# carmysouschef/mpcium

Hardware: AMD Instinct MI355X
Metric: 4096-bit modexp/s per GPU & node; 2-of-3 ECDSA sigs/s over 10k wallets (higher is better)
Workload: dtype u32; 1 GPU; config2: x^N mod N^2, 4096-bit modulus, shared 2048-bit exponent y=N; operands_per_gpu=65536, modulus_bits=4096, exp_bits=2048, parallelism=shard1 (independent operands, no collective)

## Files before the change

### include/mpcx.h

```cpp
#ifndef MPCX_H_
#define MPCX_H_

#include <stddef.h>
#include <stdint.h>

#ifdef __cplusplus
extern "C" {
#endif

#define MPCX_OK 0
#define MPCX_EINVAL 1
#define MPCX_ENODEV 2
#define MPCX_EHIP 3
#define MPCX_ENOMEM 4

#define MPCX_MAX_MODULUS_BITS 4096

typedef struct mpcx_modulus_s* mpcx_mod_t;

int mpcx_version(void);

const char* mpcx_last_error(void);

int mpcx_device_count(int* out_count);

#define MPCX_MAX_DEVICES 16

int mpcx_init(int device);

int mpcx_init_devices(int n_gpus);

int mpcx_partition(uint32_t count, int n_devices, uint32_t min_slice, uint32_t* first, uint32_t* n,
                   uint32_t* n_slices);

int mpcx_bound_devices(int* out_count, int* ordinals, int max_ordinals);

int mpcx_device_launches(int index, uint64_t* out);

int mpcx_kernel_stats(char* buf, size_t cap, int reset);

int mpcx_select_device(int index);

int mpcx_shutdown(void);

int mpcx_modulus_register(const uint32_t* m_words, uint32_t m_len, mpcx_mod_t* out);
int mpcx_modulus_release(mpcx_mod_t mod);

int mpcx_modulus_info(mpcx_mod_t mod, uint32_t* out_bits, uint32_t* out_class_words);

int mpcx_modexp_batch(mpcx_mod_t mod, uint32_t count,
                      const uint32_t* bases, uint32_t base_words,
                      const uint32_t* exps, uint32_t exp_words, int exp_shared,
                      uint32_t* out, uint32_t out_words);

int mpcx_modexp_batch_device(mpcx_mod_t mod, uint32_t count,
                             const uint32_t* d_bases, uint32_t base_words,
                             const uint32_t* d_exps, uint32_t exp_words, int exp_shared,
                             uint32_t exp_bits,
                             uint32_t* d_out, uint32_t out_words, void* stream);

int mpcx_modexp_mul_batch(mpcx_mod_t mod, uint32_t count,
                          const uint32_t* bases, uint32_t base_words,
                          const uint32_t* exps, uint32_t exp_words, int exp_shared,
                          const uint32_t* muls, uint32_t mul_words,
                          uint32_t* out, uint32_t out_words);
int mpcx_modexp_mul_batch_device(mpcx_mod_t mod, uint32_t count,
                                 const uint32_t* d_bases, uint32_t base_words,
                                 const uint32_t* d_exps, uint32_t exp_words, int exp_shared,
                                 uint32_t exp_bits,
                                 const uint32_t* d_muls, uint32_t mul_words,
                                 uint32_t* d_out, uint32_t out_words, void* stream);

typedef struct mpcx_job_s* mpcx_job_t;
int mpcx_modexp_submit(mpcx_mod_t mod, uint32_t count,
                       const uint32_t* bases, uint32_t base_words,
                       const uint32_t* exps, uint32_t exp_words, int exp_shared,
                       const uint32_t* muls, uint32_t mul_words,
                       uint32_t* out, uint32_t out_words, mpcx_job_t* job);
int mpcx_job_test(mpcx_job_t job, int* done);
int mpcx_job_wait(mpcx_job_t job);

int mpcx_mulmod_batch(mpcx_mod_t mod, uint32_t count,
                      const uint32_t* a, uint32_t a_words,
                      const uint32_t* b, uint32_t b_words,
                      uint32_t* out, uint32_t out_words);

int mpcx_fermat2_batch(uint32_t count, const uint32_t* p, uint32_t p_words, uint8_t* ok);

typedef struct {
  mpcx_mod_t mod;
  uint32_t count;
  const uint32_t* bases;
  uint32_t base_words;
  const uint32_t* exps;
  uint32_t exp_words;
  int exp_shared;
  const uint32_t* muls;
  uint32_t mul_words;
  uint32_t* out;
  uint32_t out_words;
} mpcx_modexp_group_t;
int mpcx_modexp_multi_batch(uint32_t n_groups, const mpcx_modexp_group_t* groups);

int mpcx_ec_combine_batch(uint32_t count, const uint32_t* scalars, const uint32_t* points, uint32_t* out);

int mpcx_mr_batch(uint32_t count, const uint32_t* n, uint32_t n_words, const uint32_t* bases, uint8_t* ok);

int mpcx_lucas_batch(uint32_t count, const uint32_t* n, uint32_t n_words, const uint32_t* P, uint8_t* ok);

int mpcx_safeprime_step(uint64_t seed, const uint8_t* raw, uint64_t stream_off, uint32_t count, uint32_t q_bits,
                        const uint32_t* sprp_q, uint32_t n_sprp, uint32_t max_pass, uint32_t* n_sieved,
                        uint32_t* n_pass, uint32_t* pass_idx, uint32_t* pass_p, uint8_t* sprp_ok);

int mpcx_safeprime_sieve_fermat(const uint8_t* raw, uint32_t nbytes, uint32_t count, uint32_t q_bits,
                                uint32_t* n_out, uint32_t* idx_out, uint8_t* ok_out);

typedef struct mpcx_fixedbase_s* mpcx_fb_t;
#define MPCX_FB_MAX_EXP_BITS 65536
int mpcx_fixedbase_register(mpcx_mod_t mod, const uint32_t* base, uint32_t base_words,
                            uint32_t max_exp_bits, mpcx_fb_t* out);
int mpcx_fixedbase_release(mpcx_fb_t fb);
int mpcx_fixedbase_info(mpcx_fb_t fb, uint32_t* max_exp_bits, size_t* table_bytes);

int mpcx_fixedbase_exp_batch(uint32_t nbases, const mpcx_fb_t* fbs, uint32_t count,
                             const uint32_t* const* exps, const uint32_t* exp_words,
                             const uint32_t* muls, uint32_t mul_words,
                             uint32_t* out, uint32_t out_words);

#define MPCX_FB_MAX_BASES 2
typedef struct {
  uint32_t nbases;
  mpcx_fb_t fbs[MPCX_FB_MAX_BASES];
  uint32_t count;
  const uint32_t* exps[MPCX_FB_MAX_BASES];
  uint32_t exp_words[MPCX_FB_MAX_BASES];
  const uint32_t* muls;
  uint32_t mul_words;
  uint32_t* out;
  uint32_t out_words;
} mpcx_fixedbase_group_t;
int mpcx_fixedbase_multi_batch(uint32_t n_groups, const mpcx_fixedbase_group_t* groups);

int mpcx_dev_alloc(size_t bytes, void** out_ptr);
int mpcx_dev_free(void* ptr);
int mpcx_host_alloc(size_t bytes, void** out_ptr);
int mpcx_host_free(void* ptr);
int mpcx_copy_stats(uint64_t* direct_bytes, uint64_t* bounced_bytes, uint64_t* bounce_allocs);
int mpcx_memcpy_h2d(void* d_dst, const void* h_src, size_t bytes);
int mpcx_memcpy_d2h(void* h_dst, const void* d_src, size_t bytes);
int mpcx_stream_create(void** out_stream);
int mpcx_stream_destroy(void* stream);
int mpcx_stream_sync(void* stream);
int mpcx_sync(void* stream);

int mpcx_set_option(const char* key, int value);
int mpcx_get_option(const char* key, int* value);

int mpcx_mx_tables(const uint32_t* m_words, uint32_t m_len, uint32_t L, uint8_t* out, size_t cap);

int mpcx_modulus_geometry(mpcx_mod_t mod, uint32_t* L, uint32_t* P, uint32_t* K, uint32_t* G);

#ifdef __cplusplus
}
#endif

#endif
```

### mpcium_amd/csrc/mpcx_api.cpp

```cpp
#include <hip/hip_runtime.h>

#include <algorithm>
#include <atomic>
#include <chrono>
#include <cmath>
#include <condition_variable>
#include <cstdarg>
#include <cstdio>
#include <cstdlib>
#include <cstring>
#include <ctime>
#include <deque>
#include <functional>
#include <map>
#include <memory>
#include <mutex>
#include <shared_mutex>
#include <string>
#include <thread>
#include <vector>

#include "../../include/mpcx.h"
#include "mpcx_internal.h"

#define MPCX_GEOM_DECL(g)                                                                              \
  hipError_t mpcx_launch_modexp_g##g(const mpcx::ModexpArgs* a, uint32_t waves, hipStream_t st);     \
  hipError_t mpcx_launch_modexp_multi_g##g(const mpcx::ModexpArgs* segs, const uint32_t* first,      \
                                           uint32_t nsegs, uint32_t waves, int mx, hipStream_t st);  \
  hipError_t mpcx_modexp_occupancy_g##g(int* blocks_per_cu);
#define MPCX_FOR_EACH_GEOM(X) X(0) X(1) X(2) X(3) X(4) X(5) X(6)
static_assert(MPCX_NUM_GEOMS == 7, "update MPCX_FOR_EACH_GEOM and build.py GEOMS");
extern "C" {
MPCX_FOR_EACH_GEOM(MPCX_GEOM_DECL)
hipError_t mpcx_launch_drbg(const mpcx::DrbgArgs* a, hipStream_t st);
hipError_t mpcx_launch_prime2c(mpcx::Prime2Args a, hipStream_t st);
hipError_t mpcx_launch_mrc(const mpcx::MrArgs* a, hipStream_t st);
hipError_t mpcx_launch_lucasc(const mpcx::LucasArgs* a, hipStream_t st);
hipError_t mpcx_launch_lucasc_wide(const mpcx::LucasArgs* a, hipStream_t st);
hipError_t mpcx_launch_expsched(const mpcx::ExpSchedArgs* a, hipStream_t st);
hipError_t mpcx_launch_fixedbase_g0(const mpcx::FixedBaseArgs* a, uint32_t blocks, uint32_t split, hipStream_t st);
hipError_t mpcx_launch_fixedbase_g1(const mpcx::FixedBaseArgs* a, uint32_t blocks, uint32_t split, hipStream_t st);
hipError_t mpcx_launch_fixedbase_multi_g0(const mpcx::FixedBaseArgs* segs, const uint32_t* first, uint32_t nsegs,
                                          uint32_t blocks, uint32_t split, hipStream_t st);
hipError_t mpcx_launch_fixedbase_multi_g1(const mpcx::FixedBaseArgs* segs, const uint32_t* first, uint32_t nsegs,
                                          uint32_t blocks, uint32_t split, hipStream_t st);
hipError_t mpcx_launch_sieve(const mpcx::SieveArgs* a, hipStream_t st);
hipError_t mpcx_launch_selftest(uint32_t* d_out, hipStream_t st);
hipError_t mpcx_launch_ec_combine(const uint32_t* sc, const uint32_t* pts, uint32_t* out, const uint32_t* gtab,
                                  uint32_t* ws, uint32_t count, hipStream_t st);
}

namespace {
constexpr int kMaxDevices = MPCX_MAX_DEVICES;
}

struct mpcx_modulus_s {
  int cls;
  uint32_t bits;
  uint32_t words;
  uint32_t n0inv;
  uint32_t const_off[MPCX_NUM_GEOMS];
  std::vector<uint32_t> m;
  std::vector<uint32_t> host_const;
  std::mutex mu;
  uint32_t* d_const[kMaxDevices] = {};
  std::vector<uint8_t> mx_host;
  uint8_t* d_mx[kMaxDevices] = {};
};

struct mpcx_fixedbase_s {
  mpcx_mod_t mod;
  int geom;
  uint32_t nwin;
  uint32_t wbits;
  std::vector<uint32_t> host_table;
  size_t table_words = 0;
  std::mutex mu;
  uint32_t* d_table[kMaxDevices] = {};
};

namespace {

constexpr int kDigitBits = 28;
constexpr uint32_t kM28 = (1u << kDigitBits) - 1u;

thread_local std::string g_err;
std::mutex g_mu;
int g_force_geom = -1;
double g_narrow_rounds = 0.15;
int g_geom_policy = 1;
int g_fixed_win = 5;
int g_sched_width = MPCX_SCHED_MAX_WIDTH;
int g_main_geom[MPCX_NUM_CLASSES] = {MPCX_MAIN_GEOM(0), MPCX_MAIN_GEOM(1), MPCX_MAIN_GEOM(2)};
int g_fb_window = MPCX_FB_WINDOW_BITS;
#ifndef MPCX_FB_SPLIT_DEFAULT
#define MPCX_FB_SPLIT_DEFAULT 0
#endif
int g_fb_split = MPCX_FB_SPLIT_DEFAULT;
uint32_t g_split_min = 4096;
bool g_dup_device = false;
#ifndef MPCX_MX_DEFAULT
#define MPCX_MX_DEFAULT 1
#endif
int g_mx = MPCX_MX_DEFAULT;
uint32_t g_mx_min = 2048;
uint32_t g_mx_seg_min = 64;
double g_mx_step = 0.81;
double g_geom_tput = 0.0;
struct Staging {
  void* ptr = nullptr;
  size_t bytes = 0;
};
struct Lane {
  std::mutex mu;
  hipStream_t st = nullptr;
  bool own_stream = true;
  hipEvent_t ev = nullptr;
  uint32_t* ws = nullptr;
  size_t ws_bytes = 0;
  Staging stage[4];
  Staging sieve[8];
  struct KEv {
    hipEvent_t a = nullptr, b = nullptr;
  };
  struct KPend {
    KEv ev;
    hipEvent_t ref;
    int dev;
    const char* kind;
    int geom;
    uint32_t ops;
    double alg;
  };
  std::vector<KEv> kev_free;
  std::vector<KPend> kpend;
  struct Bounce {
    char* p = nullptr;
    size_t cap = 0, used = 0;
    size_t peak = 0;
    uint32_t quiet = 0;
  };
  Bounce hin, hout;
  struct Post {
    void* dst;
    const void* src;
    size_t bytes;
  };
  std::vector<Post> post;
  bool pending = false;
};
constexpr int kMaxLanes = 8;
std::atomic<int> g_lanes{6};

struct Device {
  int ordinal = -1;
  hipEvent_t kref = nullptr;
  int num_cus = 0;
  int geom_slots[MPCX_NUM_GEOMS] = {0};
  Lane lanes[kMaxLanes];
  std::atomic<unsigned> lane_rr{0};
  std::mutex dev_mu;
  std::map<hipStream_t, std::unique_ptr<Lane>> dev_lanes;
  Lane build_lane;
  std::atomic<uint64_t> launches{0};
  std::mutex ec_mu;
  uint32_t* ec_gtab = nullptr;
};
Device g_devs[kMaxDevices];
std::atomic<int> g_ndev{0};
std::atomic<unsigned> g_dev_rr{0};
thread_local int t_sel = 0;
thread_local int t_hip = -1;

int fail(int code, const char* fmt, ...) {
  char buf[512];
  va_list ap;
  va_start(ap, fmt);
  vsnprintf(buf, sizeof buf, fmt, ap);
  va_end(ap);
  g_err = buf;
  return code;
}

int hip_fail(hipError_t e, const char* what) {
  return fail(MPCX_EHIP, "%s: %s", what, hipGetErrorString(e));
}

struct PinRegistry {
  std::shared_mutex mu;
  std::map<uintptr_t, size_t> ranges;
  void add(const void* p, size_t bytes) {
    std::unique_lock<std::shared_mutex> lk(mu);
    ranges[(uintptr_t)p] = bytes;
  }
  void remove(const void* p) {
    std::unique_lock<std::shared_mutex> lk(mu);
    ranges.erase((uintptr_t)p);
  }
  int lookup(const void* p, size_t bytes) {
    const uintptr_t a = (uintptr_t)p;
    std::shared_lock<std::shared_mutex> lk(mu);
    auto it = ranges.upper_bound(a);
    if (it == ranges.begin()) return 0;
    --it;
    if (a >= it->first + it->second) return 0;
    return a + bytes <= it->first + it->second ? 1 : -1;
  }
};
PinRegistry g_pins;
std::atomic<uint64_t> g_cp_direct{0}, g_cp_bounced{0}, g_cp_bounce_grow{0};

double go_macs(uint32_t mod_bits, uint32_t e_bits) {
  const double L = (double)((mod_bits + 31) / 32);
  return ((double)e_bits + (double)((e_bits + 3) / 4)) * 2.0 * L * L;
}
void launch_log(const char* kind, int geom, uint32_t count, uint32_t mod_bits, uint32_t exp_bits, double alg) {
  static std::mutex mu;
  static FILE* f = [] {
    const char* p = std::getenv("MPCX_LAUNCH_LOG");
    FILE* h = p && *p ? std::fopen(p, "w") : nullptr;
    if (h) std::fprintf(h, "kind,geom,operands,modulus_bits,exp_bits,alg_macs\n");
    return h;
  }();
  if (!f) return;
  std::lock_guard<std::mutex> lk(mu);
  std::fprintf(f, "%s,%d,%u,%u,%u,%.0f\n", kind, geom, count, mod_bits, exp_bits, alg);
  std::fflush(f);
}

std::atomic<bool> g_kstats{false};
struct KAgg {
  uint64_t launches = 0, ops = 0;
  double alg = 0.0, ms = 0.0;
};
std::mutex g_kmu;
std::map<std::pair<std::string, int>, KAgg> g_kagg;
std::vector<std::pair<double, double>> g_kiv[8];
uint64_t g_kref_host_ns[8] = {};
uint64_t mono_ns() {
  timespec ts{};
  clock_gettime(CLOCK_MONOTONIC, &ts);
  return (uint64_t)ts.tv_sec * 1000000000ull + (uint64_t)ts.tv_nsec;
}
FILE* ktrace_file() {
  static FILE* f = [] {
    const char* p = std::getenv("MPCX_KTRACE");
    FILE* h = p && *p ? std::fopen(p, "w") : nullptr;
    if (h) std::fprintf(h, "dev,kind,geom,ops,t0_ns,t1_ns\n");
    return h;
  }();
  return f;
}

int kstat_begin(Lane& l) {
  if (!g_kstats.load(std::memory_order_relaxed) || l.kpend.size() >= 512) return -1;
  Lane::KEv ev;
  if (!l.kev_free.empty()) {
    ev = l.kev_free.back();
    l.kev_free.pop_back();
  } else if (hipEventCreate(&ev.a) != hipSuccess || hipEventCreate(&ev.b) != hipSuccess) {
    return -1;
  }
  if (hipEventRecord(ev.a, l.st) != hipSuccess) {
    l.kev_free.push_back(ev);
    return -1;
  }
  l.kpend.push_back({ev, nullptr, -1, nullptr, 0, 0, 0.0});
  return (int)l.kpend.size() - 1;
}

void kstat_end(Lane& l, int slot, const Device& d, int dev, const char* kind, int geom, uint32_t ops, double alg) {
  if (slot < 0) return;
  Lane::KPend& p = l.kpend[(size_t)slot];
  if (!d.kref || hipEventRecord(p.ev.b, l.st) != hipSuccess) {
    l.kev_free.push_back(p.ev);
    l.kpend.erase(l.kpend.begin() + slot);
    return;
  }
  p.ref = d.kref;
  p.dev = dev;
  p.kind = kind;
  p.geom = geom;
  p.ops = ops;
  p.alg = alg;
}

void kstat_credit(const char* kind, int geom, uint64_t ops, double alg) {
  if (!g_kstats.load(std::memory_order_relaxed)) return;
  std::lock_guard<std::mutex> lk(g_kmu);
  KAgg& a = g_kagg[{kind, geom}];
  a.ops += ops;
  a.alg += alg;
}

void kstat_resolve(Lane& l) {
  std::lock_guard<std::mutex> lk(g_kmu);
  for (auto& p : l.kpend) {
    float ms = 0.f, t0 = 0.f;
    if (p.kind && hipEventElapsedTime(&ms, p.ev.a, p.ev.b) == hipSuccess &&
        hipEventElapsedTime(&t0, p.ref, p.ev.a) == hipSuccess) {
      KAgg& a = g_kagg[{p.kind, p.geom}];
      a.launches += 1;
      a.ops += p.ops;
      a.alg += p.alg;
      a.ms += ms;
      if (p.dev >= 0 && p.dev < 8) g_kiv[p.dev].push_back({(double)t0, (double)t0 + ms});
      if (FILE* kf = ktrace_file(); kf && p.dev >= 0 && p.dev < 8) {
        const uint64_t b = g_kref_host_ns[p.dev];
        std::fprintf(kf, "%d,%s,%d,%u,%llu,%llu\n", p.dev, p.kind, p.geom, p.ops,
                     (unsigned long long)(b + (uint64_t)(t0 * 1e6)), (unsigned long long)(b + (uint64_t)((t0 + ms) * 1e6)));
      }
    }
    l.kev_free.push_back(p.ev);
  }
  l.kpend.clear();
}

int class_for_bits(uint32_t bits) {
  for (int c = 0; c < MPCX_NUM_CLASSES; ++c)
    if ((int)bits <= MPCX_CLASS_MAXBITS(c)) return c;
  return -1;
}

uint32_t bit_length(const std::vector<uint32_t>& x) {
  for (int i = (int)x.size() - 1; i >= 0; --i)
    if (x[i]) return (uint32_t)(32 * i + (32 - __builtin_clz(x[i])));
  return 0;
}

uint32_t bit_length_words(const uint32_t* x, uint32_t n) {
  for (int i = (int)n - 1; i >= 0; --i)
    if (x[i]) return (uint32_t)(32 * i + (32 - __builtin_clz(x[i])));
  return 0;
}

bool geq(const std::vector<uint32_t>& x, const std::vector<uint32_t>& m) {
  for (int i = (int)x.size() - 1; i >= 0; --i)
    if (x[i] != m[i]) return x[i] > m[i];
  return true;
}

std::vector<uint32_t> pow2_mod(uint32_t k, const std::vector<uint32_t>& m) {
  const size_t n = m.size();
  std::vector<uint32_t> x(n + 1, 0), mm(m);
  mm.push_back(0);
  x[0] = 1;
  if (n == 1 && m[0] == 1) return std::vector<uint32_t>(n, 0);
  for (uint32_t i = 0; i < k; ++i) {
    uint32_t c = 0;
    for (size_t j = 0; j <= n; ++j) {
      const uint32_t nc = x[j] >> 31;
      x[j] = (x[j] << 1) | c;
      c = nc;
    }
    if (geq(x, mm)) {
      uint64_t br = 0;
      for (size_t j = 0; j <= n; ++j) {
        const uint64_t d = (uint64_t)x[j] - mm[j] - br;
        x[j] = (uint32_t)d;
        br = (d >> 63) & 1;
      }
    }
  }
  x.resize(n);
  return x;
}

std::vector<uint32_t> to_digits(const std::vector<uint32_t>& w, uint32_t L) {
  std::vector<uint32_t> d(L, 0);
  for (uint32_t i = 0; i < L; ++i) {
    const uint32_t bit = i * kDigitBits, wi = bit >> 5, s = bit & 31;
    uint64_t v = 0;
    if (wi < w.size()) v = w[wi];
    if (wi + 1 < w.size()) v |= (uint64_t)w[wi + 1] << 32;
    d[i] = (uint32_t)(v >> s) & kM28;
  }
  return d;
}

static void mul_lo(const uint32_t* a, const uint32_t* b, uint32_t* out, uint32_t n) {
  std::vector<uint64_t> acc(n, 0);
  for (uint32_t i = 0; i < n; ++i) {
    uint64_t carry = 0;
    for (uint32_t j = 0; i + j < n; ++j) {
      const uint64_t t = (uint64_t)a[i] * b[j] + (acc[i + j] & 0xFFFFFFFFu) + carry;
      acc[i + j] = (acc[i + j] & ~0xFFFFFFFFull) | (t & 0xFFFFFFFFu);
      carry = t >> 32;
    }
  }
  for (uint32_t i = 0; i < n; ++i) out[i] = (uint32_t)acc[i];
}

struct MxDims {
  uint32_t n7, d, stride, img;
};
static bool mx_dims(uint32_t L, MxDims* o) {
  if (L == mpcx::MxG2::L) {
    *o = {mpcx::MxG2::N7, mpcx::MxG2::D, mpcx::MxG2::TAB_STRIDE, mpcx::MxG2::IMG_BYTES};
  } else if (L == mpcx::MxG5::L) {
    *o = {mpcx::MxG5::N7, mpcx::MxG5::D, mpcx::MxG5::TAB_STRIDE, mpcx::MxG5::IMG_BYTES};
  } else {
    return false;
  }
  return true;
}

static void mx_tables(const std::vector<uint32_t>& m, uint32_t L, std::vector<uint8_t>& out) {
  MxDims dm{};
  (void)mx_dims(L, &dm);
  const uint32_t W = (kDigitBits * L + 31) / 32;
  std::vector<uint32_t> mm(W, 0), x(W, 0), t(W, 0), u(W, 0);
  for (size_t i = 0; i < m.size() && i < W; ++i) mm[i] = m[i];
  uint32_t inv = mm[0];
  for (int i = 0; i < 5; ++i) inv *= 2u - mm[0] * inv;
  x[0] = inv;
  for (uint32_t prec = 1; prec < W;) {
    const uint32_t np = std::min(2 * prec, W);
    mul_lo(mm.data(), x.data(), t.data(), np);
    uint64_t c = 3;
    for (uint32_t i = 0; i < np; ++i) {
      const uint64_t v = (uint64_t)(uint32_t)~t[i] + c;
      t[i] = (uint32_t)v;
      c = v >> 32;
    }
    mul_lo(x.data(), t.data(), u.data(), np);
    for (uint32_t i = 0; i < np; ++i) x[i] = u[i];
    prec = np;
  }
  uint64_t br = 1;
  for (uint32_t i = 0; i < W; ++i) {
    const uint64_t v = (uint64_t)(uint32_t)~x[i] + br;
    x[i] = (uint32_t)v;
    br = v >> 32;
  }
  auto d7 = [](const std::vector<uint32_t>& w, uint32_t d) -> uint8_t {
    const uint32_t bit = 7 * d, wi = bit >> 5, sh = bit & 31;
    uint64_t v = wi < w.size() ? w[wi] : 0;
    if (wi + 1 < w.size()) v |= (uint64_t)w[wi + 1] << 32;
    return (uint8_t)((v >> sh) & 0x7F);
  };
  std::vector<uint8_t> n2(dm.n7), n1(dm.n7);
  std::vector<uint32_t> mv(m);
  for (uint32_t d = 0; d < dm.n7; ++d) {
    n2[d] = d7(x, d);
    n1[d] = d7(mv, d);
  }
  out.assign(dm.img, 0);
  auto fill = [&](const std::vector<uint8_t>& v7, uint8_t* dst) {
    for (int i = 0; i < 16; ++i)
      for (int xx = 0; xx < (int)dm.stride; ++xx) {
        const int idx = (int)dm.d - xx + i;
        if (idx >= 0 && idx < (int)dm.n7) dst[i * dm.stride + xx] = v7[idx];
      }
  };
  fill(n2, out.data());
  fill(n1, out.data() + dm.img / 2);
}

hipError_t mpcx_launch_modexp(int geom, const mpcx::ModexpArgs* a, uint32_t waves, hipStream_t st) {
  switch (geom) {
#define MPCX_CASE(g) \
  case g:            \
    return mpcx_launch_modexp_g##g(a, waves, st);
    MPCX_FOR_EACH_GEOM(MPCX_CASE)
#undef MPCX_CASE
    default:
      return hipErrorInvalidValue;
  }
}

hipError_t mpcx_launch_modexp_multi(int geom, const mpcx::ModexpArgs* segs, const uint32_t* first, uint32_t nsegs,
                                    uint32_t waves, int mx, hipStream_t st) {
  switch (geom) {
#define MPCX_CASE(g) \
  case g:            \
    return mpcx_launch_modexp_multi_g##g(segs, first, nsegs, waves, mx, st);
    MPCX_FOR_EACH_GEOM(MPCX_CASE)
#undef MPCX_CASE
    default:
      return hipErrorInvalidValue;
  }
}

hipError_t mpcx_modexp_occupancy(int geom, int* blocks_per_cu) {
  switch (geom) {
#define MPCX_CASE(g) \
  case g:            \
    return mpcx_modexp_occupancy_g##g(blocks_per_cu);
    MPCX_FOR_EACH_GEOM(MPCX_CASE)
#undef MPCX_CASE
    default:
      return hipErrorInvalidValue;
  }
}

int bind(const Device& d) {
  if (t_hip != d.ordinal) {
    hipError_t e = hipSetDevice(d.ordinal);
    if (e != hipSuccess) return hip_fail(e, "hipSetDevice");
    t_hip = d.ordinal;
  }
  return MPCX_OK;
}

int ndev_or_fail() {
  const int n = g_ndev.load(std::memory_order_acquire);
  if (n <= 0) return -fail(MPCX_ENODEV, "mpcx_init() has not been called");
  return n;
}

int selected(Device** out) {
  const int n = ndev_or_fail();
  if (n < 0) return -n;
  if (t_sel < 0 || t_sel >= n) return fail(MPCX_EINVAL, "selected device %d not bound (%d bound)", t_sel, n);
  *out = &g_devs[t_sel];
  return bind(**out);
}

Lane& acquire_lane(Device& d, std::unique_lock<std::mutex>& lk) {
  const unsigned start = d.lane_rr.fetch_add(1, std::memory_order_relaxed);
  const int nl = g_lanes.load(std::memory_order_relaxed);
  for (int i = 0; i < nl; ++i) {
    Lane& l = d.lanes[(start + i) % nl];
    std::unique_lock<std::mutex> t(l.mu, std::try_to_lock);
    if (t.owns_lock()) {
      lk = std::move(t);
      return l;
    }
  }
  Lane& l = d.lanes[start % nl];
  lk = std::unique_lock<std::mutex>(l.mu);
  return l;
}

int lane_stream(Lane& l) {
  if (!l.st && l.own_stream) {
    hipError_t e = hipStreamCreateWithFlags(&l.st, hipStreamNonBlocking);
    if (e != hipSuccess) {
      l.st = nullptr;
      return hip_fail(e, "hipStreamCreate(lane)");
    }
  }
  if (!l.ev) {
    hipError_t e = hipEventCreateWithFlags(&l.ev, hipEventBlockingSync | hipEventDisableTiming);
    if (e != hipSuccess) {
      l.ev = nullptr;
      return hip_fail(e, "hipEventCreate(lane)");
    }
  }
  return MPCX_OK;
}

constexpr size_t kBounceKeep = (size_t)64 << 20;
constexpr uint32_t kBounceQuiet = 256;
void retire_pinned(char* p, size_t bytes);
void bounce_trim(Lane& l) {
  for (Lane::Bounce* b : {&l.hin, &l.hout}) {
    if (b->cap <= kBounceKeep) {
      b->peak = 0;
      continue;
    }
    b->quiet = b->peak <= kBounceKeep ? b->quiet + 1 : 0;
    b->peak = 0;
    if (b->quiet >= kBounceQuiet) {
      retire_pinned(b->p, b->cap);
      *b = Lane::Bounce{};
    }
  }
}

int lane_wait(Lane& l) {
  static const int mode = [] {
    const char* e = std::getenv("MPCX_LANE_WAIT");
    return !e ? 0 : std::strcmp(e, "event") == 0 ? 1 : std::strcmp(e, "stream") == 0 ? 2 : 0;
  }();
  hipError_t e;
  if (mode == 2) {
    e = hipStreamSynchronize(l.st);
  } else {
    e = hipEventRecord(l.ev, l.st);
    if (e == hipSuccess && mode == 1) {
      e = hipEventSynchronize(l.ev);
    } else if (e == hipSuccess) {
      for (int us = 20;; us = std::min(100, us + us / 2)) {
        e = hipEventQuery(l.ev);
        if (e != hipErrorNotReady) break;
        std::this_thread::sleep_for(std::chrono::microseconds(us));
      }
    }
  }
  if (e != hipSuccess) {
    (void)hipStreamSynchronize(l.st);
    l.post.clear();
    l.hin.used = l.hout.used = 0;
    l.pending = false;
    return hip_fail(e, "lane wait");
  }
  for (const auto& p : l.post) std::memcpy(p.dst, p.src, p.bytes);
  l.post.clear();
  l.hin.used = l.hout.used = 0;
  l.pending = false;
  bounce_trim(l);
  if (!l.kpend.empty()) kstat_resolve(l);
  return MPCX_OK;
}

struct LaneDrain {
  Lane& l;
  explicit LaneDrain(Lane& lane) : l(lane) {}
  ~LaneDrain() {
    if (!l.pending) return;
    if (l.st) (void)hipStreamSynchronize(l.st);
    l.post.clear();
    l.hin.used = l.hout.used = 0;
    l.pending = false;
  }
  LaneDrain(const LaneDrain&) = delete;
  LaneDrain& operator=(const LaneDrain&) = delete;
};

void retire_pinned(char* p, size_t bytes);
int bounce_reserve(Lane& l, Lane::Bounce& b, size_t bytes, char** out) {
  const size_t need = (bytes + 255) & ~(size_t)255;
  if (b.used + need > b.cap) {
    if (l.hin.used || l.hout.used) {
      hipError_t e = hipStreamSynchronize(l.st);
      if (e != hipSuccess) return hip_fail(e, "bounce-buffer wait");
      for (const auto& p : l.post) std::memcpy(p.dst, p.src, p.bytes);
      l.post.clear();
      l.hin.used = l.hout.used = 0;
    }
    if (need > b.cap) {
      if (b.p) retire_pinned(b.p, b.cap);
      b.p = nullptr;
      b.cap = 0;
      const size_t want = std::max<size_t>({need + need / 4, (size_t)1 << 20});
      hipError_t e = hipHostMalloc((void**)&b.p, want, hipHostMallocPortable);
      if (e != hipSuccess) {
        b.p = nullptr;
        return fail(MPCX_ENOMEM, "hipHostMalloc(bounce %zu): %s", want, hipGetErrorString(e));
      }
      b.cap = want;
      g_cp_bounce_grow.fetch_add(1, std::memory_order_relaxed);
    }
  }
  *out = b.p + b.used;
  b.used += need;
  b.peak = std::max(b.peak, b.used);
  return MPCX_OK;
}

int h2d(Lane& l, void* d, const void* h, size_t bytes) {
  if (!bytes) return MPCX_OK;
  const int pin = g_pins.lookup(h, bytes);
  if (pin < 0) return fail(MPCX_EINVAL, "host source of %zu B at %p overruns its pinned allocation", bytes, h);
  const void* src = h;
  if (pin == 0) {
    char* b = nullptr;
    if (int rc = bounce_reserve(l, l.hin, bytes, &b)) return rc;
    std::memcpy(b, h, bytes);
    src = b;
    g_cp_bounced.fetch_add(bytes, std::memory_order_relaxed);
  } else {
    g_cp_direct.fetch_add(bytes, std::memory_order_relaxed);
  }
  l.pending = true;
  hipError_t e = hipMemcpyAsync(d, src, bytes, hipMemcpyHostToDevice, l.st);
  return e == hipSuccess ? MPCX_OK : hip_fail(e, "copy inputs");
}

int d2h(Lane& l, void* h, const void* d, size_t bytes) {
  if (!bytes) return MPCX_OK;
  const int pin = g_pins.lookup(h, bytes);
  if (pin < 0) return fail(MPCX_EINVAL, "host destination of %zu B at %p overruns its pinned allocation", bytes, h);
  void* dst = h;
  if (pin == 0) {
    char* b = nullptr;
    if (int rc = bounce_reserve(l, l.hout, bytes, &b)) return rc;
    dst = b;
    l.post.push_back({h, b, bytes});
    g_cp_bounced.fetch_add(bytes, std::memory_order_relaxed);
  } else {
    g_cp_direct.fetch_add(bytes, std::memory_order_relaxed);
  }
  l.pending = true;
  hipError_t e = hipMemcpyAsync(dst, d, bytes, hipMemcpyDeviceToHost, l.st);
  return e == hipSuccess ? MPCX_OK : hip_fail(e, "copy results");
}

int d2h_sync(void* h, const void* d, size_t bytes, Lane& l) {
  if (int rc = d2h(l, h, d, bytes)) return rc;
  return lane_wait(l);
}

constexpr size_t kStageChunk = (size_t)16 << 20;
struct StageChunks {
  std::mutex mu;
  std::vector<char*> free_list;
  size_t allocated = 0;
  char* get() {
    {
      std::lock_guard<std::mutex> lk(mu);
      if (!free_list.empty()) {
        char* c = free_list.back();
        free_list.pop_back();
        return c;
      }
    }
    char* c = nullptr;
    if (hipHostMalloc((void**)&c, kStageChunk, hipHostMallocPortable) != hipSuccess) return nullptr;
    std::lock_guard<std::mutex> lk(mu);
    ++allocated;
    return c;
  }
  void put(char* c) {
    std::lock_guard<std::mutex> lk(mu);
    free_list.push_back(c);
  }
  void release_all() {
    std::lock_guard<std::mutex> lk(mu);
    for (char* c : free_list) (void)hipHostFree(c);
    free_list.clear();
    allocated = 0;
  }
};
StageChunks g_stage_chunks;

constexpr size_t kRetireMax = (size_t)1 << 30;
std::mutex g_retire_mu;
std::vector<std::pair<char*, size_t>> g_retired;
size_t g_retired_bytes = 0;
void retire_pinned(char* p, size_t bytes) {
  std::vector<std::pair<char*, size_t>> out;
  {
    std::lock_guard<std::mutex> lk(g_retire_mu);
    g_retired.push_back({p, bytes});
    g_retired_bytes += bytes;
    if (g_retired_bytes > kRetireMax) {
      out.swap(g_retired);
      g_retired_bytes = 0;
    }
  }
  for (auto& r : out) (void)hipHostFree(r.first);
}
void free_retired() {
  std::lock_guard<std::mutex> lk(g_retire_mu);
  for (auto& r : g_retired) (void)hipHostFree(r.first);
  g_retired.clear();
  g_retired_bytes = 0;
}

int copy_sync(void* dst, const void* src, size_t bytes, hipMemcpyKind kind, hipStream_t st) {
  if (!bytes) return MPCX_OK;
  const void* hp = kind == hipMemcpyHostToDevice ? src : dst;
  const int pin = g_pins.lookup(hp, bytes);
  if (pin < 0) return fail(MPCX_EINVAL, "host range of %zu B at %p overruns its pinned allocation", bytes, hp);
  hipError_t e;
  if (pin == 1) {
    e = hipMemcpyAsync(dst, src, bytes, kind, st);
    if (e == hipSuccess) e = hipStreamSynchronize(st);
    return e == hipSuccess ? MPCX_OK : hip_fail(e, "copy");
  }
  char* buf = g_stage_chunks.get();
  if (!buf) return fail(MPCX_ENOMEM, "hipHostMalloc(copy chunk %zu)", kStageChunk);
  const size_t cb = std::min(bytes, kStageChunk);
  e = hipSuccess;
  for (size_t off = 0; off < bytes && e == hipSuccess; off += cb) {
    const size_t n = std::min(cb, bytes - off);
    if (kind == hipMemcpyHostToDevice) {
      std::memcpy(buf, (const char*)src + off, n);
      e = hipMemcpyAsync((char*)dst + off, buf, n, kind, st);
      if (e == hipSuccess) e = hipStreamSynchronize(st);
    } else {
      e = hipMemcpyAsync(buf, (const char*)src + off, n, kind, st);
      if (e == hipSuccess) e = hipStreamSynchronize(st);
      if (e == hipSuccess) std::memcpy((char*)dst + off, buf, n);
    }
  }
  g_stage_chunks.put(buf);
  g_cp_bounced.fetch_add(bytes, std::memory_order_relaxed);
  return e == hipSuccess ? MPCX_OK : hip_fail(e, "copy");
}

size_t grown(size_t old_bytes, size_t bytes) {
  return std::max<size_t>({bytes + bytes / 4, old_bytes + old_bytes / 2, (size_t)1 << 20});
}

int ensure_buffer(Staging& s, size_t bytes) {
  if (s.bytes >= bytes && s.ptr) return MPCX_OK;
  const size_t want = grown(s.bytes, bytes);
  if (s.ptr) (void)hipFree(s.ptr);
  s.ptr = nullptr;
  s.bytes = 0;
  hipError_t e = hipMalloc(&s.ptr, want);
  if (e != hipSuccess) return fail(MPCX_ENOMEM, "hipMalloc(%zu): %s", want, hipGetErrorString(e));
  s.bytes = want;
  return MPCX_OK;
}

int ensure_workspace(Lane& l, size_t bytes) {
  if (l.ws_bytes >= bytes) return MPCX_OK;
  if (l.ws) {
    (void)hipStreamSynchronize(l.st);
    (void)hipFree(l.ws);
  }
  const size_t want = grown(l.ws_bytes, bytes);
  l.ws = nullptr;
  l.ws_bytes = 0;
  hipError_t e = hipMalloc((void**)&l.ws, want);
  if (e != hipSuccess) return fail(MPCX_ENOMEM, "hipMalloc(workspace %zu): %s", want, hipGetErrorString(e));
  l.ws_bytes = want;
  return MPCX_OK;
}

void drop_lane(Lane& l) {
  std::lock_guard<std::mutex> ll(l.mu);
  if (l.st) {
    (void)hipStreamSynchronize(l.st);
    if (l.own_stream) (void)hipStreamDestroy(l.st);
  }
  l.st = nullptr;
  if (l.ev) (void)hipEventDestroy(l.ev);
  l.ev = nullptr;
  for (auto& p : l.kpend) l.kev_free.push_back(p.ev);
  l.kpend.clear();
  for (auto& ev : l.kev_free) {
    (void)hipEventDestroy(ev.a);
    (void)hipEventDestroy(ev.b);
  }
  l.kev_free.clear();
  if (l.ws) (void)hipFree(l.ws);
  l.ws = nullptr;
  l.ws_bytes = 0;
  for (auto& s : l.stage) {
    if (s.ptr) (void)hipFree(s.ptr);
    s = Staging{};
  }
  for (auto& s : l.sieve) {
    if (s.ptr) (void)hipFree(s.ptr);
    s = Staging{};
  }
  for (Lane::Bounce* b : {&l.hin, &l.hout}) {
    if (b->p) (void)hipHostFree(b->p);
    *b = Lane::Bounce{};
  }
  l.post.clear();
  l.pending = false;
}

Lane& stream_lane(Device& d, hipStream_t st) {
  std::lock_guard<std::mutex> lk(d.dev_mu);
  auto& p = d.dev_lanes[st];
  if (!p) {
    p.reset(new Lane());
    p->own_stream = false;
    p->st = st;
  }
  return *p;
}

int run_selftest() {
  uint32_t* d = nullptr;
  hipError_t e = hipMalloc((void**)&d, 256 * sizeof(uint32_t));
  if (e != hipSuccess) return hip_fail(e, "selftest alloc");
  e = mpcx_launch_selftest(d, nullptr);
  std::vector<uint32_t> h(256);
  if (e == hipSuccess && copy_sync(h.data(), d, 256 * sizeof(uint32_t), hipMemcpyDeviceToHost, nullptr) != MPCX_OK)
    e = hipErrorInvalidValue;
  (void)hipFree(d);
  if (e != hipSuccess) return hip_fail(e, "selftest");
  for (uint32_t l = 0; l < 64; ++l) {
    const uint32_t nxt = l < 63 ? 1000 + l + 1 : 0;
    const uint32_t prv = l > 0 ? 1000 + l - 1 : 0;
    const uint32_t bp = 2000 + (l / 7) * 7;
    const uint64_t acc = (uint64_t)(0xFFFFFFF0u + l) * (0xFFFFFFF7u - l) + 0xFFFFFFFFFFFFull;
    if (h[l] != nxt || h[64 + l] != prv || h[128 + l] != bp || h[192 + l] != (uint32_t)(acc >> 32))
      return fail(MPCX_EHIP,
                  "device self-test failed at lane %u (dpp next %u/%u prev %u/%u bpermute %u/%u mad %u/%u)", l,
                  h[l], nxt, h[64 + l], prv, h[128 + l], bp, h[192 + l], (uint32_t)(acc >> 32));
  }
  return MPCX_OK;
}

int bind_new_device(int ordinal) {
  const int n = g_ndev.load();
  for (int i = 0; i < n && !g_dup_device; ++i)
    if (g_devs[i].ordinal == ordinal) return MPCX_OK;
  if (n >= kMaxDevices) return fail(MPCX_EINVAL, "more than %d devices", kMaxDevices);
  int vis = 0;
  hipError_t e = hipGetDeviceCount(&vis);
  if (e != hipSuccess || vis <= 0) return fail(MPCX_ENODEV, "no HIP device visible");
  if (ordinal < 0 || ordinal >= vis) return fail(MPCX_EINVAL, "device %d out of range [0,%d)", ordinal, vis);
  e = hipSetDevice(ordinal);
  if (e != hipSuccess) return hip_fail(e, "hipSetDevice");
  t_hip = ordinal;
  hipDeviceProp_t prop;
  e = hipGetDeviceProperties(&prop, ordinal);
  if (e != hipSuccess) return hip_fail(e, "hipGetDeviceProperties");
  if (std::strncmp(prop.gcnArchName, "gfx950", 6) != 0)
    return fail(MPCX_ENODEV, "device %d is %s; libmpcx is built for gfx950 only", ordinal, prop.gcnArchName);
  Device& d = g_devs[n];
  d.ordinal = ordinal;
  d.num_cus = prop.multiProcessorCount;
  for (int g = 0; g < MPCX_NUM_GEOMS; ++g) {
    int b = 0;
    if (mpcx_modexp_occupancy(g, &b) != hipSuccess || b <= 0) b = 1;
    d.geom_slots[g] = b * d.num_cus;
  }
  int rc = run_selftest();
  if (rc != MPCX_OK) {
    d.ordinal = -1;
    return rc;
  }
  g_ndev.store(n + 1, std::memory_order_release);
  return MPCX_OK;
}

int mod_const(mpcx_mod_t mod, int di, const uint32_t** out) {
  std::lock_guard<std::mutex> lk(mod->mu);
  if (!mod->d_const[di]) {
    uint32_t* p = nullptr;
    hipError_t e = hipMalloc((void**)&p, mod->host_const.size() * sizeof(uint32_t));
    if (e != hipSuccess) return fail(MPCX_ENOMEM, "hipMalloc(modulus): %s", hipGetErrorString(e));
    if (int rc = copy_sync(p, mod->host_const.data(), mod->host_const.size() * sizeof(uint32_t),
                           hipMemcpyHostToDevice, nullptr)) {
      (void)hipFree(p);
      return rc;
    }
    mod->d_const[di] = p;
  }
  *out = mod->d_const[di];
  return MPCX_OK;
}

int mx_const(mpcx_mod_t mod, int di, const uint8_t** out) {
  std::lock_guard<std::mutex> lk(mod->mu);
  if (!mod->d_mx[di]) {
    if (mod->mx_host.empty()) mx_tables(mod->m, (uint32_t)MPCX_GEOM_L(MPCX_MAIN_GEOM(mod->cls)), mod->mx_host);
    uint8_t* p = nullptr;
    hipError_t e = hipMalloc((void**)&p, mod->mx_host.size());
    if (e != hipSuccess) return fail(MPCX_ENOMEM, "hipMalloc(mx tables): %s", hipGetErrorString(e));
    if (int rc = copy_sync(p, mod->mx_host.data(), mod->mx_host.size(), hipMemcpyHostToDevice, nullptr)) {
      (void)hipFree(p);
      return rc;
    }
    mod->d_mx[di] = p;
  }
  *out = mod->d_mx[di];
  return MPCX_OK;
}

int fb_table(mpcx_fb_t fb, int di, const uint32_t** out) {
  std::lock_guard<std::mutex> lk(fb->mu);
  if (!fb->d_table[di]) {
    uint32_t* p = nullptr;
    const size_t bytes = fb->table_words * sizeof(uint32_t);
    hipError_t e = hipMalloc((void**)&p, bytes);
    if (e != hipSuccess) return fail(MPCX_ENOMEM, "hipMalloc(fixed-base table %zu B)", bytes);
    if (!fb->host_table.empty()) {
      const int rc = copy_sync(p, fb->host_table.data(), bytes, hipMemcpyHostToDevice, nullptr);
      e = rc ? hipErrorInvalidValue : hipSuccess;
      if (rc == MPCX_OK) std::vector<uint32_t>().swap(fb->host_table);
    } else {
      int src = -1;
      for (int j = 0; j < kMaxDevices && src < 0; ++j)
        if (fb->d_table[j]) src = j;
      e = src < 0 ? hipErrorInvalidValue
                  : hipMemcpyPeerAsync(p, g_devs[di].ordinal, fb->d_table[src], g_devs[src].ordinal, bytes, nullptr);
      if (e == hipSuccess) e = hipStreamSynchronize(nullptr);
    }
    if (e != hipSuccess) {
      (void)hipFree(p);
      return hip_fail(e, "upload fixed-base table");
    }
    fb->d_table[di] = p;
  }
  *out = fb->d_table[di];
  return MPCX_OK;
}

uint32_t partition(uint32_t count, int n_dev, uint32_t min_slice, uint32_t* first, uint32_t* cnt) {
  uint32_t slices = n_dev > 0 ? (uint32_t)n_dev : 1u;
  if (min_slice == 0) slices = 1;
  else slices = std::min<uint32_t>(slices, std::max<uint32_t>(1, count / min_slice));
  const uint32_t per = (count + slices - 1) / std::max<uint32_t>(slices, 1);
  uint32_t used = 0;
  for (uint32_t s = 0; s < slices; ++s) {
    const uint32_t f = std::min(count, s * per), c = std::min(count, f + per) - f;
    if (first) first[s] = f;
    if (cnt) cnt[s] = c;
    used = s + 1;
  }
  return used;
}

int run_sliced(uint32_t count, uint32_t min_slice, const std::function<int(int, uint32_t, uint32_t)>& fn) {
  const int n = ndev_or_fail();
  if (n < 0) return -n;
  uint32_t first[kMaxDevices], cnt[kMaxDevices];
  const uint32_t slices = partition(count, n, min_slice, first, cnt);
  if (slices <= 1) {
    const int di = (int)(g_dev_rr.fetch_add(1, std::memory_order_relaxed) % (unsigned)n);
    int rc = bind(g_devs[di]);
    return rc ? rc : fn(di, 0, count);
  }
  std::vector<int> rcs(slices, MPCX_OK);
  std::vector<std::string> msgs(slices);
  std::vector<std::thread> th;
  for (uint32_t s = 0; s < slices; ++s) {
    th.emplace_back([&, s] {
      int rc = bind(g_devs[s]);
      if (!rc) rc = fn((int)s, first[s], cnt[s]);
      rcs[s] = rc;
      if (rc) msgs[s] = g_err;
    });
  }
  for (auto& t : th) t.join();
  for (uint32_t s = 0; s < slices; ++s)
    if (rcs[s]) {
      g_err = msgs[s];
      return rcs[s];
    }
  return MPCX_OK;
}

bool geom_serves(int g, const mpcx_modulus_s* mod, bool ops_fit) {
  const uint32_t rb = (uint32_t)MPCX_GEOM_RBITS(g);
  if (mod->bits + 2u > rb) return false;
  return ops_fit || rb >= 32u * (uint32_t)MPCX_CLASS_WORDS(mod->cls);
}

bool host_ops_below(const uint32_t* x, uint32_t count, uint32_t words, uint32_t rbits) {
  if (!x || 32u * words <= rbits) return true;
  const uint32_t w0 = rbits / 32u, sh = rbits % 32u;
  for (uint32_t i = 0; i < count; ++i) {
    const uint32_t* v = x + (size_t)i * words;
    if (sh && (v[w0] >> sh)) return false;
    for (uint32_t w = w0 + (sh ? 1u : 0u); w < words; ++w)
      if (v[w]) return false;
  }
  return true;
}

int main_geom_for(const mpcx_modulus_s* mod, bool ops_fit) {
  const int g = g_main_geom[mod->cls];
  return geom_serves(g, mod, ops_fit) ? g : MPCX_FULL_GEOM(mod->cls);
}


bool runs_on_mx(int g, uint32_t total, uint32_t min_seg, bool multi) {
  const bool has_kernel = g == 2 || (g == 5 && !multi && g_mx >= 2);
  return g_mx && has_kernel && total >= g_mx_min && (!multi || min_seg >= g_mx_seg_min);
}

int fastest_geom(int cls, uint32_t count, int nsimd, bool mx_ok) {
  struct M {
    int g;
    double c0, s;
  };
  const M ms[3] = {{MPCX_MAIN_GEOM(cls), 0.10, mx_ok ? g_mx_step : 1.0}, {MPCX_MID_GEOM(cls), 0.12, 0.585},
                   {MPCX_NARROW_GEOM(cls), 0.20, 0.245}};
  int best = ms[0].g;
  double tb = 1e300;
  for (const M& m : ms) {
    const uint32_t G = (uint32_t)MPCX_GEOM_G(m.g);
    const double waves = (double)((count + G - 1) / G);
    const double t = m.c0 + m.s * std::ceil(waves / (double)std::max(1, nsimd)) +
                     g_geom_tput * m.s * waves / (double)std::max(1, nsimd);
    if (t < tb) {
      tb = t;
      best = m.g;
    }
  }
  return best;
}

int choose_geom(const Device& dev, int cls, uint32_t count, bool main_serves, bool forced_serves, bool mx_ok) {
  const int gm = main_serves ? g_main_geom[cls] : MPCX_FULL_GEOM(cls);
  const int gn = MPCX_NARROW_GEOM(cls), gmid = MPCX_MID_GEOM(cls);
  if (g_force_geom >= 0 && MPCX_GEOM_CLASS(g_force_geom) == cls)
    return forced_serves ? g_force_geom : MPCX_FULL_GEOM(cls);
  if (g_geom_policy == 2) return gm;
  if (g_geom_policy == 1 && gmid >= 0 && gn >= 0) return fastest_geom(cls, count, dev.num_cus * 4, mx_ok && main_serves);
  const uint32_t G = (uint32_t)MPCX_GEOM_G(gm);
  const double rounds = (double)((count + G - 1) / G) / (double)std::max(1, dev.geom_slots[gm]);
  if (gn >= 0 && rounds < g_narrow_rounds) return gn;
  return gm;
}

int check_batch(const char* pre, const mpcx_modulus_s* mod, uint32_t count, const uint32_t* bases,
                uint32_t base_words, const uint32_t* exps, uint32_t exp_words, const uint32_t* muls,
                uint32_t mul_words, const uint32_t* out, uint32_t out_words) {
  const bool grp = *pre;
  const uint32_t cw = (uint32_t)MPCX_CLASS_WORDS(mod->cls);
  if (base_words == 0 || base_words > cw)
    return grp ? fail(MPCX_EINVAL, "%sbase_words %u", pre, base_words)
               : fail(MPCX_EINVAL, "base_words %u outside [1, %u] (reduce mod m first)", base_words, cw);
  if (muls && (mul_words == 0 || mul_words > cw))
    return grp ? fail(MPCX_EINVAL, "%smul_words", pre)
               : fail(MPCX_EINVAL, "mul_words %u outside [1, %u]", mul_words, cw);
  if (out_words < mod->words)
    return grp ? fail(MPCX_EINVAL, "%sout_words < modulus words", pre)
               : fail(MPCX_EINVAL, "out_words %u < modulus words %u", out_words, mod->words);
  if (count && (!bases || !out || (exp_words && !exps))) return fail(MPCX_EINVAL, "%snull buffer", pre);
  return MPCX_OK;
}

double go_macs_sum(uint32_t mod_bits, const uint32_t* exps, uint32_t exp_words, uint32_t count) {
  double alg = 0.0;
  for (uint32_t i = 0; i < count; ++i)
    alg += go_macs(mod_bits, bit_length_words(exps + (size_t)i * exp_words, exp_words));
  return alg;
}

int launch_expsched(const uint32_t* d_exp, uint32_t exp_words, uint32_t* sched, hipStream_t st) {
  mpcx::ExpSchedArgs sa{};
  sa.exp = d_exp;
  sa.exp_words = exp_words;
  sa.max_width = (uint32_t)g_sched_width;
  sa.sched = sched;
  hipError_t e = mpcx_launch_expsched(&sa, st);
  return e == hipSuccess ? MPCX_OK : hip_fail(e, "launch k_expsched");
}

mpcx::ModexpArgs modexp_args(const mpcx_modulus_s* mod, int geom, const uint32_t* dconst, uint32_t count,
                             const uint32_t* base, uint32_t base_words, const uint32_t* exps, uint32_t exp_words,
                             const uint32_t* mul, uint32_t mul_words, uint32_t* out, uint32_t out_words,
                             uint32_t* table, uint32_t exp_bits, int exp_shared, const uint32_t* sched,
                             const uint8_t* mx_img, uint32_t nwaves) {
  const uint32_t L = (uint32_t)MPCX_GEOM_L(geom);
  mpcx::ModexpArgs a{};
  a.nd = dconst + mod->const_off[geom];
  a.r1d = a.nd + L;
  a.r2d = a.nd + 2 * L;
  a.base = base;
  a.exps = exps;
  a.mul = mul;
  a.out = out;
  a.table = table;
  a.count = count;
  a.base_words = base_words;
  a.exp_words = exp_words;
  a.mul_words = mul ? mul_words : 0;
  a.exp_bits = exp_words ? exp_bits : 0;
  a.win_bits = (!exp_shared && a.exp_bits > 1024u && g_fixed_win >= 5) ? 5u : 4u;
  a.out_words = out_words;
  a.n0inv = mod->n0inv;
  a.exp_shared = exp_shared ? 1 : 0;
  a.sched = sched;
  a.mx_img = mx_img;
  a.nwaves = nwaves;
  return a;
}


int fb_group_check(const mpcx_fixedbase_group_t& g, const char* pre, uint32_t* nwin) {
  const bool grp = *pre;
  if (g.nbases == 0 || g.nbases > MPCX_FB_MAX_BASES)
    return fail(MPCX_EINVAL, "%snbases %u outside [1, %d]", pre, g.nbases, MPCX_FB_MAX_BASES);
  for (uint32_t t = 0; t < g.nbases; ++t) {
    if (!g.fbs[t]) return fail(MPCX_EINVAL, "%snull fixed base %u", pre, t);
    if (g.fbs[t]->mod != g.fbs[0]->mod) return fail(MPCX_EINVAL, "%sfixed bases of different moduli", pre);
  }
  mpcx_mod_t mod = g.fbs[0]->mod;
  const uint32_t cw = (uint32_t)MPCX_CLASS_WORDS(mod->cls);
  if (g.out_words < mod->words)
    return grp ? fail(MPCX_EINVAL, "%sout_words < modulus words", pre)
               : fail(MPCX_EINVAL, "out_words %u < modulus words %u", g.out_words, mod->words);
  if (g.muls && (g.mul_words == 0 || g.mul_words > cw))
    return grp ? fail(MPCX_EINVAL, "%smul_words", pre)
               : fail(MPCX_EINVAL, "mul_words %u outside [1, %u]", g.mul_words, cw);
  if (g.count == 0) return MPCX_OK;
  if (!g.out) return fail(MPCX_EINVAL, "%snull output", pre);
  for (uint32_t t = 0; t < g.nbases; ++t) {
    if (g.exp_words[t] && !g.exps[t]) return fail(MPCX_EINVAL, "%snull exponents %u", pre, t);
    uint32_t bits = 0;
    for (uint32_t i = 0; i < g.count && g.exp_words[t]; ++i)
      bits = std::max(bits, bit_length_words(g.exps[t] + (size_t)i * g.exp_words[t], g.exp_words[t]));
    const uint32_t wb = g.fbs[t]->wbits;
    if (bits > g.fbs[t]->nwin * wb)
      return fail(MPCX_EINVAL, "%sexponent of %u bits > fixed-base table's %u", pre, bits, g.fbs[t]->nwin * wb);
    nwin[t] = (bits + wb - 1) / wb;
  }
  return MPCX_OK;
}

struct FbWork {
  double alg = 0.0, exec = 0.0;
  uint32_t eb_max = 0;
};
FbWork fb_group_work(const mpcx_fixedbase_group_t& g) {
  FbWork w;
  const uint32_t bits = g.fbs[0]->mod->bits;
  const double l2 = 2.0 * (double)((bits + 31) / 32) * (double)((bits + 31) / 32);
  for (uint32_t t = 0; t < g.nbases; ++t)
    for (uint32_t i = 0; i < g.count && g.exp_words[t]; ++i) {
      const uint32_t b = bit_length_words(g.exps[t] + (size_t)i * g.exp_words[t], g.exp_words[t]);
      w.alg += go_macs(bits, b);
      w.exec += (double)((b + g.fbs[t]->wbits - 1) / g.fbs[t]->wbits) * l2;
      w.eb_max = std::max(w.eb_max, b);
    }
  if (g.muls) w.exec += (double)g.count * l2;
  return w;
}

int fixedbase_args(const mpcx_fixedbase_group_t& g, int geom, int di, const uint32_t* nwin,
                   const uint32_t* const* d_exps, const uint32_t* d_mul, uint32_t* d_out, mpcx::FixedBaseArgs* out) {
  mpcx_mod_t mod = g.fbs[0]->mod;
  const uint32_t* dconst = nullptr;
  int rc;
  if ((rc = mod_const(mod, di, &dconst))) return rc;
  mpcx::FixedBaseArgs a{};
  a.nd = dconst + mod->const_off[geom];
  a.r1d = a.nd + MPCX_GEOM_L(geom);
  a.r2d = a.nd + 2 * MPCX_GEOM_L(geom);
  for (uint32_t t = 0; t < g.nbases; ++t) {
    if ((rc = fb_table(g.fbs[t], di, &a.tables[t]))) return rc;
    a.exps[t] = d_exps[t];
    a.exp_words[t] = g.exp_words[t];
    a.nwin[t] = nwin[t];
    a.wbits[t] = g.fbs[t]->wbits;
  }
  a.nbases = g.nbases;
  a.mul = g.muls ? d_mul : nullptr;
  a.mul_words = g.muls ? g.mul_words : 0;
  a.out = d_out;
  a.out_words = g.out_words;
  a.count = g.count;
  a.n0inv = mod->n0inv;
  *out = a;
  return MPCX_OK;
}

int fb_geom_for(const mpcx_modulus_s* mod) { return MPCX_FULL_GEOM(mod->cls); }
hipError_t launch_fixedbase(int geom, const mpcx::FixedBaseArgs* a, uint32_t blocks, uint32_t split, hipStream_t st) {
  return geom == 0 ? mpcx_launch_fixedbase_g0(a, blocks, split, st) : mpcx_launch_fixedbase_g1(a, blocks, split, st);
}
hipError_t launch_fixedbase_multi(int geom, const mpcx::FixedBaseArgs* segs, const uint32_t* first, uint32_t nsegs,
                                  uint32_t blocks, uint32_t split, hipStream_t st) {
  return geom == 0 ? mpcx_launch_fixedbase_multi_g0(segs, first, nsegs, blocks, split, st)
                   : mpcx_launch_fixedbase_multi_g1(segs, first, nsegs, blocks, split, st);
}

constexpr uint32_t kFbSplitWaves = 4;
uint32_t fb_split_for(const Device& dev, uint32_t blocks) {
  if (g_fb_split) return (uint32_t)g_fb_split;
  const uint64_t cap = (uint64_t)std::max(1, dev.num_cus) * 4u * kFbSplitWaves;
  for (uint32_t s = MPCX_FB_MAX_SPLIT; s > 1; s >>= 1)
    if ((uint64_t)blocks * s <= cap) return s;
  return 1;
}

}

extern "C" {

int mpcx_version(void) { return 200; }

int mpcx_get_option(const char* key, int* value) {
  if (!key || !value) return fail(MPCX_EINVAL, "null option or output");
  std::lock_guard<std::mutex> lk(g_mu);
  if (std::strcmp(key, "mx") == 0) {
    *value = g_mx;
  } else if (std::strcmp(key, "mx_min") == 0) {
    *value = (int)g_mx_min;
  } else if (std::strcmp(key, "mx_seg_min") == 0) {
    *value = (int)g_mx_seg_min;
  } else if (std::strcmp(key, "mx_step") == 0) {
    *value = (int)std::lround(g_mx_step * 100.0);
  } else if (std::strcmp(key, "geom_tput") == 0) {
    *value = (int)std::lround(g_geom_tput * 100.0);
  } else if (std::strcmp(key, "geom_policy") == 0) {
    *value = g_geom_policy;
  } else if (std::strcmp(key, "sched_width") == 0) {
    *value = g_sched_width;
  } else if (std::strcmp(key, "fixed_window") == 0) {
    *value = g_fixed_win;
  } else if (std::strcmp(key, "fb_split") == 0) {
    *value = g_fb_split;
  } else if (std::strcmp(key, "lanes") == 0) {
    *value = g_lanes.load();
  } else {
    return fail(MPCX_EINVAL, "option %s cannot be read", key);
  }
  return MPCX_OK;
}

int mpcx_set_option(const char* key, int value) {
  if (!key) return fail(MPCX_EINVAL, "null option");
  std::lock_guard<std::mutex> lk(g_mu);
  if (std::strcmp(key, "force_geom") == 0) {
    if (value < -1 || value >= MPCX_NUM_GEOMS) return fail(MPCX_EINVAL, "force_geom %d out of range", value);
    g_force_geom = value;
  } else if (std::strcmp(key, "sched_width") == 0) {
    if (value < 0 || value > MPCX_SCHED_MAX_WIDTH) return fail(MPCX_EINVAL, "sched_width %d out of range", value);
    g_sched_width = value;
  } else if (std::strcmp(key, "narrow_rounds") == 0) {
    if (value < 0 || value > 100) return fail(MPCX_EINVAL, "narrow_rounds %d out of range", value);
    g_narrow_rounds = value / 100.0;
  } else if (std::strcmp(key, "fb_window") == 0) {
    if (value < 4 || value > MPCX_FB_MAX_WINDOW_BITS) return fail(MPCX_EINVAL, "fb_window %d out of range", value);
    g_fb_window = value;
  } else if (std::strcmp(key, "fb_split") == 0) {
    if (value != 0 && value != 1 && value != 2 && value != 4) return fail(MPCX_EINVAL, "fb_split %d not 0/1/2/4", value);
    g_fb_split = value;
  } else if (std::strcmp(key, "mx") == 0) {
    if (value < 0 || value > 2) return fail(MPCX_EINVAL, "mx %d not 0, 1 or 2", value);
    g_mx = value;
  } else if (std::strcmp(key, "mx_min") == 0) {
    if (value < 1) return fail(MPCX_EINVAL, "mx_min %d < 1", value);
    g_mx_min = (uint32_t)value;
  } else if (std::strcmp(key, "mx_seg_min") == 0) {
    if (value < 1) return fail(MPCX_EINVAL, "mx_seg_min %d < 1", value);
    g_mx_seg_min = (uint32_t)value;
  } else if (std::strcmp(key, "mx_step") == 0) {
    if (value < 10 || value > 200) return fail(MPCX_EINVAL, "mx_step %d outside [10, 200]", value);
    g_mx_step = value / 100.0;
  } else if (std::strcmp(key, "geom_tput") == 0) {
    if (value < 0 || value > 1000) return fail(MPCX_EINVAL, "geom_tput %d outside [0, 1000]", value);
    g_geom_tput = value / 100.0;
  } else if (std::strcmp(key, "fixed_window") == 0) {
    if (value != 4 && value != 5) return fail(MPCX_EINVAL, "fixed_window %d not 4 or 5", value);
    g_fixed_win = value;
  } else if (std::strcmp(key, "lanes") == 0) {
    if (value < 1 || value > kMaxLanes) return fail(MPCX_EINVAL, "lanes %d outside [1, %d]", value, kMaxLanes);
    g_lanes = value;
  } else if (std::strcmp(key, "geom_policy") == 0) {
    if (value < 0 || value > 2) return fail(MPCX_EINVAL, "geom_policy %d out of range", value);
    g_geom_policy = value;
  } else if (std::strcmp(key, "main_geom") == 0) {
    if (value < 0 || value >= MPCX_NUM_GEOMS) return fail(MPCX_EINVAL, "main_geom %d out of range", value);
    g_main_geom[MPCX_GEOM_CLASS(value)] = value;
  } else if (std::strcmp(key, "duplicate_device") == 0) {
    g_dup_device = value != 0;
  } else if (std::strcmp(key, "kernel_stats") == 0) {
    g_kstats = value != 0;
  } else if (std::strcmp(key, "device_split_min") == 0) {
    if (value < 0) return fail(MPCX_EINVAL, "device_split_min %d < 0", value);
    g_split_min = (uint32_t)value;
  } else {
    return fail(MPCX_EINVAL, "unknown option %s", key);
  }
  return MPCX_OK;
}

const char* mpcx_last_error(void) { return g_err.c_str(); }

int mpcx_device_count(int* out_count) {
  if (!out_count) return fail(MPCX_EINVAL, "null out_count");
  int n = 0;
  hipError_t e = hipGetDeviceCount(&n);
  if (e != hipSuccess) n = 0;
  *out_count = n;
  return MPCX_OK;
}

static void read_env_options() {
  const char* nr = std::getenv("MPCX_NARROW_ROUNDS");
  if (nr) g_narrow_rounds = std::max(0, std::min(100, std::atoi(nr))) / 100.0;
  const char* gp = std::getenv("MPCX_GEOM_POLICY");
  if (gp) g_geom_policy = std::max(0, std::min(2, std::atoi(gp)));
  const char* ln = std::getenv("MPCX_LANES");
  if (ln && g_ndev.load() == 0) g_lanes = std::max(1, std::min(kMaxLanes, std::atoi(ln)));
  const char* fw = std::getenv("MPCX_FB_WINDOW");
  if (fw) g_fb_window = std::max(4, std::min(MPCX_FB_MAX_WINDOW_BITS, std::atoi(fw)));
  const char* mx = std::getenv("MPCX_MX");
  if (mx) g_mx = std::max(0, std::min(2, std::atoi(mx)));
  const char* ms = std::getenv("MPCX_MX_STEP");
  if (ms) g_mx_step = std::max(10, std::min(200, std::atoi(ms))) / 100.0;
  const char* gt = std::getenv("MPCX_GEOM_TPUT");
  if (gt) g_geom_tput = std::max(0, std::min(1000, std::atoi(gt))) / 100.0;
}

int mpcx_init(int device) {
  std::lock_guard<std::mutex> lk(g_mu);
  read_env_options();
  return bind_new_device(device);
}

int mpcx_init_devices(int n_gpus) {
  std::lock_guard<std::mutex> lk(g_mu);
  read_env_options();
  int vis = 0;
  hipError_t e = hipGetDeviceCount(&vis);
  if (e != hipSuccess || vis <= 0) return fail(MPCX_ENODEV, "no HIP device visible");
  if (n_gpus <= 0) n_gpus = vis;
  if (n_gpus > vis) return fail(MPCX_EINVAL, "%d GPUs requested, %d visible", n_gpus, vis);
  for (int i = 0; i < n_gpus; ++i)
    if (int rc = bind_new_device(i)) return rc;
  return MPCX_OK;
}

int mpcx_bound_devices(int* out_count, int* ordinals, int max_ordinals) {
  if (!out_count) return fail(MPCX_EINVAL, "null out_count");
  const int n = g_ndev.load(std::memory_order_acquire);
  *out_count = n;
  for (int i = 0; ordinals && i < n && i < max_ordinals; ++i) ordinals[i] = g_devs[i].ordinal;
  return MPCX_OK;
}

int mpcx_partition(uint32_t count, int n_devices, uint32_t min_slice, uint32_t* first, uint32_t* n,
                   uint32_t* n_slices) {
  if (!n_slices) return fail(MPCX_EINVAL, "null n_slices");
  if (n_devices < 1 || n_devices > kMaxDevices) return fail(MPCX_EINVAL, "n_devices %d outside [1, %d]", n_devices, kMaxDevices);
  *n_slices = partition(count, n_devices, min_slice, first, n);
  return MPCX_OK;
}

int mpcx_device_launches(int index, uint64_t* out) {
  const int n = g_ndev.load(std::memory_order_acquire);
  if (!out) return fail(MPCX_EINVAL, "null out");
  if (index < 0 || index >= n) return fail(MPCX_EINVAL, "device index %d not bound (%d bound)", index, n);
  *out = g_devs[index].launches.load();
  return MPCX_OK;
}

int mpcx_kernel_stats(char* buf, size_t cap, int reset) {
  const int n = g_ndev.load(std::memory_order_acquire);
  std::string out;
  {
    std::lock_guard<std::mutex> lk(g_kmu);
    double busy = 0.0, alg = 0.0;
    for (int i = 0; i < n && i < 8; ++i) {
      auto iv = g_kiv[i];
      std::sort(iv.begin(), iv.end());
      double s0 = 0.0, e0 = -1.0;
      for (const auto& x : iv) {
        if (x.first > e0) {
          if (e0 > s0) busy += e0 - s0;
          s0 = x.first;
          e0 = x.second;
        } else {
          e0 = std::max(e0, x.second);
        }
      }
      if (e0 > s0) busy += e0 - s0;
    }
    char line[320];
    std::string ks;
    for (const auto& kv : g_kagg) {
      alg += kv.second.alg;
      std::snprintf(line, sizeof line,
                    "%s{\"kind\":\"%s\",\"geom\":%d,\"launches\":%llu,\"operands\":%llu,\"alg_macs\":%.6e,"
                    "\"kernel_ms\":%.4f}",
                    ks.empty() ? "" : ",", kv.first.first.c_str(), kv.first.second,
                    (unsigned long long)kv.second.launches, (unsigned long long)kv.second.ops, kv.second.alg,
                    kv.second.ms);
      ks += line;
    }
    std::snprintf(line, sizeof line, "{\"enabled\":%d,\"busy_ms\":%.4f,\"alg_macs\":%.6e,\"kernels\":[",
                  g_kstats.load() ? 1 : 0, busy, alg);
    out = line + ks + "]}";
    if (reset) {
      g_kagg.clear();
      for (auto& v : g_kiv) v.clear();
    }
  }
  if (reset) {
    for (int i = 0; i < n; ++i) {
      Device& d = g_devs[i];
      if (int rc = bind(d)) return rc;
      hipError_t e = d.kref ? hipSuccess : hipEventCreate(&d.kref);
      if (e == hipSuccess) e = hipEventRecord(d.kref, nullptr);
      if (e == hipSuccess) e = hipEventSynchronize(d.kref);
      if (e != hipSuccess) return hip_fail(e, "kernel stats time origin");
      if (i < 8) g_kref_host_ns[i] = mono_ns();
    }
  }
  if (buf && cap) {
    if (out.size() + 1 > cap) return fail(MPCX_EINVAL, "kernel stats need %zu bytes", out.size() + 1);
    std::memcpy(buf, out.c_str(), out.size() + 1);
  }
  return MPCX_OK;
}

int mpcx_select_device(int index) {
  const int n = g_ndev.load(std::memory_order_acquire);
  if (index < 0 || index >= n) return fail(MPCX_EINVAL, "device index %d not bound (%d bound)", index, n);
  t_sel = index;
  return bind(g_devs[index]);
}

int mpcx_shutdown(void) {
  std::lock_guard<std::mutex> lk(g_mu);
  const int n = g_ndev.load();
  for (int i = 0; i < n; ++i) {
    Device& d = g_devs[i];
    if (hipSetDevice(d.ordinal) != hipSuccess) continue;
    t_hip = d.ordinal;
    for (auto& l : d.lanes) drop_lane(l);
    drop_lane(d.build_lane);
    if (d.ec_gtab) (void)hipFree(d.ec_gtab);
    d.ec_gtab = nullptr;
    {
      std::lock_guard<std::mutex> dl(d.dev_mu);
      for (auto& kv : d.dev_lanes) drop_lane(*kv.second);
      d.dev_lanes.clear();
    }
    d.ordinal = -1;
  }
  g_stage_chunks.release_all();
  free_retired();
  g_ndev.store(0);
  return MPCX_OK;
}

int mpcx_modulus_register(const uint32_t* m_words, uint32_t m_len, mpcx_mod_t* out) {
  if (!m_words || !out || m_len == 0) return fail(MPCX_EINVAL, "null modulus or output");
  Device* dev = nullptr;
  if (int rc = selected(&dev)) return rc;
  std::vector<uint32_t> m(m_words, m_words + m_len);
  while (m.size() > 1 && m.back() == 0) m.pop_back();
  const uint32_t bits = bit_length(m);
  if (bits == 0) return fail(MPCX_EINVAL, "modulus is zero");
  if ((m[0] & 1u) == 0) return fail(MPCX_EINVAL, "modulus is even (math/big uses a non-Montgomery path; keep it on the host)");
  const int cls = class_for_bits(bits);
  if (cls < 0) return fail(MPCX_EINVAL, "modulus has %u bits > %d", bits, MPCX_MAX_MODULUS_BITS);
  auto* mod = new mpcx_modulus_s();
  mod->cls = cls;
  mod->bits = bits;
  mod->words = (uint32_t)m.size();
  mod->m = m;
  uint32_t inv = m[0];
  for (int i = 0; i < 5; ++i) inv *= 2u - m[0] * inv;
  mod->n0inv = (0u - inv) & kM28;
  for (int g = 0; g < MPCX_NUM_GEOMS; ++g) {
    mod->const_off[g] = 0;
    if (MPCX_GEOM_CLASS(g) != cls) continue;
    const uint32_t L = (uint32_t)MPCX_GEOM_L(g);
    mod->const_off[g] = (uint32_t)mod->host_const.size();
    auto nd = to_digits(m, L);
    auto r1 = to_digits(pow2_mod(kDigitBits * L, m), L);
    auto r2 = to_digits(pow2_mod(2 * kDigitBits * L, m), L);
    auto& h = mod->host_const;
    h.insert(h.end(), nd.begin(), nd.end());
    h.insert(h.end(), r1.begin(), r1.end());
    h.insert(h.end(), r2.begin(), r2.end());
  }
  const uint32_t* p = nullptr;
  if (int rc = mod_const(mod, (int)(dev - g_devs), &p)) {
    delete mod;
    return rc;
  }
  *out = mod;
  return MPCX_OK;
}

int mpcx_modulus_release(mpcx_mod_t mod) {
  if (!mod) return fail(MPCX_EINVAL, "null modulus");
  const int n = g_ndev.load();
  for (int i = 0; i < n && i < kMaxDevices; ++i) {
    if (mod->d_const[i] && bind(g_devs[i]) == MPCX_OK) (void)hipFree(mod->d_const[i]);
    if (mod->d_mx[i] && bind(g_devs[i]) == MPCX_OK) (void)hipFree(mod->d_mx[i]);
  }
  delete mod;
  return MPCX_OK;
}

int mpcx_mx_tables(const uint32_t* m_words, uint32_t m_len, uint32_t L, uint8_t* out, size_t cap) {
  if (!m_words || !out || m_len == 0) return fail(MPCX_EINVAL, "null modulus or output");
  MxDims dm{};
  if (!mx_dims(L, &dm)) return fail(MPCX_EINVAL, "L %u is not an MX geometry's (148 or 74)", L);
  if (cap < dm.img) return fail(MPCX_EINVAL, "mx tables need %u bytes", dm.img);
  std::vector<uint32_t> m(m_words, m_words + m_len);
  while (m.size() > 1 && m.back() == 0) m.pop_back();
  if ((m[0] & 1u) == 0 || bit_length(m) + 2 > kDigitBits * L)
    return fail(MPCX_EINVAL, "mx tables need an odd modulus of < %u bits", kDigitBits * L - 2);
  std::vector<uint8_t> t;
  mx_tables(m, L, t);
  std::memcpy(out, t.data(), dm.img);
  return MPCX_OK;
}

int mpcx_modulus_info(mpcx_mod_t mod, uint32_t* out_bits, uint32_t* out_class_words) {
  if (!mod) return fail(MPCX_EINVAL, "null modulus");
  if (out_bits) *out_bits = mod->bits;
  if (out_class_words) *out_class_words = (uint32_t)MPCX_CLASS_WORDS(mod->cls);
  return MPCX_OK;
}

int mpcx_modulus_geometry(mpcx_mod_t mod, uint32_t* L, uint32_t* P, uint32_t* K, uint32_t* G) {
  if (!mod) return fail(MPCX_EINVAL, "null modulus");
  const int g = main_geom_for(mod, true);
  if (L) *L = (uint32_t)MPCX_GEOM_L(g);
  if (P) *P = (uint32_t)MPCX_GEOM_P(g);
  if (K) *K = (uint32_t)MPCX_GEOM_K(g);
  if (G) *G = (uint32_t)MPCX_GEOM_G(g);
  return MPCX_OK;
}

}

static int modexp_enqueue(int di, Lane& lane, mpcx_mod_t mod, uint32_t count, const uint32_t* d_bases,
                          uint32_t base_words, const uint32_t* d_exps, uint32_t exp_words, int exp_shared,
                          uint32_t exp_bits, const uint32_t* d_muls, uint32_t mul_words, uint32_t* d_out,
                          uint32_t out_words, bool ops_fit, double alg_macs = -1.0) {
  Device& dev = g_devs[di];
  int rc;
  if ((rc = check_batch("", mod, count, d_bases, base_words, d_exps, exp_words, d_muls, mul_words, d_out, out_words)))
    return rc;
  if (exp_bits > 32u * exp_words) return fail(MPCX_EINVAL, "exp_bits %u > 32*exp_words", exp_bits);
  if (count == 0) return MPCX_OK;
  const uint32_t* dconst = nullptr;
  if ((rc = mod_const(mod, di, &dconst))) return rc;
  const int cls = mod->cls;
  const bool forced_serves =
      g_force_geom >= 0 && MPCX_GEOM_CLASS(g_force_geom) == cls && geom_serves(g_force_geom, mod, ops_fit);
  const bool mx_ok = runs_on_mx(main_geom_for(mod, ops_fit), count, count, false);
  const int geom = choose_geom(dev, cls, count, geom_serves(g_main_geom[cls], mod, ops_fit), forced_serves, mx_ok);
  const uint32_t G = (uint32_t)MPCX_GEOM_G(geom), K = (uint32_t)MPCX_GEOM_K(geom);
  const uint32_t waves = (count + G - 1) / G;
  const bool use_sched = exp_shared && exp_bits > 0 && g_sched_width > 0;
  const size_t sched_off = (size_t)waves * MPCX_TABLE_ENTRIES * K * 64u;
  const size_t ws_words = sched_off + (use_sched ? MPCX_SCHED_WORDS(32u * exp_words) : 0);
  if ((rc = ensure_workspace(lane, ws_words * sizeof(uint32_t)))) return rc;
  uint32_t* sched = use_sched ? lane.ws + sched_off : nullptr;
  if (use_sched && (rc = launch_expsched(d_exps, exp_words, sched, lane.st))) return rc;
  const bool mx = runs_on_mx(geom, count, count, false);
  const uint8_t* mx_img = nullptr;
  if (mx && (rc = mx_const(mod, di, &mx_img))) return rc;
  const mpcx::ModexpArgs a =
      modexp_args(mod, geom, dconst, count, d_bases, base_words, d_exps, exp_words, d_muls, mul_words, d_out,
                  out_words, lane.ws, exp_bits, exp_shared, sched, mx_img, waves);
  const char* kind = mx ? "modexp_mx" : "modexp";
  const int ks = kstat_begin(lane);
  hipError_t e = mpcx_launch_modexp(geom, &a, waves, lane.st);
  if (e != hipSuccess) return hip_fail(e, "launch k_modexp");
  dev.launches.fetch_add(1, std::memory_order_relaxed);
  const double alg = alg_macs >= 0 ? alg_macs : go_macs(mod->bits, a.exp_bits) * count;
  kstat_end(lane, ks, dev, di, kind, geom, count, alg);
  launch_log(kind, geom, count, mod->bits, a.exp_bits, alg);
  return MPCX_OK;
}

static uint32_t max_exp_bits(const uint32_t* exps, uint32_t exp_words, int exp_shared, uint32_t count) {
  uint32_t bits = 0;
  if (!exp_words) return 0;
  if (exp_shared) return bit_length_words(exps, exp_words);
  for (uint32_t i = 0; i < count; ++i) bits = std::max(bits, bit_length_words(exps + (size_t)i * exp_words, exp_words));
  return bits;
}

static int modexp_host_range(int di, mpcx_mod_t mod, uint32_t count, const uint32_t* bases, uint32_t base_words,
                             const uint32_t* exps, uint32_t exp_words, int exp_shared, const uint32_t* muls,
                             uint32_t mul_words, uint32_t* out, uint32_t out_words) {
  const uint32_t exp_bits = max_exp_bits(exps, exp_words, exp_shared, count);
  const size_t n_exp_words = exp_shared ? exp_words : (size_t)count * exp_words;
  const size_t bb = (size_t)count * base_words * 4, eb = std::max<size_t>(n_exp_words * 4, 4),
               ob = (size_t)count * out_words * 4, mb = muls ? (size_t)count * mul_words * 4 : 0;
  std::unique_lock<std::mutex> lk;
  Lane& l = acquire_lane(g_devs[di], lk);
  LaneDrain drain(l);
  int rc;
  if ((rc = lane_stream(l))) return rc;
  Staging* sg = l.stage;
  if ((rc = ensure_buffer(sg[0], bb)) || (rc = ensure_buffer(sg[1], eb)) || (rc = ensure_buffer(sg[2], ob)) ||
      (muls && (rc = ensure_buffer(sg[3], mb))))
    return rc;
  if ((rc = h2d(l, sg[0].ptr, bases, bb)) || (rc = h2d(l, sg[1].ptr, exps, n_exp_words * 4)) ||
      (muls && (rc = h2d(l, sg[3].ptr, muls, mb))))
    return rc;
  const uint32_t rb = (uint32_t)MPCX_GEOM_RBITS(g_main_geom[mod->cls]);
  const bool ops_fit = host_ops_below(bases, count, base_words, rb) && host_ops_below(muls, count, mul_words, rb);
  const double alg = !exp_shared && exp_words ? go_macs_sum(mod->bits, exps, exp_words, count) : -1.0;
  rc = modexp_enqueue(di, l, mod, count, (const uint32_t*)sg[0].ptr, base_words, (const uint32_t*)sg[1].ptr,
                      exp_words, exp_shared, exp_bits, muls ? (const uint32_t*)sg[3].ptr : nullptr, mul_words,
                      (uint32_t*)sg[2].ptr, out_words, ops_fit, alg);
  if (rc) return rc;
  return d2h_sync(out, sg[2].ptr, ob, l);
}

static int modexp_host(mpcx_mod_t mod, uint32_t count, const uint32_t* bases, uint32_t base_words,
                       const uint32_t* exps, uint32_t exp_words, int exp_shared, const uint32_t* muls,
                       uint32_t mul_words, uint32_t* out, uint32_t out_words) {
  if (!mod) return fail(MPCX_EINVAL, "null modulus");
  if (count == 0) return MPCX_OK;
  if (!bases || !out || (exp_words && !exps)) return fail(MPCX_EINVAL, "null buffer");
  return run_sliced(count, g_split_min, [&](int di, uint32_t first, uint32_t n) {
    return modexp_host_range(di, mod, n, bases + (size_t)first * base_words, base_words,
                             exps ? (exp_shared ? exps : exps + (size_t)first * exp_words) : nullptr, exp_words,
                             exp_shared, muls ? muls + (size_t)first * mul_words : nullptr, mul_words,
                             out + (size_t)first * out_words, out_words);
  });
}

struct mpcx_job_s {
  std::mutex mu;
  std::condition_variable cv;
  bool done = false;
  int rc = MPCX_OK;
  std::string msg;
  std::function<int()> work;
};

namespace {
struct JobPool {
  std::mutex mu;
  std::condition_variable cv;
  std::deque<mpcx_job_t> q;
  std::vector<std::thread> th;
  void start(size_t n) {
    while (th.size() < n)
      th.emplace_back([this] {
        for (;;) {
          mpcx_job_t j;
          {
            std::unique_lock<std::mutex> lk(mu);
            cv.wait(lk, [&] { return !q.empty(); });
            j = q.front();
            q.pop_front();
          }
          const int rc = j->work();
          std::lock_guard<std::mutex> lk(j->mu);
          j->rc = rc;
          if (rc) j->msg = g_err;
          j->done = true;
          j->cv.notify_all();
        }
      });
  }
};
JobPool& job_pool() {
  static JobPool* p = new JobPool();
  return *p;
}
}

extern "C" {

int mpcx_modexp_batch_device(mpcx_mod_t mod, uint32_t count, const uint32_t* d_bases, uint32_t base_words,
                             const uint32_t* d_exps, uint32_t exp_words, int exp_shared, uint32_t exp_bits,
                             uint32_t* d_out, uint32_t out_words, void* stream) {
  if (!mod) return fail(MPCX_EINVAL, "null modulus");
  Device* dev = nullptr;
  if (int rc = selected(&dev)) return rc;
  Lane& l = stream_lane(*dev, (hipStream_t)stream);
  std::lock_guard<std::mutex> lk(l.mu);
  const bool ops_fit = 32u * base_words <= (uint32_t)MPCX_GEOM_RBITS(g_main_geom[mod->cls]);
  return modexp_enqueue((int)(dev - g_devs), l, mod, count, d_bases, base_words, d_exps, exp_words, exp_shared,
                        exp_bits, nullptr, 0, d_out, out_words, ops_fit);
}

int mpcx_modexp_mul_batch_device(mpcx_mod_t mod, uint32_t count, const uint32_t* d_bases, uint32_t base_words,
                                 const uint32_t* d_exps, uint32_t exp_words, int exp_shared, uint32_t exp_bits,
                                 const uint32_t* d_muls, uint32_t mul_words, uint32_t* d_out, uint32_t out_words,
                                 void* stream) {
  if (!mod) return fail(MPCX_EINVAL, "null modulus");
  if (!d_muls) return fail(MPCX_EINVAL, "null multipliers");
  Device* dev = nullptr;
  if (int rc = selected(&dev)) return rc;
  Lane& l = stream_lane(*dev, (hipStream_t)stream);
  std::lock_guard<std::mutex> lk(l.mu);
  const uint32_t rb = (uint32_t)MPCX_GEOM_RBITS(g_main_geom[mod->cls]);
  const bool ops_fit = 32u * base_words <= rb && 32u * mul_words <= rb;
  return modexp_enqueue((int)(dev - g_devs), l, mod, count, d_bases, base_words, d_exps, exp_words, exp_shared,
                        exp_bits, d_muls, mul_words, d_out, out_words, ops_fit);
}

int mpcx_modexp_batch(mpcx_mod_t mod, uint32_t count, const uint32_t* bases, uint32_t base_words,
                      const uint32_t* exps, uint32_t exp_words, int exp_shared, uint32_t* out,
                      uint32_t out_words) {
  return modexp_host(mod, count, bases, base_words, exps, exp_words, exp_shared, nullptr, 0, out, out_words);
}

int mpcx_modexp_mul_batch(mpcx_mod_t mod, uint32_t count, const uint32_t* bases, uint32_t base_words,
                          const uint32_t* exps, uint32_t exp_words, int exp_shared, const uint32_t* muls,
                          uint32_t mul_words, uint32_t* out, uint32_t out_words) {
  if (!muls) return fail(MPCX_EINVAL, "null multipliers");
  return modexp_host(mod, count, bases, base_words, exps, exp_words, exp_shared, muls, mul_words, out, out_words);
}

int mpcx_modexp_submit(mpcx_mod_t mod, uint32_t count, const uint32_t* bases, uint32_t base_words,
                       const uint32_t* exps, uint32_t exp_words, int exp_shared, const uint32_t* muls,
                       uint32_t mul_words, uint32_t* out, uint32_t out_words, mpcx_job_t* job) {
  if (!job) return fail(MPCX_EINVAL, "null job");
  *job = nullptr;
  if (!mod) return fail(MPCX_EINVAL, "null modulus");
  const int n = ndev_or_fail();
  if (n < 0) return -n;
  auto* j = new mpcx_job_s();
  j->work = [=] {
    return modexp_host(mod, count, bases, base_words, exps, exp_words, exp_shared, muls, mul_words, out, out_words);
  };
  JobPool& p = job_pool();
  {
    std::lock_guard<std::mutex> lk(p.mu);
    p.start((size_t)n * kMaxLanes);
    p.q.push_back(j);
  }
  p.cv.notify_one();
  *job = j;
  return MPCX_OK;
}

int mpcx_job_test(mpcx_job_t job, int* done) {
  if (!job || !done) return fail(MPCX_EINVAL, "null job");
  std::lock_guard<std::mutex> lk(job->mu);
  *done = job->done ? 1 : 0;
  return MPCX_OK;
}

int mpcx_job_wait(mpcx_job_t job) {
  if (!job) return fail(MPCX_EINVAL, "null job");
  int rc;
  {
    std::unique_lock<std::mutex> lk(job->mu);
    job->cv.wait(lk, [&] { return job->done; });
    rc = job->rc;
    if (rc) g_err = job->msg;
  }
  delete job;
  return rc;
}

int mpcx_mulmod_batch(mpcx_mod_t mod, uint32_t count, const uint32_t* a, uint32_t a_words, const uint32_t* b,
                      uint32_t b_words, uint32_t* out, uint32_t out_words) {
  if (!a || !b) return fail(MPCX_EINVAL, "null operands");
  const uint32_t one = 1;
  return modexp_host(mod, count, a, a_words, &one, 1, 1, b, b_words, out, out_words);
}

int mpcx_modexp_multi_batch(uint32_t n_groups, const mpcx_modexp_group_t* gs) {
  if (n_groups == 0) return MPCX_OK;
  if (!gs) return fail(MPCX_EINVAL, "null groups");
  const int n = ndev_or_fail();
  if (n < 0) return -n;
  int cls = -1, rc;
  uint64_t total = 0;
  uint32_t min_seg = 0xFFFFFFFFu;
  for (uint32_t i = 0; i < n_groups; ++i) {
    const mpcx_modexp_group_t& g = gs[i];
    if (!g.mod) return fail(MPCX_EINVAL, "group %u: null modulus", i);
    if (cls < 0) cls = g.mod->cls;
    if (g.mod->cls != cls) return fail(MPCX_EINVAL, "group %u: modulus class differs from group 0's", i);
    if (g.count == 0) continue;
    char pre[24];
    std::snprintf(pre, sizeof pre, "group %u: ", i);
    if ((rc = check_batch(pre, g.mod, g.count, g.bases, g.base_words, g.exps, g.exp_words, g.muls, g.mul_words, g.out,
                          g.out_words)))
      return rc;
    total += g.count;
    min_seg = std::min(min_seg, g.count);
  }
  if (total == 0) return MPCX_OK;
  if (total > 0xFFFFFFFFull) return fail(MPCX_EINVAL, "too many operands");
  const int di = (int)(g_dev_rr.fetch_add(1, std::memory_order_relaxed) % (unsigned)n);
  Device& dev = g_devs[di];
  if ((rc = bind(dev))) return rc;
  bool main_ok = true, forced_ok = true;
  {
    const int gf = g_force_geom >= 0 && MPCX_GEOM_CLASS(g_force_geom) == cls ? g_force_geom : -1;
    const uint32_t rb = (uint32_t)MPCX_GEOM_RBITS(g_main_geom[cls]);
    for (uint32_t i = 0; i < n_groups && (main_ok || forced_ok); ++i) {
      const mpcx_modexp_group_t& g = gs[i];
      if (g.count == 0) continue;
      const bool fit = host_ops_below(g.bases, g.count, g.base_words, rb) &&
                       host_ops_below(g.muls, g.count, g.mul_words, rb);
      main_ok = main_ok && geom_serves(g_main_geom[cls], g.mod, fit);
      if (gf >= 0) {
        const uint32_t rf = (uint32_t)MPCX_GEOM_RBITS(gf);
        forced_ok = forced_ok && geom_serves(gf, g.mod, host_ops_below(g.bases, g.count, g.base_words, rf) &&
                                                            host_ops_below(g.muls, g.count, g.mul_words, rf));
      }
    }
  }
  const bool mx_ok = runs_on_mx(MPCX_MAIN_GEOM(cls), (uint32_t)total, min_seg, true);
  const int geom = choose_geom(dev, cls, (uint32_t)total, main_ok, forced_ok, mx_ok);
  const uint32_t G = (uint32_t)MPCX_GEOM_G(geom), K = (uint32_t)MPCX_GEOM_K(geom);
  const bool mx = runs_on_mx(geom, (uint32_t)total, min_seg, true);
  struct Seg {
    uint32_t gi, waves, exp_bits;
    size_t in_b, in_e, in_m, out_o, ws, sched;
    bool use_sched;
    double alg;
  };
  std::vector<Seg> segs;
  size_t in_words = 0, out_words = 0, ws_words = 0;
  for (uint32_t i = 0; i < n_groups; ++i) {
    const mpcx_modexp_group_t& g = gs[i];
    if (g.count == 0) continue;
    Seg sg{};
    sg.gi = i;
    sg.waves = (g.count + G - 1) / G;
    sg.exp_bits = max_exp_bits(g.exps, g.exp_words, g.exp_shared, g.count);
    sg.in_b = in_words;
    in_words += (size_t)g.count * g.base_words;
    sg.in_e = in_words;
    in_words += g.exp_shared ? g.exp_words : (size_t)g.count * g.exp_words;
    sg.in_m = in_words;
    if (g.muls) in_words += (size_t)g.count * g.mul_words;
    sg.out_o = out_words;
    out_words += (size_t)g.count * g.out_words;
    sg.ws = ws_words;
    ws_words += (size_t)sg.waves * MPCX_TABLE_ENTRIES * K * 64u;
    sg.use_sched = g.exp_shared && sg.exp_bits > 0 && g_sched_width > 0;
    sg.alg = g.exp_shared || !g.exp_words ? go_macs(g.mod->bits, sg.exp_bits) * g.count
                                          : go_macs_sum(g.mod->bits, g.exps, g.exp_words, g.count);
    segs.push_back(sg);
  }
  for (auto& sg : segs)
    if (sg.use_sched) {
      sg.sched = ws_words;
      ws_words += MPCX_SCHED_WORDS(32u * gs[sg.gi].exp_words);
    }
  const size_t nseg = segs.size();
  const size_t seg_bytes = nseg * sizeof(mpcx::ModexpArgs), first_bytes = (nseg + 1) * sizeof(uint32_t);
  std::unique_lock<std::mutex> lk;
  Lane& l = acquire_lane(dev, lk);
  LaneDrain drain(l);
  if ((rc = lane_stream(l))) return rc;
  if ((rc = ensure_buffer(l.stage[0], std::max<size_t>(in_words * 4, 4))) ||
      (rc = ensure_buffer(l.stage[2], out_words * 4)) || (rc = ensure_buffer(l.stage[3], seg_bytes + first_bytes)) ||
      (rc = ensure_workspace(l, ws_words * 4)))
    return rc;
  const uint32_t* d_in = (const uint32_t*)l.stage[0].ptr;
  uint32_t* d_out = (uint32_t*)l.stage[2].ptr;
  for (const auto& sg : segs) {
    const mpcx_modexp_group_t& g = gs[sg.gi];
    const size_t ne = g.exp_shared ? g.exp_words : (size_t)g.count * g.exp_words;
    if ((rc = h2d(l, (uint32_t*)l.stage[0].ptr + sg.in_b, g.bases, (size_t)g.count * g.base_words * 4)) ||
        (rc = h2d(l, (uint32_t*)l.stage[0].ptr + sg.in_e, g.exps, ne * 4)) ||
        (g.muls && (rc = h2d(l, (uint32_t*)l.stage[0].ptr + sg.in_m, g.muls, (size_t)g.count * g.mul_words * 4))))
      return rc;
  }
  std::vector<mpcx::ModexpArgs> args(nseg);
  std::vector<uint32_t> first(nseg + 1, 0);
  for (size_t k = 0; k < nseg; ++k) {
    const Seg& sg = segs[k];
    const mpcx_modexp_group_t& g = gs[sg.gi];
    const uint32_t* dconst = nullptr;
    const uint8_t* mx_img = nullptr;
    if ((rc = mod_const(g.mod, di, &dconst)) || (mx && (rc = mx_const(g.mod, di, &mx_img)))) return rc;
    uint32_t* sched = sg.use_sched ? l.ws + sg.sched : nullptr;
// ... 808 lines not shown
```

### mpcium_amd/csrc/mpcx_device.hpp

```cpp
#pragma once
#include <hip/hip_runtime.h>
#include <stdint.h>

#include <type_traits>

#include "mpcx_internal.h"

#if defined(MX_EMIT) || defined(MX_ITER_FENCE) || defined(MX_SPLIT_MAD) || defined(MX_READ_FENCE) ||          \
    defined(MX_PRIO) || defined(MX_PRIO_P) || defined(MX_PRIO_F) || defined(MX_PRIO_R) || defined(MX_PRIO_R2) || \
    defined(MX_PRIO_C) || defined(MX_CARRY_SKIP) || defined(MPCX_SCHED_BARRIER) || defined(MPCX_SQR_OPT) ||      \
    defined(MPCX_PREFETCH_B) || defined(MPCX_SQR_B2) || defined(MPCX_PRIME2C_DBL_FOLD)
#error "retired A/B switch; see DESIGN.md 5.2g"
#endif

#ifndef MPCX_PREFETCH2_KMAX
#define MPCX_PREFETCH2_KMAX 24
#endif
#ifndef MPCX_BLOCK_FENCE
#define MPCX_BLOCK_FENCE 0
#endif
#ifndef MPCX_WAVES_PER_EU_PRIME2C
#define MPCX_WAVES_PER_EU_PRIME2C 3
#endif
#ifndef MPCX_WAVES_PER_EU_MRC
// ... 170 lines not shown
  constexpr int L = P * K;
  canonicalize<P, K>(A);
  bool eq = true;
#pragma unroll
  for (int k = 0; k < K; ++k) eq &= (A[k] == Nd[k]);
  const uint64_t bal = __ballot(eq || idle);
  const uint64_t gmask = (P == 64 ? ~0ull : (((1ull << P) - 1ull) << (g_raw * P)));
  if (!idle && (bal & gmask) == gmask) {
#pragma unroll
    for (int k = 0; k < K; ++k) A[k] = 0;
  }
  wave_lds_fence();
  lds_store_digits<K>(bl, p, A);
  wave_lds_fence();
  if (active) {
    for (uint32_t w = (uint32_t)p; w < out_words; w += P) {
      const uint32_t bit = w * 32u;
      const uint32_t d0 = bit / DB, s0 = bit % DB;
      uint32_t v = 0;
      if (d0 < (uint32_t)L) {
        const uint64_t lo = bl[d0];
        const uint64_t hi = (d0 + 1 < (uint32_t)L) ? bl[d0 + 1] : 0u;
        v = (uint32_t)((lo | (hi << DB)) >> s0);
      }
      o[w] = v;
    }
  }
}

}
#include "mpcx_mx.hpp"
namespace mpcx {

template <int P, int K, int G, bool MX = false>
__device__ __forceinline__ void modexp_wave(const ModexpArgs& a, const uint32_t blk) {
  constexpr int L = P * K;
  using S = MxShape<P, K, G>;
  static_assert(!MX || (P == 4 && K == 37 && G == 16) || (P == 2 && K == 37 && G == 32),
                "montmul_mx serves geometries 2 and 5");
  __shared__ __attribute__((aligned(16))) uint32_t lds_all[MX ? S::LDS_WORDS_WG : (G + 1) * L + 2];
  uint32_t* lds = lds_all;
  if constexpr (MX) {
    const uint32_t* img = static_cast<const uint32_t*>(a.mx_img);
    for (int i = (int)threadIdx.x; i < S::IMG_BYTES / 4; i += 64 * MX_WG) lds_all[i] = img[i];
    for (int i = (int)threadIdx.x; i < L; i += 64 * MX_WG) lds_all[S::IMG_BYTES / 4 + i] = a.nd[i];
    __syncthreads();
    if (blk >= a.nwaves) return;
    lds = lds_all + S::IMG_BYTES / 4 + L + 4 + (threadIdx.x >> 6) * S::WAVE_WORDS;
  }
  const int lane = MX ? (int)(threadIdx.x & 63u) : (int)threadIdx.x;
  const int g_raw = lane / P;
  const bool idle = g_raw >= G;
  const int g = idle ? G : g_raw;
  const int p = lane - g_raw * P;
  const uint32_t op = blk * G + (idle ? 0 : g_raw);
  const bool active = !idle && op < a.count;
  uint32_t* bl = lds + g * (MX ? S::ROW : L);
  const int m_src_addr = (idle ? lane : g_raw * P) * 4;

  uint32_t Nd[K], A[K];
  auto load_const = [&] __attribute__((always_inline))(const uint32_t* src, uint32_t (&v)[K]) {
    if constexpr (MX) asm volatile("" : "+s"(src));
    int pp = p;
    if constexpr (MX) asm volatile("" : "+v"(pp));
#pragma unroll
    for (int k = 0; k < K; ++k) v[k] = idle ? 0u : src[pp * K + k];
  };
  auto load_nd = [&] __attribute__((always_inline))() { load_const(a.nd, Nd); };
  if constexpr (!MX) load_nd();
  MxConsts mxc{};
  const uint32_t* mx_md = lds_all + S::IMG_BYTES / 4;
  if constexpr (MX) mxc = mx_consts<S>(reinterpret_cast<const uint8_t*>(lds_all), lane);

  auto load_digits = [&] __attribute__((always_inline))(const uint32_t* src, uint32_t words) {
    asm volatile("" : "+s"(src));
    int pp = p;
    asm volatile("" : "+v"(pp));
#pragma unroll
    for (int k = 0; k < K; ++k) {
      const uint32_t bit = (uint32_t)(pp * K + k) * DB;
      const uint32_t w = bit >> 5, sh = bit & 31u;
      uint64_t v = 0;
      if (active) {
        const uint32_t* x = src + (size_t)op * words;
        const uint32_t lo = w < words ? x[w] : 0u;
        const uint32_t hi = (w + 1) < words ? x[w + 1] : 0u;
        v = ((uint64_t)hi << 32) | lo;
      }
      A[k] = (uint32_t)(v >> sh) & M28;
    }
  };

  const uint32_t wb = a.win_bits;
  const uint32_t nw = (a.exp_bits + wb - 1u) / wb;
  const uint32_t* ex = a.exp_shared ? a.exps : a.exps + (size_t)(active ? op : 0) * a.exp_words;
  uint32_t* tbl = a.table + (size_t)blk * MPCX_TABLE_ENTRIES * K * 64u;
  const auto tbl_rsrc =
      __builtin_amdgcn_make_buffer_rsrc(tbl, (short)0, (int)(MPCX_TABLE_ENTRIES * K * 64u * 4u), 0x00020000);
  const int tbl_lane_off = lane * 4;
  auto tbl_store = [&](uint32_t e, const uint32_t (&v)[K]) __attribute__((always_inline)) {
    const int voff = tbl_lane_off + (int)(e * K * 256u);
#pragma unroll
    for (int k = 0; k < K; ++k) __builtin_amdgcn_raw_buffer_store_b32(v[k], tbl_rsrc, voff, k * 256, 0);
  };
  auto tbl_load = [&](uint32_t e, uint32_t (&v)[K]) __attribute__((always_inline)) {
    const int voff = tbl_lane_off + (int)(e * K * 256u);
#pragma unroll
    for (int k = 0; k < K; ++k) v[k] = __builtin_amdgcn_raw_buffer_load_b32(tbl_rsrc, voff, k * 256, 0);
  };
  auto lds_from_table = [&] __attribute__((always_inline))(uint32_t e) {
    uint32_t tv[K];
    tbl_load(e, tv);
    lds_store_digits<K>(bl, p, tv);
  };
  auto lds_one = [&] __attribute__((always_inline))() {
    uint32_t one[K];
#pragma unroll
    for (int k = 0; k < K; ++k) one[k] = (p == 0 && k == 0 && !idle) ? 1u : 0u;
    lds_store_digits<K>(bl, p, one);
  };

  {
    uint32_t r1[K];
#pragma unroll
    for (int k = 0; k < K; ++k) r1[k] = idle ? 0u : a.r1d[p * K + k];
    tbl_store(0, r1);
  }
  {
    uint32_t r2[K];
#pragma unroll
    for (int k = 0; k < K; ++k) r2[k] = idle ? 0u : a.r2d[p * K + k];
    lds_store_digits<K>(bl, p, r2);
  }
  const bool has_mul = a.mul != nullptr;
  const bool sched = a.exp_shared != 0 && a.sched != nullptr &&
                     __builtin_amdgcn_readfirstlane(a.sched[MPCX_SCHED_TOP]) != MPCX_SCHED_NONE;
  const uint32_t wt = nw > 0 ? window_of(ex, nw - 1u, wb, a.exp_words) : 0u;
  const uint32_t wt_u = __builtin_amdgcn_readfirstlane(wt);
  const uint32_t T = sched ? __builtin_amdgcn_readfirstlane(a.sched[MPCX_SCHED_TN])
                           : (a.exp_shared && nw <= 1u ? (wt_u > 1u ? wt_u : 1u) : (1u << wb) - 1u);
  const uint32_t nsteps = sched ? __builtin_amdgcn_readfirstlane(a.sched[MPCX_SCHED_N]) : (nw > 0 ? nw - 1u : 0u);

  enum { ST_PRE, ST_TAB, ST_TSQ, ST_STAB, ST_EXP, ST_MULF, ST_FIN };
  int st;
  uint32_t idx = 1;
  bool sqr = false;
  if (has_mul) {
    load_digits(a.mul, a.mul_words);
    st = ST_PRE;
  } else {
    load_digits(a.base, a.base_words);
    st = ST_TAB;
  }
  wave_lds_fence();

  uint32_t sq_left = 0;
  int pend = -1;
  auto prepare_exp = [&] __attribute__((always_inline))() {
    for (;;) {
      if (sq_left) {
        --sq_left;
        lds_store_sqr<K>(bl, p, A);
        sqr = true;
        return;
      }
      if (pend >= 0) {
        lds_from_table(pend == 0x100 ? window_of(ex, nw - 1u - idx, wb, a.exp_words) : (uint32_t)pend);
        pend = -1;
        return;
      }
      if (idx == nsteps) {
        if (has_mul) {
          st = ST_MULF;
          lds_from_table(MPCX_MUL_ENTRY);
        } else {
          st = ST_FIN;
          lds_one();
        }
        return;
      }
      if (sched) {
        const uint32_t s = __builtin_amdgcn_readfirstlane(a.sched[MPCX_SCHED_STEPS + idx]);
        sq_left = s >> 8;
        pend = (s & 0xFFu) == 0xFFu ? -1 : (int)(s & 0xFFu);
      } else {
        sq_left = wb;
        pend = 0x100;
      }
      ++idx;
    }
  };

  int restage = -1;
  constexpr int MX_RESTAGE_R2 = -2;
  for (;;) {
    if constexpr (MX) {
      if (restage != -1) {
        if (restage == MX_RESTAGE_R2) {
          uint32_t r2[K];
          load_const(a.r2d, r2);
          lds_store_digits<K>(bl, p, r2);
        } else {
          lds_from_table((uint32_t)restage);
        }
        restage = -1;
        wave_lds_fence();
      }
      if (st == ST_FIN) break;
      if (sqr) {
        montmul_mx<S, true, true>(A, lds, mx_md, mxc, lane);
      } else {
        montmul_mx<S, false, false>(A, lds, mx_md, mxc, lane);
      }
    } else if (sqr) {
      montmul<P, K, true, true>(A, bl, Nd, a.n0inv, m_src_addr, p);
    } else {
      montmul<P, K, false>(A, bl, Nd, a.n0inv, m_src_addr, p);
    }
    sqr = false;
    wave_lds_fence();
    bool start_exp = false, run_exp = false;
    if (st == ST_PRE) {
      tbl_store(MPCX_MUL_ENTRY, A);
      load_digits(a.base, a.base_words);
      if constexpr (MX) restage = MX_RESTAGE_R2;
      st = ST_TAB;
      idx = 1;
    } else if (st == ST_TAB) {
      tbl_store(sched ? 0u : idx, A);
      if (sched && T > 0u) {
        lds_store_sqr<K>(bl, p, A);
        sqr = true;
        st = ST_TSQ;
      } else if (!sched && idx == 1) {
        lds_store_digits<K>(bl, p, A);
      } else if (MX && !sched && idx < T) {
        restage = 1;
      }
      if (!sched && idx < T) {
        ++idx;
      } else if (st == ST_TAB) {
        start_exp = true;
      }
    } else if (st == ST_TSQ) {
      lds_store_digits<K>(bl, p, A);
      if constexpr (MX) tbl_store(MPCX_SQ_ENTRY, A);
      tbl_load(0, A);
      st = ST_STAB;
      idx = 1;
    } else if (st == ST_STAB) {
      tbl_store(idx, A);
      if (MX && idx < T) restage = MPCX_SQ_ENTRY;
      if (idx < T) {
        ++idx;
      } else {
        start_exp = true;
      }
    } else if (st == ST_EXP) {
      run_exp = true;
    } else if (st == ST_MULF) {
      st = ST_FIN;
      lds_one();
    } else {
      break;
    }
    if (start_exp) {
      tbl_load(sched ? __builtin_amdgcn_readfirstlane(a.sched[MPCX_SCHED_TOP]) : wt, A);
      st = ST_EXP;
      idx = 0;
      run_exp = true;
    }
    if (run_exp) prepare_exp();
    wave_lds_fence();
  }

  if constexpr (MX) {
    load_nd();
    montmul<P, K, false>(A, bl, Nd, a.n0inv, m_src_addr, p);
  }
  store_result<P, K>(A, Nd, bl, p, g_raw, idle, active, a.out + (size_t)op * a.out_words, a.out_words);
}

template <int P, int K, int G, int WPE>
__global__ __launch_bounds__(64) __attribute__((amdgpu_waves_per_eu(WPE))) void k_modexp(const ModexpArgs a) {
  modexp_wave<P, K, G>(a, blockIdx.x);
}

template <int P, int K, int G, int WPE>
__global__ __launch_bounds__(64 * MX_WG) __attribute__((amdgpu_waves_per_eu(WPE))) void k_modexp_multi_mx(
    const ModexpArgs* __restrict__ segs, const uint32_t* __restrict__ first, uint32_t nsegs) {
  const uint32_t b = blockIdx.x;
  uint32_t s = 0;
  while (s + 1u < nsegs && __builtin_amdgcn_readfirstlane(first[s + 1u]) <= b) ++s;
  s = __builtin_amdgcn_readfirstlane(s);
  modexp_wave<P, K, G, true>(segs[s], (b - __builtin_amdgcn_readfirstlane(first[s])) * MX_WG + (threadIdx.x >> 6));
}

template <int P, int K, int G, int WPE>
__global__ __launch_bounds__(64 * MX_WG) __attribute__((amdgpu_waves_per_eu(WPE))) void k_modexp_mx(
    const ModexpArgs a) {
  modexp_wave<P, K, G, true>(a, blockIdx.x * MX_WG + (threadIdx.x >> 6));
}

template <int P, int K, int G, int WPE>
__global__ __launch_bounds__(64) __attribute__((amdgpu_waves_per_eu(WPE))) void k_modexp_multi(
    const ModexpArgs* __restrict__ segs, const uint32_t* __restrict__ first, uint32_t nsegs) {
  const uint32_t b = blockIdx.x;
  uint32_t s = 0;
  while (s + 1u < nsegs && __builtin_amdgcn_readfirstlane(first[s + 1u]) <= b) ++s;
  s = __builtin_amdgcn_readfirstlane(s);
  modexp_wave<P, K, G>(segs[s], b - __builtin_amdgcn_readfirstlane(first[s]));
}

template <int P, int K, int G>
constexpr uint32_t fb_lds_slice_words() {
  return (uint32_t)((G + 1) * P * K + 2);
}

template <int P, int K, int G>
__device__ __forceinline__ void fixedbase_wave(const FixedBaseArgs& a, const uint32_t blk) {
  constexpr int L = P * K;
  constexpr uint32_t kSlice = fb_lds_slice_words<P, K, G>();
  extern __shared__ uint32_t fb_lds[];
  const uint32_t S = __builtin_amdgcn_readfirstlane(blockDim.x >> 6);
  const uint32_t wv = __builtin_amdgcn_readfirstlane(threadIdx.x >> 6);
  const int lane = __builtin_amdgcn_mbcnt_hi(~0u, __builtin_amdgcn_mbcnt_lo(~0u, 0u));
  const int g_raw = lane / P;
  const bool idle = g_raw >= G;
  const int g = idle ? G : g_raw;
  const int p = lane - g_raw * P;
  const uint32_t op = blk * G + (idle ? 0 : g_raw);
  const bool active = !idle && op < a.count;
  uint32_t* bl = fb_lds + wv * kSlice + g * L;
  const int m_src_addr = (idle ? lane : g_raw * P) * 4;

  uint32_t Nd[K], A[K];
#pragma unroll
  for (int k = 0; k < K; ++k) Nd[k] = idle ? 0u : a.nd[p * K + k];
  auto lds_digits = [&](const uint32_t* src) __attribute__((always_inline)) {
    uint32_t t[K];
#pragma unroll
    for (int k = 0; k < K; ++k) t[k] = idle ? 0u : src[p * K + k];
    lds_store_digits<K>(bl, p, t);
  };
  uint32_t t = 0, j = wv;
  uint32_t part = 1;
  bool own = true, fin = false;
  auto fetch = [&] __attribute__((always_inline))() -> bool {
    for (; t < a.nbases; ++t, j = wv) {
      const uint32_t ew = a.exp_words[t], wb = a.wbits[t];
      const uint32_t* ex = a.exps[t] + (size_t)(active ? op : 0) * ew;
      for (; j < a.nwin[t]; j += S) {
        const uint32_t v = (active && ew) ? window_of(ex, j, wb, ew) : 0u;
        if (__ballot(v != 0u) == 0ull) continue;
        const uint32_t* e = a.tables[t] + (((size_t)j << wb) + v) * L;
        uint32_t nx[K];
#pragma unroll
        for (int k = 0; k < K; ++k) nx[k] = idle ? 0u : e[k * P + p];
        lds_store_digits<K>(bl, p, nx);
        j += S;
        return true;
      }
    }
    if (own) {
      own = false;
      if (S > 1u) {
        if (wv) lds_store_digits<K>(bl, p, A);
        __syncthreads();
        if (wv) return false;
      }
    }
    if (part < S) {
      const uint32_t* src = fb_lds + part * kSlice + g * L;
      uint32_t nx[K];
#pragma unroll
      for (int k = 0; k < K; ++k) nx[k] = src[p * K + k];
      lds_store_digits<K>(bl, p, nx);
      ++part;
      return true;
    }
    if (fin) return false;
    fin = true;
    uint32_t one[K];
#pragma unroll
    for (int k = 0; k < K; ++k) one[k] = (p == 0 && k == 0 && !idle) ? 1u : 0u;
    lds_store_digits<K>(bl, p, one);
    return true;
  };

  bool more = true;
  if (a.mul && wv == 0u) {
    lds_digits(a.r2d);
#pragma unroll
    for (int k = 0; k < K; ++k) {
      const uint32_t bit = (uint32_t)(p * K + k) * DB;
      const uint32_t w = bit >> 5, sh = bit & 31u;
      uint64_t v = 0;
      if (active) {
        const uint32_t* x = a.mul + (size_t)op * a.mul_words;
        const uint32_t lo = w < a.mul_words ? x[w] : 0u;
        const uint32_t hi = (w + 1) < a.mul_words ? x[w + 1] : 0u;
        v = ((uint64_t)hi << 32) | lo;
      }
      A[k] = (uint32_t)(v >> sh) & M28;
    }
  } else {
#pragma unroll
    for (int k = 0; k < K; ++k) A[k] = idle ? 0u : a.r1d[p * K + k];
    more = fetch();
  }
  while (more) {
    wave_lds_fence();
    montmul<P, K, false>(A, bl, Nd, a.n0inv, m_src_addr, p);
    wave_lds_fence();
    more = fetch();
  }
  if (wv == 0u)
    store_result<P, K>(A, Nd, bl, p, g_raw, idle, active, a.out + (size_t)op * a.out_words, a.out_words);
}

template <int P, int K, int G, int WPE>
__global__ __launch_bounds__(64 * MPCX_FB_MAX_SPLIT) __attribute__((amdgpu_waves_per_eu(WPE))) void k_fixedbase(
    const FixedBaseArgs a) {
  fixedbase_wave<P, K, G>(a, blockIdx.x);
}

template <int P, int K, int G, int WPE>
__global__ __launch_bounds__(64 * MPCX_FB_MAX_SPLIT) __attribute__((amdgpu_waves_per_eu(WPE))) void k_fixedbase_multi(
    const FixedBaseArgs* __restrict__ segs, const uint32_t* __restrict__ first, uint32_t nsegs) {
  const uint32_t b = blockIdx.x;
  uint32_t s = 0;
  while (s + 1u < nsegs && __builtin_amdgcn_readfirstlane(first[s + 1u]) <= b) ++s;
  s = __builtin_amdgcn_readfirstlane(s);
  fixedbase_wave<P, K, G>(segs[s], b - __builtin_amdgcn_readfirstlane(first[s]));
}

template <int K>
__device__ __forceinline__ bool ge_digits(const uint32_t (&x)[K], const uint32_t (&y)[K]) {
  int r = 0;
#pragma unroll
  for (int k = K - 1; k >= 0; --k) {
    const int c = (x[k] > y[k]) - (x[k] < y[k]);
    r = r != 0 ? r : c;
  }
  return r >= 0;
}
template <int K>
__device__ __forceinline__ void sub_digits(uint32_t (&x)[K], const uint32_t (&y)[K]) {
  uint32_t br = 0;
#pragma unroll
  for (int k = 0; k < K; ++k) {
    const uint32_t t = x[k] - y[k] - br;
    br = (t >> 31) & 1u;
    x[k] = t & M28;
  }
}
template <int K>
__device__ __forceinline__ void norm_serial(uint32_t (&x)[K]) {
  uint32_t c = 0;
#pragma unroll
  for (int k = 0; k < K; ++k) {
    const uint32_t t = x[k] + c;
    x[k] = t & M28;
    c = t >> DB;
  }
}
template <int K>
__device__ __forceinline__ void add_digits(uint32_t (&x)[K], const uint32_t (&y)[K]) {
#pragma unroll
  for (int k = 0; k < K; ++k) x[k] += y[k];
  norm_serial<K>(x);
}
template <int K>
__device__ __forceinline__ void load_candidate(const uint32_t* w, uint32_t words, uint32_t (&Nd)[K]) {
#pragma unroll
  for (int k = 0; k < K; ++k) {
    const uint32_t bit = (uint32_t)k * DB, wi = bit >> 5, sh = bit & 31u;
    const uint64_t v = ((uint64_t)((wi + 1) < words ? w[wi + 1] : 0u) << 32) | (wi < words ? w[wi] : 0u);
    Nd[k] = (uint32_t)(v >> sh) & M28;
  }
}
__device__ __forceinline__ uint32_t neg_inv28(uint32_t n0) {
  uint32_t inv = n0;
  for (int i = 0; i < 5; ++i) inv *= 2u - n0 * inv;
  return (0u - inv) & M28;
}
template <int K>
__device__ __forceinline__ int bitlen_digits(const uint32_t (&Nd)[K]) {
  int nbits = 1;
#pragma unroll
  for (int k = 0; k < K; ++k)
    if (Nd[k] != 0u) nbits = k * DB + (32 - __builtin_clz(Nd[k]));
  return nbits;
}
template <int K>
__device__ __forceinline__ void r_mod(const uint32_t (&Nd)[K], int nbits, uint32_t (&A)[K]) {
  uint32_t c = 1;
#pragma unroll
  for (int k = 0; k < K; ++k) {
    const int lo = k * DB;
    uint32_t maskk = 0;
    if (nbits >= lo + DB) maskk = M28;
    else if (nbits > lo) maskk = (1u << (nbits - lo)) - 1u;
    const uint32_t t = ((~Nd[k]) & maskk) + c;
    c = t >> DB;
    A[k] = t & maskk;
  }
  for (int i = nbits; i < DB * K; ++i) {
#pragma unroll
    for (int k = 0; k < K; ++k) A[k] <<= 1;
    norm_serial<K>(A);
    if (ge_digits<K>(A, Nd)) sub_digits<K>(A, Nd);
  }
}
__device__ __forceinline__ uint32_t word_bit(const uint32_t* w, int j) { return (w[j >> 5] >> (j & 31)) & 1u; }


template <int L>
__device__ __forceinline__ void pprep_item(const uint32_t* nw, uint32_t n_words, uint32_t* r1_out, uint32_t* meta_out) {
  uint32_t Nd[L], R1[L];
  load_candidate<L>(nw, n_words, Nd);
  const int nbits = bitlen_digits<L>(Nd);
  r_mod<L>(Nd, nbits, R1);
  int s = 1;
  while (s < nbits && !word_bit(nw, s)) ++s;
#pragma unroll
  for (int d = 0; d < L; ++d) r1_out[d] = R1[d];
  meta_out[0] = neg_inv28(Nd[0]);
  meta_out[1] = (uint32_t)nbits | ((uint32_t)s << 16);
}

template <int L>
__global__ __launch_bounds__(64) void k_pprep_prime2(const Prime2Args a) {
  const bool strong = blockIdx.x >= a.fp_blocks;
  uint32_t cnt, i;
  const uint32_t* src;
  size_t base;
  if (!strong) {
    cnt = a.count_dev ? min(a.count_f, *a.count_dev) : a.count_f;
    i = blockIdx.x * 64u + threadIdx.x;
    src = a.nf;
    base = 0;
  } else {
    cnt = a.count_s;
    i = (blockIdx.x - a.fp_blocks) * 64u + threadIdx.x;
    src = a.ns;
    base = a.count_f;
  }
  if (i >= cnt) return;
  pprep_item<L>(src + (size_t)i * a.n_words, a.n_words, a.r1 + (base + i) * L, a.meta + (base + i) * 2);
}

template <int L>
__global__ __launch_bounds__(64) void k_pprep_mr(const MrArgs a) {
  const uint32_t i = blockIdx.x * 64u + threadIdx.x;
  if (i >= a.count) return;
  pprep_item<L>(a.n + (size_t)i * a.n_words, a.n_words, a.r1 + (size_t)i * L, a.meta + (size_t)i * 2);
}

template <int K>
__device__ __forceinline__ void load_group_digits(const uint32_t* w, uint32_t words, int p, uint32_t (&D)[K]) {
#pragma unroll
  for (int k = 0; k < K; ++k) {
    const uint32_t bit = (uint32_t)(p * K + k) * DB, wi = bit >> 5, sh = bit & 31u;
    const uint64_t v = ((uint64_t)((wi + 1) < words ? w[wi + 1] : 0u) << 32) | (wi < words ? w[wi] : 0u);
    D[k] = (uint32_t)(v >> sh) & M28;
  }
}

__device__ __forceinline__ int wave_max(int v) {
#pragma unroll
  for (int off = 32; off > 0; off >>= 1) v = max(v, __shfl_xor(v, off));
  return v;
}

template <int P>
__device__ __forceinline__ bool group_all(bool v, int g) {
  const uint64_t bal = __ballot(v);
  const uint64_t gmask = (P == 64 ? ~0ull : (((1ull << P) - 1ull) << (g * P)));
  return (bal & gmask) == gmask;
}

template <int P, int K>
__device__ __forceinline__ void exit_compare(const uint32_t (&X)[K], const uint32_t (&Nd)[K], uint32_t n0inv,
                                             uint32_t* bl, int p, int g, bool* is_one, bool* is_nm1) {
  uint32_t Y[K], one[K];
#pragma unroll
  for (int k = 0; k < K; ++k) {
    Y[k] = X[k];
    one[k] = (p == 0 && k == 0) ? 1u : 0u;
  }
  wave_lds_fence();
  lds_store_digits<K>(bl, p, one);
  wave_lds_fence();
  montmul<P, K, false>(Y, bl, Nd, n0inv, 0, p);
  wave_lds_fence();
  canonicalize<P, K>(Y);
  bool e1 = true, em = true;
#pragma unroll
  for (int k = 0; k < K; ++k) {
    const bool d0 = p == 0 && k == 0;
    e1 &= Y[k] == (d0 ? 1u : 0u);
    em &= Y[k] == (d0 ? Nd[0] - 1u : Nd[k]);
  }
  *is_one = group_all<P>(e1, g);
  *is_nm1 = group_all<P>(em, g);
// ... 404 lines not shown
```

### mpcium_amd/csrc/mpcx_geom.hip

```cpp
#include "mpcx_device.hpp"

#ifndef MPCX_GEOM_ID
#error "compile with -DMPCX_GEOM_ID=<geometry id>"
#endif

#ifndef MPCX_WPE
#if MPCX_GEOM_ID == 0
#define MPCX_WPE 2
#elif MPCX_GEOM_ID == 1
#define MPCX_WPE 3
#elif MPCX_GEOM_ID == 2
#define MPCX_WPE 2
#elif MPCX_GEOM_ID == 3 || MPCX_GEOM_ID == 4
#define MPCX_WPE 8
#elif MPCX_GEOM_ID == 5
#define MPCX_WPE 2
#else
#define MPCX_WPE 3
#endif
#endif

#if MPCX_GEOM_ID == 1
#ifndef MPCX_WPE_MULTI_G1
#define MPCX_WPE_MULTI_G1 4
#endif
#define MPCX_WPE_MULTI MPCX_WPE_MULTI_G1
#endif
#ifndef MPCX_WPE_MULTI
#define MPCX_WPE_MULTI MPCX_WPE
#endif
#if MPCX_GEOM_ID == 1 && defined(MPCX_WPE_SINGLE_G1)
#define MPCX_WPE_SINGLE MPCX_WPE_SINGLE_G1
#endif
#ifndef MPCX_WPE_SINGLE
#define MPCX_WPE_SINGLE MPCX_WPE
#endif

#define MPCX_CAT2(a, b) a##b
#define MPCX_CAT(a, b) MPCX_CAT2(a, b)
#define MPCX_THIS_KERNEL \
  mpcx::k_modexp<MPCX_GEOM_P(MPCX_GEOM_ID), MPCX_GEOM_K(MPCX_GEOM_ID), MPCX_GEOM_G(MPCX_GEOM_ID), MPCX_WPE_SINGLE>

extern "C" {

__attribute__((visibility("hidden"))) hipError_t MPCX_CAT(mpcx_launch_modexp_g, MPCX_GEOM_ID)(
    const mpcx::ModexpArgs* a, uint32_t waves, hipStream_t st) {
#if MPCX_GEOM_ID == 2 || MPCX_GEOM_ID == 5
  if (a->mx_img) {
    hipLaunchKernelGGL((mpcx::k_modexp_mx<MPCX_GEOM_P(MPCX_GEOM_ID), MPCX_GEOM_K(MPCX_GEOM_ID),
                                          MPCX_GEOM_G(MPCX_GEOM_ID), MPCX_WPE_SINGLE>),
                       dim3((waves + MX_WG - 1) / MX_WG), dim3(64 * MX_WG), 0, st, *a);
    return hipGetLastError();
  }
#endif
  hipLaunchKernelGGL((MPCX_THIS_KERNEL), dim3(waves), dim3(64), 0, st, *a);
  return hipGetLastError();
}

__attribute__((visibility("hidden"))) hipError_t MPCX_CAT(mpcx_launch_modexp_multi_g, MPCX_GEOM_ID)(
    const mpcx::ModexpArgs* segs, const uint32_t* first, uint32_t nsegs, uint32_t waves, int mx, hipStream_t st) {
#if MPCX_GEOM_ID == 2
  if (mx) {
    hipLaunchKernelGGL((mpcx::k_modexp_multi_mx<MPCX_GEOM_P(MPCX_GEOM_ID), MPCX_GEOM_K(MPCX_GEOM_ID),
                                                MPCX_GEOM_G(MPCX_GEOM_ID), MPCX_WPE_SINGLE>),
                       dim3(waves), dim3(64 * MX_WG), 0, st, segs, first, nsegs);
    return hipGetLastError();
  }
#else
  if (mx) return hipErrorInvalidValue;
#endif
  hipLaunchKernelGGL((mpcx::k_modexp_multi<MPCX_GEOM_P(MPCX_GEOM_ID), MPCX_GEOM_K(MPCX_GEOM_ID),
                                           MPCX_GEOM_G(MPCX_GEOM_ID), MPCX_WPE_MULTI>),
                     dim3(waves), dim3(64), 0, st, segs, first, nsegs);
  return hipGetLastError();
}

#if MPCX_GEOM_ID == MPCX_FULL_GEOM(0) || MPCX_GEOM_ID == MPCX_FULL_GEOM(1)
#define MPCX_FB_ARGS MPCX_GEOM_P(MPCX_GEOM_ID), MPCX_GEOM_K(MPCX_GEOM_ID), MPCX_GEOM_G(MPCX_GEOM_ID)
__attribute__((visibility("hidden"))) hipError_t MPCX_CAT(mpcx_launch_fixedbase_g, MPCX_GEOM_ID)(
    const mpcx::FixedBaseArgs* a, uint32_t blocks, uint32_t split, hipStream_t st) {
  const size_t lds = (size_t)mpcx::fb_lds_slice_words<MPCX_FB_ARGS>() * 4u * split;
  hipLaunchKernelGGL((mpcx::k_fixedbase<MPCX_FB_ARGS, MPCX_WPE>), dim3(blocks), dim3(64 * split), lds, st, *a);
  return hipGetLastError();
}

__attribute__((visibility("hidden"))) hipError_t MPCX_CAT(mpcx_launch_fixedbase_multi_g, MPCX_GEOM_ID)(
    const mpcx::FixedBaseArgs* segs, const uint32_t* first, uint32_t nsegs, uint32_t blocks, uint32_t split,
    hipStream_t st) {
  const size_t lds = (size_t)mpcx::fb_lds_slice_words<MPCX_FB_ARGS>() * 4u * split;
  hipLaunchKernelGGL((mpcx::k_fixedbase_multi<MPCX_FB_ARGS, MPCX_WPE>), dim3(blocks), dim3(64 * split), lds, st,
                     segs, first, nsegs);
  return hipGetLastError();
}
#undef MPCX_FB_ARGS
#endif

__attribute__((visibility("hidden"))) hipError_t MPCX_CAT(mpcx_modexp_occupancy_g, MPCX_GEOM_ID)(int* blocks_per_cu) {
  return hipOccupancyMaxActiveBlocksPerMultiprocessor(blocks_per_cu, MPCX_THIS_KERNEL, 64, 0);
}

}
```

### mpcium_amd/csrc/mpcx_internal.h

```cpp
#ifndef MPCX_INTERNAL_H_
#define MPCX_INTERNAL_H_

#include <stdint.h>

#define MPCX_NUM_CLASSES 3
#define MPCX_CLASS_LMIN(c) ((c) == 0 ? 37 : (c) == 1 ? 75 : 147)
#define MPCX_CLASS_WORDS(c) ((28 * MPCX_CLASS_LMIN(c)) / 32)
#define MPCX_CLASS_MAXBITS(c) (32 * MPCX_CLASS_WORDS(c))

#define MPCX_NUM_GEOMS 7
#define MPCX_GEOM_P(g) \
  ((g) == 0 ? 1 : (g) == 1 ? 4 : (g) == 2 ? 4 : (g) == 3 ? 16 : (g) == 4 ? 32 : (g) == 5 ? 2 : 8)
#define MPCX_GEOM_K(g) \
  ((g) == 0 ? 37 : (g) == 1 ? 19 : (g) == 2 ? 37 : (g) == 3 ? 5 : (g) == 4 ? 5 : (g) == 5 ? 37 : 19)
#define MPCX_GEOM_G(g) \
  ((g) == 0 ? 64 : (g) == 1 ? 16 : (g) == 2 ? 16 : (g) == 3 ? 4 : (g) == 4 ? 2 : (g) == 5 ? 32 : 8)
#define MPCX_GEOM_CLASS(g) ((g) == 0 ? 0 : ((g) == 1 || (g) == 3 || (g) == 5) ? 1 : 2)
#define MPCX_GEOM_L(g) (MPCX_GEOM_P(g) * MPCX_GEOM_K(g))
#define MPCX_GEOM_RBITS(g) (28 * MPCX_GEOM_L(g))
#define MPCX_MAIN_GEOM(c) ((c) == 0 ? 0 : (c) == 1 ? 5 : 2)
#define MPCX_NARROW_GEOM(c) ((c) == 1 ? 3 : (c) == 2 ? 4 : -1)
#define MPCX_MID_GEOM(c) ((c) == 2 ? 6 : -1)
#define MPCX_FULL_GEOM(c) ((c) == 0 ? 0 : (c) == 1 ? 1 : 2)

#define MPCX_TABLE_ENTRIES 34
#define MPCX_MUL_ENTRY 32
#define MPCX_SQ_ENTRY 33

#define MPCX_SCHED_TOP 0
#define MPCX_SCHED_TN 1
#define MPCX_SCHED_N 2
#define MPCX_SCHED_WIDTH 3
#define MPCX_SCHED_STEPS 4
#define MPCX_SCHED_NONE 0xFFFFFFFFu
#define MPCX_SCHED_MAX_WIDTH 6
#define MPCX_SCHED_WORDS(bits) (MPCX_SCHED_STEPS + (bits) + 1)

namespace mpcx {

struct ModexpArgs {
  const uint32_t* nd;
  const uint32_t* r1d;
  const uint32_t* r2d;
  const uint32_t* base;
  const uint32_t* exps;
  const uint32_t* mul;
  uint32_t* out;
  uint32_t* table;
  uint32_t count;
  uint32_t base_words;
  uint32_t exp_words;
  uint32_t mul_words;
  uint32_t exp_bits;
  uint32_t win_bits;
  uint32_t out_words;
  uint32_t n0inv;
  int exp_shared;
  const uint32_t* sched;
  const void* mx_img;
  uint32_t nwaves;
};
#ifndef MX_WG
#define MX_WG 4
#endif

template <int P_, int K_, int G_>
struct MxShape {
  static constexpr int P = P_, K = K_, G = G_, L = P * K;
  static constexpr int HALVES = G / 16;
  static constexpr int N7 = 4 * L;
  static constexpr int ROW = (((L + 3) / 4) % 2 == 1 ? (L + 3) / 4 : (L + 3) / 4 + 1) * 4;
  static constexpr int KB = (N7 + 63) / 64;
  static constexpr int O1 = (N7 + 15) / 16;
  static constexpr int NJ1 = O1;
  static constexpr int NJ2 = (N7 + 62) / 16 + 1;
  static constexpr int JMAX = (NJ1 > NJ2 ? NJ1 : NJ2) - 1;
  static constexpr int D = 16 * JMAX;
  static constexpr int TAB_STRIDE = (((D + 64) / 16) % 2 == 1 ? (D + 64) / 16 : (D + 64) / 16 + 1) * 16;
  static constexpr int TAB_BYTES = 16 * TAB_STRIDE;
  static constexpr int IMG_BYTES = 2 * TAB_BYTES;
  static constexpr int O2LO = (N7 - 4) / 16;
  static constexpr int O2HI = (2 * N7 + 15) / 16;
#ifndef MX_CS
#define MX_CS 13
#endif
  static constexpr int CS1 = MX_CS, CS2 = MX_CS;
  static constexpr int TRASH_OFF = G * ROW + 4;
  static constexpr int WAVE_WORDS = TRASH_OFF + ((64 + L + 3) / 4) * 4;
  static constexpr int LDS_WORDS_WG = IMG_BYTES / 4 + L + 4 + MX_WG * WAVE_WORDS;
};
using MxG2 = MxShape<4, 37, 16>;
using MxG5 = MxShape<2, 37, 32>;


#define MPCX_FB_WINDOW_BITS 12
#define MPCX_FB_MAX_WINDOW_BITS 12
#define MPCX_FB_MAX_TABLE_BYTES (512ull << 20)
#define MPCX_FB_MAX_SPLIT 4
#ifndef MPCX_FB_MAX_BASES
#define MPCX_FB_MAX_BASES 2
#endif

struct FixedBaseArgs {
  const uint32_t* nd;
  const uint32_t* r1d;
  const uint32_t* r2d;
  const uint32_t* tables[MPCX_FB_MAX_BASES];
  const uint32_t* exps[MPCX_FB_MAX_BASES];
  uint32_t exp_words[MPCX_FB_MAX_BASES];
  uint32_t nwin[MPCX_FB_MAX_BASES];
  uint32_t wbits[MPCX_FB_MAX_BASES];
  uint32_t nbases;
  const uint32_t* mul;
  uint32_t mul_words;
  uint32_t* out;
  uint32_t out_words;
  uint32_t count;
  uint32_t n0inv;
};

struct ExpSchedArgs {
  const uint32_t* exp;
  uint32_t exp_words;
  uint32_t max_width;
  uint32_t* sched;
};


#define MPCX_SIEVE_MAX_BYTES 128
struct SieveArgs {
  const uint8_t* raw;
  uint32_t nbytes, count, q_bits;
  const uint32_t* tprod;
  const uint64_t* tinv;
  const uint32_t* tstart;
  const uint32_t* tprimes;
  uint32_t ngroups;
  uint32_t* out_p;
  uint32_t* out_idx;
  uint32_t* out_count;
};

struct Prime2Args {
  const uint32_t* nf;
  uint32_t count_f;
  const uint32_t* count_dev;
  uint32_t f_blocks;
  uint8_t* ok_f;
  const uint32_t* sieve_idx;
  uint32_t* pass_count;
  uint32_t* pass_idx;
  uint32_t* pass_n;
  const uint32_t* ns;
  uint32_t count_s;
  uint8_t* ok_s;
  uint32_t n_words;
  uint32_t* r1;
  uint32_t* meta;
  uint32_t fp_blocks;
};

#define MPCX_PRIME_P 2
#define MPCX_PRIME_K 19
#define MPCX_PRIME_L (MPCX_PRIME_P * MPCX_PRIME_K)
#define MPCX_MR_P 16
#define MPCX_MR_K 3
#define MPCX_MR_L (MPCX_MR_P * MPCX_MR_K)
#define MPCX_LUCASW_K 5
#define MPCX_LUCASW_L (MPCX_MR_P * MPCX_LUCASW_K)

struct LucasArgs {
  const uint32_t* n;
  const uint32_t* P;
  uint8_t* ok;
  uint32_t count;
  uint32_t n_words;
  uint32_t* consts;
  uint32_t* meta;
};

struct DrbgArgs {
  uint64_t seed;
  uint64_t off;
  uint64_t n;
  uint8_t* out;
};

struct MrArgs {
  const uint32_t* n;
  const uint32_t* a;
  uint8_t* ok;
  uint32_t count;
  uint32_t n_words;
  uint32_t* r1;
  uint32_t* meta;
};

}

#endif
```

### mpcium_amd/csrc/mpcx_mx.hpp

```cpp
#pragma once

namespace mpcx {

typedef int mx_v4i __attribute__((ext_vector_type(4)));


struct MxConsts {
  const uint8_t* t1;
  const uint8_t* t2;
};
template <class S>
__device__ __forceinline__ MxConsts mx_consts(const uint8_t* img, int lane) {
  const int off = (lane & 15) * S::TAB_STRIDE + 16 * (lane >> 4);
  return MxConsts{img + off, img + S::TAB_BYTES + off};
}

__device__ __forceinline__ uint32_t mx_spread7(uint32_t x) {
  x += x & 0xFFFFFF80u;
  x += x & 0xFFFF8000u;
  x += x & 0xFF800000u;
  return x;
}

template <int P, int K, bool SQR, bool B2IN>
__device__ __forceinline__ void mx_product(uint32_t (&A)[K], const uint32_t* bl, uint32_t* tl, uint32_t* tr, int p) {
  static_assert(!SQR || (K % 2) == 1, "squaring schedule needs an odd digit count per lane");
  uint64_t acc[K];
#pragma unroll
  for (int k = 0; k < K; ++k) acc[k] = 0;
  uint32_t bnext = bl[0];
#pragma nounroll
  for (int o = 0; o < P; ++o) {
    const uint32_t* bo = bl + o * K;
    uint32_t* to = (p == 0 ? tl : tr) + o * K;
    const uint32_t dsh = p > o ? 0u : (p == o ? 1u : 31u);
    static_for<0, K>([&](auto uc) {
      constexpr int u = decltype(uc)::value;
      const uint32_t bi = bnext;
      bnext = bo[u + 1];
      const uint32_t b2 = B2IN ? bi : bi << 1;
      const uint32_t bd = b2 >> dsh;
      static_for<0, K>([&](auto kc) {
        constexpr int k = decltype(kc)::value;
        if constexpr (!SQR) {
          mad64(acc[(k + u) % K], A[k], bi);
        } else {
          constexpr int d = ((k - u) % K + K) % K;
          if constexpr (d == 0) {
            mad64(acc[(k + u) % K], A[k], bd);
          } else if constexpr (d <= (K - 1) / 2) {
            mad64(acc[(k + u) % K], A[k], b2);
          }
        }
      });
      const uint64_t a0 = acc[u];
      acc[(u + 1) % K] += a0 >> DB;
      const uint32_t lo = (uint32_t)a0 & M28;
      to[u] = lo;
      acc[u] = from_next_lane(p == 0 ? 0u : lo);
    });
  }
  carry_pass64<P, K>(acc);
  const uint32_t ctop = (uint32_t)(acc[K - 1] >> DB);
#pragma unroll
  for (int k = K - 1; k >= 1; --k) A[k] = ((uint32_t)acc[k] & M28) + (uint32_t)(acc[k - 1] >> DB);
  A[0] = (uint32_t)acc[0] & M28;
  A[0] += from_prev_lane(ctop);
}

__device__ __forceinline__ int mx_from_prev_quarter(int v, int lane) {
  return __builtin_amdgcn_ds_bpermute(((lane - 16) & 63) << 2, v);
}

__device__ __forceinline__ int64_t mx_sum64(const mx_v4i c, int add) {
  int64_t v = (int64_t)(c[0] + add);
  uint64_t cy;
  asm("v_mad_i64_i32 %0, %1, %2, %3, %0" : "+v"(v), "=s"(cy) : "v"(c[1]), "s"(1 << 7));
  asm("v_mad_i64_i32 %0, %1, %2, %3, %0" : "+v"(v), "=s"(cy) : "v"(c[2]), "s"(1 << 14));
  asm("v_mad_i64_i32 %0, %1, %2, %3, %0" : "+v"(v), "=s"(cy) : "v"(c[3]), "s"(1 << 21));
  return v;
}
__device__ __forceinline__ int mx_hi28(int64_t v) {
  return (int)__builtin_amdgcn_alignbit((uint32_t)((uint64_t)v >> 32), (uint32_t)v, 28);
}

template <class S, int NJ, int O0, int O1>
__device__ __forceinline__ void mx_toeplitz(mx_v4i (&acc)[O1 - O0], const uint8_t* f, const mx_v4i (&bf)[S::KB]) {
  auto ld = [&](int j) __attribute__((always_inline)) {
    return *reinterpret_cast<const mx_v4i*>(f + 16 * (S::JMAX - j));
  };
  static_for<0, O1 - O0>([&](auto oc) { acc[decltype(oc)::value] = mx_v4i{0, 0, 0, 0}; });
  constexpr int JLO = (O0 - 4 * (S::KB - 1)) > 0 ? (O0 - 4 * (S::KB - 1)) : 0;
  constexpr int JHI = (O1 - 1) < (NJ - 1) ? (O1 - 1) : (NJ - 1);
  mx_v4i fnext = ld(JLO);
  static_for<JLO, JHI + 1>([&](auto jc) {
    constexpr int j = decltype(jc)::value;
    const mx_v4i fj = fnext;
    if constexpr (j + 1 <= JHI) fnext = ld(j + 1);
    __builtin_amdgcn_sched_barrier(0x000F);
    static_for<0, S::KB>([&](auto kc) {
      constexpr int kb = decltype(kc)::value;
      constexpr int o = j + 4 * kb;
      if constexpr (o >= O0 && o < O1) acc[o - O0] = __builtin_amdgcn_mfma_i32_16x16x64_i8(fj, bf[kb], acc[o - O0], 0, 0, 0);
    });
  });
}

__device__ __forceinline__ mx_v4i mx_transpose4(uint32_t x0, uint32_t x1, uint32_t x2, uint32_t x3) {
  auto r02 = __builtin_amdgcn_permlane32_swap(x0, x2, false, false);
  auto r13 = __builtin_amdgcn_permlane32_swap(x1, x3, false, false);
  auto r01 = __builtin_amdgcn_permlane16_swap(r02[0], r13[0], false, false);
  auto r23 = __builtin_amdgcn_permlane16_swap(r02[1], r13[1], false, false);
  return mx_v4i{(int)r01[0], (int)r01[1], (int)r23[0], (int)r23[1]};
}

#ifdef MX_PROF
struct MxProf {
  uint64_t t[7];
  uint64_t last;
};
#define MX_STAMP(i)                                          \
  do {                                                       \
    __builtin_amdgcn_sched_barrier(0);                       \
    const uint64_t now_ = __builtin_amdgcn_s_memtime();      \
    if ((i) > 0) pf->t[(i) - 1] += now_ - pf->last;          \
    pf->last = now_;                                         \
    __builtin_amdgcn_sched_barrier(0);                       \
  } while (0)
#define MX_PROF_ARG , MxProf* pf
#else
#define MX_STAMP(i) \
  do {              \
  } while (0)
#define MX_PROF_ARG
#endif
template <class S, bool SQR, bool B2IN>
__device__ __forceinline__ void montmul_mx(uint32_t (&A)[S::K], uint32_t* rows, const uint32_t* md,
                                           const MxConsts& c, int lane MX_PROF_ARG) {
  constexpr int P = S::P, K = S::K, L = S::L, ROW = S::ROW, KB = S::KB;
  const int g = lane / P, p = lane % P;
  const int n = lane & 15, h = lane >> 4;
  uint32_t* rg = rows + g * ROW;
#ifndef MPCX_MX_TIMING
#define MPCX_MX_TIMING 0
#endif
  constexpr int PRIO_PRODUCT = 3;
  constexpr int PRIO_FRAG = 2;
  constexpr int PRIO_Q = 1;
  constexpr int PRIO_QM = 0;
  constexpr int PRIO_CARRY = 0;
  MX_STAMP(0);
  __builtin_amdgcn_s_setprio(PRIO_PRODUCT);
  if constexpr (MPCX_MX_TIMING != 2) mx_product<P, K, SQR, B2IN>(A, rg, rg, rows + S::TRASH_OFF + lane, p);
  __builtin_amdgcn_s_setprio(PRIO_FRAG);
  MX_STAMP(1);
  if constexpr (MPCX_MX_TIMING == 1) return;
  wave_lds_fence();
  mx_v4i bf[S::HALVES][KB];
  int ttop[S::HALVES];
  static_for<0, S::HALVES>([&](auto sc) {
    constexpr int s = decltype(sc)::value;
    const uint32_t* rn = rows + (16 * s + n) * ROW;
    static_for<0, KB>([&](auto kc) {
      constexpr int kb = decltype(kc)::value;
      mx_v4i v = {0, 0, 0, 0};
      if (16 * kb + 4 * h < L) v = *reinterpret_cast<const mx_v4i*>(rn + 16 * kb + 4 * h);
      if constexpr (16 * kb + 15 >= L) {
#pragma unroll
        for (int i = 0; i < 4; ++i)
          if (16 * kb + 4 * h + i >= L) v[i] = 0;
      }
#pragma unroll
      for (int i = 0; i < 4; ++i) v[i] = (int)mx_spread7((uint32_t)v[i]);
      bf[s][kb] = v;
    });
    ttop[s] = (int)rn[L - 1];
  });
  wave_lds_fence();
  MX_STAMP(2);
#pragma unroll
  for (int k = 0; k < K; ++k) rg[p * K + k] = A[k] + md[p * K + k];
  __builtin_amdgcn_s_setprio(PRIO_Q);
  static_for<0, S::HALVES>([&](auto sc) {
    constexpr int s = decltype(sc)::value;
    uint32_t* rn = rows + (16 * s + n) * ROW;
    if constexpr (s > 0) __builtin_amdgcn_s_setprio(PRIO_Q);
    mx_v4i qf[KB];
    {
      int xprev = 0;
      uint32_t X[4] = {0u, 0u, 0u, 0u};
      auto norm = [&](const mx_v4i& cs, int o) __attribute__((always_inline)) -> uint32_t {
        const int64_t v = mx_sum64(cs, 1 << 27);
        const int lo = ((int)(uint32_t)v & (int)M28) - (1 << 27);
        const int hi = mx_hi28(v);
        const int x = mx_from_prev_quarter(hi, lane);
        int e = lo + (h == 0 ? xprev : x);
        xprev = x;
        if (4 * o + 3 >= L && 4 * o + h >= L) e = 0;
        return mx_spread7((uint32_t)e);
      };
      auto norm_block = [&](const mx_v4i& cs, auto oc) __attribute__((always_inline)) {
        constexpr int o = decltype(oc)::value;
        X[o & 3] = norm(cs, o);
        if constexpr ((o & 3) == 3) {
          qf[o >> 2] = mx_transpose4(X[0], X[1], X[2], X[3]);
        } else if constexpr (o == S::O1 - 1) {
          qf[o >> 2] = mx_transpose4(X[0], (o & 3) >= 1 ? X[1] : 0u, (o & 3) >= 2 ? X[2] : 0u, 0u);
        }
      };
      constexpr int NC = (S::O1 + S::CS1 - 1) / S::CS1;
      static_for<0, NC>([&](auto cc) {
        constexpr int O0 = S::CS1 * decltype(cc)::value;
        constexpr int O1 = O0 + S::CS1 < S::O1 ? O0 + S::CS1 : S::O1;
        mx_v4i acc[O1 - O0];
        mx_toeplitz<S, S::NJ1, O0, O1>(acc, c.t1, bf[s]);
        static_for<0, O1 - O0>([&](auto oc) {
          norm_block(acc[decltype(oc)::value], std::integral_constant<int, O0 + decltype(oc)::value>{});
        });
        __builtin_amdgcn_sched_barrier(0);
      });
    }
    MX_STAMP(3);
    __builtin_amdgcn_s_setprio(PRIO_QM);
    {
      int xprev = 0;
      auto emit = [&](const mx_v4i& cs, int o) __attribute__((always_inline)) {
        const int pos = 16 * o + 4 * h;
        const bool carry_lane = pos == S::N7 - 4;
        const int d = (pos - S::N7) >> 2;
        const int dc = d < 0 ? 0 : d;
        const int add = carry_lane ? ttop[s] + (1 << 27) : (int)rn[dc];
        const int64_t v = mx_sum64(cs, add);
        const int hi = mx_hi28(v);
        const int top = (int)(uint32_t)v;
        const int dig = top & (int)M28;
        const int x = mx_from_prev_quarter(hi, lane);
        const int cin = h == 0 ? xprev : x;
        xprev = x;
        const int u = d == L - 1 ? top + cin : dig + cin;
        if (d >= 0) rn[dc] = (uint32_t)u;
      };
      constexpr int NC = (S::O2HI - S::O2LO + S::CS2 - 1) / S::CS2;
      static_for<0, NC>([&](auto cc) {
        constexpr int O0 = S::O2LO + S::CS2 * decltype(cc)::value;
        constexpr int O1 = O0 + S::CS2 < S::O2HI ? O0 + S::CS2 : S::O2HI;
        mx_v4i acc[O1 - O0];
        mx_toeplitz<S, S::NJ2, O0, O1>(acc, c.t2, qf);
        static_for<0, O1 - O0>([&](auto oc) { emit(acc[decltype(oc)::value], O0 + decltype(oc)::value); });
        __builtin_amdgcn_sched_barrier(0);
      });
    }
  });
  __builtin_amdgcn_s_setprio(PRIO_CARRY);
  MX_STAMP(4);
  wave_lds_fence();
#pragma unroll
  for (int k = 0; k < K; ++k) A[k] = rg[p * K + k];
  MX_STAMP(5);
  uint32_t sg = 0;
#pragma unroll
  for (int k = 0; k < K; ++k) sg |= A[k];
  const bool need = __any((int)sg < 0);
  for (int it = 0; need && it < L + 2; ++it) {
    const int top = (int)A[K - 1];
    const int ctop = (p == P - 1) ? 0 : (top >> DB);
#pragma unroll
    for (int k = K - 1; k >= 1; --k) {
      const int cur = (int)A[k];
      const bool keep = (k == K - 1) && (p == P - 1);
      A[k] = (uint32_t)((keep ? cur : (cur & (int)M28)) + ((int)A[k - 1] >> DB));
    }
    const int c0 = (int)from_prev_lane((uint32_t)ctop);
    A[0] = (uint32_t)(((int)A[0] & (int)M28) + (p == 0 ? 0 : c0));
    bool neg = false;
#pragma unroll
    for (int k = 0; k < K; ++k) neg |= (int)A[k] < 0;
    if (!__any(neg)) break;
  }
  MX_STAMP(6);
}

}
```

### mpcium_amd/mpcx.py

```python
from __future__ import annotations

import ctypes
import os
from typing import Iterable, List, Optional, Sequence, Union

import numpy as np

_HERE = os.path.dirname(os.path.abspath(__file__))
_LIB_PATH = os.path.join(_HERE, "libmpcx.so")

MPCX_OK, MPCX_EINVAL, MPCX_ENODEV, MPCX_EHIP, MPCX_ENOMEM = 0, 1, 2, 3, 4

_u32p = ctypes.POINTER(ctypes.c_uint32)
_vp = ctypes.c_void_p

SIGNATURES = [
    ("mpcx_version", ctypes.c_int, []),
    ("mpcx_set_option", ctypes.c_int, [ctypes.c_char_p, ctypes.c_int]),
    ("mpcx_get_option", ctypes.c_int, [ctypes.c_char_p, ctypes.POINTER(ctypes.c_int)]),
    ("mpcx_last_error", ctypes.c_char_p, []),
    ("mpcx_device_count", ctypes.c_int, [ctypes.POINTER(ctypes.c_int)]),
    ("mpcx_init", ctypes.c_int, [ctypes.c_int]),
    ("mpcx_init_devices", ctypes.c_int, [ctypes.c_int]),
    ("mpcx_bound_devices", ctypes.c_int, [ctypes.POINTER(ctypes.c_int), ctypes.POINTER(ctypes.c_int), ctypes.c_int]),
    ("mpcx_select_device", ctypes.c_int, [ctypes.c_int]),
    ("mpcx_device_launches", ctypes.c_int, [ctypes.c_int, ctypes.POINTER(ctypes.c_uint64)]),
    ("mpcx_kernel_stats", ctypes.c_int, [ctypes.c_char_p, ctypes.c_size_t, ctypes.c_int]),
    ("mpcx_partition", ctypes.c_int, [ctypes.c_uint32, ctypes.c_int, ctypes.c_uint32, _u32p, _u32p, _u32p]),
    ("mpcx_shutdown", ctypes.c_int, []),
    ("mpcx_modulus_register", ctypes.c_int, [_vp, ctypes.c_uint32, ctypes.POINTER(_vp)]),
    ("mpcx_modulus_release", ctypes.c_int, [_vp]),
    ("mpcx_modulus_info", ctypes.c_int, [_vp, _u32p, _u32p]),
    ("mpcx_modulus_geometry", ctypes.c_int, [_vp, _u32p, _u32p, _u32p, _u32p]),
    ("mpcx_mx_tables", ctypes.c_int, [_u32p, ctypes.c_uint32, ctypes.c_uint32, ctypes.c_void_p, ctypes.c_size_t]),
    ("mpcx_modexp_batch", ctypes.c_int, [_vp, ctypes.c_uint32, _vp, ctypes.c_uint32, _vp, ctypes.c_uint32,
                                         ctypes.c_int, _vp, ctypes.c_uint32]),
    ("mpcx_modexp_batch_device", ctypes.c_int, [_vp, ctypes.c_uint32, _vp, ctypes.c_uint32, _vp, ctypes.c_uint32,
                                                ctypes.c_int, ctypes.c_uint32, _vp, ctypes.c_uint32, _vp]),
    ("mpcx_modexp_mul_batch", ctypes.c_int, [_vp, ctypes.c_uint32, _vp, ctypes.c_uint32, _vp, ctypes.c_uint32,
                                             ctypes.c_int, _vp, ctypes.c_uint32, _vp, ctypes.c_uint32]),
    ("mpcx_modexp_mul_batch_device", ctypes.c_int, [_vp, ctypes.c_uint32, _vp, ctypes.c_uint32, _vp,
                                                    ctypes.c_uint32, ctypes.c_int, ctypes.c_uint32, _vp,
                                                    ctypes.c_uint32, _vp, ctypes.c_uint32, _vp]),
    ("mpcx_modexp_submit", ctypes.c_int, [_vp, ctypes.c_uint32, _vp, ctypes.c_uint32, _vp, ctypes.c_uint32,
                                          ctypes.c_int, _vp, ctypes.c_uint32, _vp, ctypes.c_uint32,
                                          ctypes.POINTER(_vp)]),
    ("mpcx_job_test", ctypes.c_int, [_vp, ctypes.POINTER(ctypes.c_int)]),
    ("mpcx_job_wait", ctypes.c_int, [_vp]),
    ("mpcx_mulmod_batch", ctypes.c_int, [_vp, ctypes.c_uint32, _vp, ctypes.c_uint32, _vp, ctypes.c_uint32, _vp,
                                         ctypes.c_uint32]),
    ("mpcx_fermat2_batch", ctypes.c_int, [ctypes.c_uint32, _vp, ctypes.c_uint32, _vp]),
    ("mpcx_ec_combine_batch", ctypes.c_int, [ctypes.c_uint32, _vp, _vp, _vp]),
    ("mpcx_modexp_multi_batch", ctypes.c_int, [ctypes.c_uint32, _vp]),
    ("mpcx_mr_batch", ctypes.c_int, [ctypes.c_uint32, _vp, ctypes.c_uint32, _vp, _vp]),
    ("mpcx_fixedbase_register", ctypes.c_int, [_vp, _vp, ctypes.c_uint32, ctypes.c_uint32, ctypes.POINTER(_vp)]),
    ("mpcx_fixedbase_release", ctypes.c_int, [_vp]),
    ("mpcx_fixedbase_info", ctypes.c_int, [_vp, _u32p, ctypes.POINTER(ctypes.c_size_t)]),
    ("mpcx_fixedbase_exp_batch", ctypes.c_int, [ctypes.c_uint32, ctypes.POINTER(_vp), ctypes.c_uint32,
                                                ctypes.POINTER(_vp), _u32p, _vp, ctypes.c_uint32, _vp,
                                                ctypes.c_uint32]),
    ("mpcx_fixedbase_multi_batch", ctypes.c_int, [ctypes.c_uint32, _vp]),
    ("mpcx_lucas_batch", ctypes.c_int, [ctypes.c_uint32, _vp, ctypes.c_uint32, _vp, _vp]),
    ("mpcx_safeprime_step", ctypes.c_int, [ctypes.c_uint64, _vp, ctypes.c_uint64, ctypes.c_uint32, ctypes.c_uint32,
                                           _vp, ctypes.c_uint32, ctypes.c_uint32, _u32p, _u32p, _vp, _vp, _vp]),
    ("mpcx_safeprime_sieve_fermat", ctypes.c_int, [_vp, ctypes.c_uint32, ctypes.c_uint32, ctypes.c_uint32, _u32p,
                                                   _vp, _vp]),
    ("mpcx_dev_alloc", ctypes.c_int, [ctypes.c_size_t, ctypes.POINTER(_vp)]),
    ("mpcx_dev_free", ctypes.c_int, [_vp]),
    ("mpcx_host_alloc", ctypes.c_int, [ctypes.c_size_t, ctypes.POINTER(ctypes.c_void_p)]),
    ("mpcx_host_free", ctypes.c_int, [_vp]),
    ("mpcx_copy_stats", ctypes.c_int, [ctypes.POINTER(ctypes.c_uint64), ctypes.POINTER(ctypes.c_uint64),
                                       ctypes.POINTER(ctypes.c_uint64)]),
    ("mpcx_memcpy_h2d", ctypes.c_int, [_vp, _vp, ctypes.c_size_t]),
    ("mpcx_memcpy_d2h", ctypes.c_int, [_vp, _vp, ctypes.c_size_t]),
    ("mpcx_stream_create", ctypes.c_int, [ctypes.POINTER(_vp)]),
    ("mpcx_stream_destroy", ctypes.c_int, [_vp]),
    ("mpcx_stream_sync", ctypes.c_int, [_vp]),
    ("mpcx_sync", ctypes.c_int, [_vp]),
]


class MpcxError(RuntimeError):
    def __init__(self, code: int, msg: str):
        super().__init__(f"mpcx error {code}: {msg}")
        self.code = code


_lib = None


def lib() -> ctypes.CDLL:
    global _lib
    if _lib is None:
        path = os.environ.get("MPCX_LIB_PATH") or _LIB_PATH
        if not os.path.exists(path):
            raise MpcxError(MPCX_ENODEV, f"{path} not built: run `python -m mpcium_amd.build`")
        l = ctypes.CDLL(path)
        for name, res, args in SIGNATURES:
            if path != _LIB_PATH and not hasattr(l, name):
                continue
            f = getattr(l, name)
            f.restype = res
            f.argtypes = args
        _lib = l
    return _lib


def _check(rc: int):
    if rc != MPCX_OK:
        raise MpcxError(rc, lib().mpcx_last_error().decode(errors="replace"))


def device_count() -> int:
    n = ctypes.c_int(0)
    _check(lib().mpcx_device_count(ctypes.byref(n)))
    return n.value


def init(device: int = 0):
    _check(lib().mpcx_init(device))


def init_devices(n_gpus: int = 0):
    _check(lib().mpcx_init_devices(n_gpus))


def bound_devices() -> List[int]:
    n = ctypes.c_int(0)
    ords = (ctypes.c_int * 16)()
    _check(lib().mpcx_bound_devices(ctypes.byref(n), ords, 16))
    return list(ords[:n.value])


def partition(count: int, n_devices: int, min_slice: int = 4096):
    f = (ctypes.c_uint32 * 16)()
    n = (ctypes.c_uint32 * 16)()
    k = ctypes.c_uint32(0)
    _check(lib().mpcx_partition(count, n_devices, min_slice, f, n, ctypes.byref(k)))
    return [(f[i], n[i]) for i in range(k.value)]


def device_launches(index: int) -> int:
    v = ctypes.c_uint64(0)
    _check(lib().mpcx_device_launches(index, ctypes.byref(v)))
    return v.value


def kernel_stats(reset: bool = False) -> dict:
    import json
    buf = ctypes.create_string_buffer(1 << 16)
    _check(lib().mpcx_kernel_stats(buf, len(buf), 1 if reset else 0))
    return json.loads(buf.value.decode())


def copy_stats() -> dict:
    v = [ctypes.c_uint64(0) for _ in range(3)]
    _check(lib().mpcx_copy_stats(*(ctypes.byref(x) for x in v)))
    return {"direct_bytes": v[0].value, "bounced_bytes": v[1].value, "bounce_allocs": v[2].value}


MX_TABLE_BYTES = {148: 2 * 16 * 720, 74: 2 * 16 * 432}


def mx_tables(m: int, L: int = 148) -> bytes:
    w = int_to_words(m, 128)
    n = MX_TABLE_BYTES.get(L, 0)
    out = ctypes.create_string_buffer(max(n, 1))
    _check(lib().mpcx_mx_tables(w.ctypes.data_as(ctypes.POINTER(ctypes.c_uint32)), 128, L, out, n))
    return out.raw


def select_device(index: int):
    _check(lib().mpcx_select_device(index))


def set_option(key: str, value: int):
    _check(lib().mpcx_set_option(key.encode(), int(value)))


def get_option(key: str) -> int:
    v = ctypes.c_int(0)
    _check(lib().mpcx_get_option(key.encode(), ctypes.byref(v)))
    return v.value


def shutdown():
    _check(lib().mpcx_shutdown())


def int_to_words(v: int, n: int) -> np.ndarray:
    if v < 0:
        raise ValueError("negative integers do not cross the C-ABI")
    return np.frombuffer(v.to_bytes(4 * n, "little"), dtype="<u4").copy()


def ints_to_words(vals: Sequence[int], n: int) -> np.ndarray:
    buf = b"".join(int(v).to_bytes(4 * n, "little") for v in vals)
    return np.frombuffer(buf, dtype="<u4").reshape(len(vals), n).copy()


def words_to_ints(arr: np.ndarray) -> List[int]:
    arr = np.ascontiguousarray(arr, dtype="<u4")
    n = arr.shape[1]
    raw = arr.tobytes()
    return [int.from_bytes(raw[i * 4 * n:(i + 1) * 4 * n], "little") for i in range(arr.shape[0])]


def nwords(v: int) -> int:
    return max(1, (v.bit_length() + 31) // 32)


class Modulus:

    def __init__(self, m: int):
        if m <= 0:
            raise ValueError("modulus must be positive")
        self.m = m
        w = int_to_words(m, nwords(m))
        h = _vp()
        _check(lib().mpcx_modulus_register(w.ctypes.data, len(w), ctypes.byref(h)))
        self._h = h
        bits, cw = ctypes.c_uint32(), ctypes.c_uint32()
        _check(lib().mpcx_modulus_info(h, ctypes.byref(bits), ctypes.byref(cw)))
        self.bits, self.class_words = bits.value, cw.value
        g = [ctypes.c_uint32() for _ in range(4)]
        _check(lib().mpcx_modulus_geometry(h, *[ctypes.byref(x) for x in g]))
        self.L, self.P, self.K, self.G = (x.value for x in g)
        self.words = nwords(m)

    @property
    def handle(self):
        return self._h

    def release(self):
        if self._h:
            _check(lib().mpcx_modulus_release(self._h))
            self._h = None

    def exp_words(self, bases: np.ndarray, exps: np.ndarray, shared: bool, out_words: Optional[int] = None) -> np.ndarray:
        bases = np.ascontiguousarray(bases, dtype="<u4")
        exps = np.ascontiguousarray(exps, dtype="<u4")
        count, bw = bases.shape
        ew = exps.shape[-1] if exps.size else 0
        ow = out_words or self.words
        out = np.zeros((count, ow), dtype="<u4")
        _check(lib().mpcx_modexp_batch(self._h, count, bases.ctypes.data, bw,
                                       exps.ctypes.data if exps.size else None, ew, 1 if shared else 0,
                                       out.ctypes.data, ow))
        return out

    def _operands(self, vals: Sequence[int], what: str) -> np.ndarray:
        bw = self.class_words
        lim = 1 << (32 * bw)
        if any(v < 0 or v >= lim for v in vals):
            raise ValueError(f"{what} must be in [0, 2^(32*class_words)); reduce mod m first")
        return ints_to_words(vals, bw)

    def mulmod(self, a: Sequence[int], b: Sequence[int]) -> List[int]:
        if len(a) != len(b):
            raise ValueError("length mismatch")
        if len(a) == 0:
            return []
        A, B = self._operands(a, "a"), self._operands(b, "b")
        out = np.zeros((len(a), self.words), dtype="<u4")
        _check(lib().mpcx_mulmod_batch(self._h, len(a), A.ctypes.data, A.shape[1], B.ctypes.data, B.shape[1],
                                       out.ctypes.data, self.words))
        return words_to_ints(out)

    def exp_mul(self, bases: Sequence[int], exps: Union[int, Sequence[int]], muls: Sequence[int]) -> List[int]:
        if len(muls) != len(bases):
            raise ValueError("one multiplier per base")
        if len(bases) == 0:
            return []
        B = self._operands(bases, "bases")
        Mu = self._operands(muls, "muls")
        E, shared = self._exps(exps, len(bases))
        out = np.zeros((len(bases), self.words), dtype="<u4")
        _check(lib().mpcx_modexp_mul_batch(self._h, len(bases), B.ctypes.data, B.shape[1],
                                           E.ctypes.data if E.size else None, E.shape[-1] if E.size else 0,
                                           1 if shared else 0, Mu.ctypes.data, Mu.shape[1], out.ctypes.data,
                                           self.words))
        return words_to_ints(out)

    @staticmethod
    def _exps(exps, count):
        if isinstance(exps, int):
            if exps < 0:
                raise ValueError("negative exponent")
            return (int_to_words(exps, nwords(exps)) if exps else np.zeros(0, dtype="<u4")), True
        if len(exps) != count:
            raise ValueError("one exponent per base")
        if any(e < 0 for e in exps):
            raise ValueError("negative exponent")
        ew = max(nwords(e) for e in exps)
        return ints_to_words(exps, ew), False

    def submit(self, bases: Sequence[int], exps: Union[int, Sequence[int]]) -> "Job":
        B = self._operands(bases, "bases")
        E, shared = self._exps(exps, len(bases))
        out = np.zeros((len(bases), self.words), dtype="<u4")
        h = _vp()
        _check(lib().mpcx_modexp_submit(self._h, len(bases), B.ctypes.data, B.shape[1],
                                        E.ctypes.data if E.size else None, E.shape[-1] if E.size else 0,
                                        1 if shared else 0, None, 0, out.ctypes.data, self.words, ctypes.byref(h)))
        return Job(h, (B, E, out), lambda: words_to_ints(out))

    def exp(self, bases: Sequence[int], exps: Union[int, Sequence[int]]) -> List[int]:
        if len(bases) == 0:
            return []
        B = self._operands(bases, "bases")
        E, shared = self._exps(exps, len(bases))
        return words_to_ints(self.exp_words(B, E, shared))


class ModexpGroup(ctypes.Structure):
    _fields_ = [("mod", _vp), ("count", ctypes.c_uint32), ("bases", _vp), ("base_words", ctypes.c_uint32),
                ("exps", _vp), ("exp_words", ctypes.c_uint32), ("exp_shared", ctypes.c_int), ("muls", _vp),
                ("mul_words", ctypes.c_uint32), ("out", _vp), ("out_words", ctypes.c_uint32)]


def modexp_multi(groups) -> List[List[int]]:
    keep, outs = [], []
    arr = (ModexpGroup * max(1, len(groups)))()
    for i, (mod, bases, exps, muls) in enumerate(groups):
        B = mod._operands(bases, "bases")
        E, shared = Modulus._exps(exps, len(bases))
        Mu = mod._operands(muls, "muls") if muls is not None else None
        out = np.zeros((len(bases), mod.words), dtype="<u4")
        keep += [B, E, Mu]
        outs.append(out)
        arr[i] = ModexpGroup(mod.handle, len(bases), B.ctypes.data if len(bases) else None, mod.class_words,
                             E.ctypes.data if E.size else None, E.shape[-1] if E.size else 0, 1 if shared else 0,
                             Mu.ctypes.data if Mu is not None else None, mod.class_words if Mu is not None else 0,
                             out.ctypes.data if len(bases) else None, mod.words)
    _check(lib().mpcx_modexp_multi_batch(len(groups), arr))
    return [words_to_ints(o) if o.shape[0] else [] for o in outs]


class Job:

    def __init__(self, h, bufs, result):
        self._h, self._bufs, self._result = h, bufs, result

    def done(self) -> bool:
        d = ctypes.c_int(0)
        _check(lib().mpcx_job_test(self._h, ctypes.byref(d)))
        return bool(d.value)

    def wait(self):
        h, self._h = self._h, None
        if h is None:
            raise RuntimeError("job already waited")
        _check(lib().mpcx_job_wait(h))
        r = self._result()
        self._bufs = None
        return r


class FixedBase:

    def __init__(self, mod: Modulus, base: int, max_exp_bits: int):
        self.mod, self.base = mod, base % mod.m
        w = mod._operands([self.base], "base")
        h = _vp()
        _check(lib().mpcx_fixedbase_register(mod.handle, w.ctypes.data, w.shape[1], max_exp_bits, ctypes.byref(h)))
        self._h = h
        mb, tb = ctypes.c_uint32(), ctypes.c_size_t()
        _check(lib().mpcx_fixedbase_info(h, ctypes.byref(mb), ctypes.byref(tb)))
        self.max_exp_bits, self.table_bytes = mb.value, tb.value

    @property
    def handle(self):
        return self._h

    def release(self):
        if self._h:
            _check(lib().mpcx_fixedbase_release(self._h))
            self._h = None


def fixedbase_exp(fbs: Sequence[FixedBase], exps: Sequence[Sequence[int]],
                  muls: Optional[Sequence[int]] = None) -> List[int]:
    nb = len(fbs)
    if nb != len(exps) or nb == 0:
        raise ValueError("one exponent list per fixed base")
    count = len(exps[0])
    if any(len(e) != count for e in exps):
        raise ValueError("exponent lists differ in length")
    if count == 0:
        return []
    mod = fbs[0].mod
    Es = []
    for e in exps:
        if any(v < 0 for v in e):
            raise ValueError("negative exponent")
        ew = max(nwords(v) for v in e)
        Es.append(ints_to_words(e, ew))
    Mu = mod._operands(muls, "muls") if muls is not None else None
    out = np.zeros((count, mod.words), dtype="<u4")
    hs = (_vp * nb)(*[f.handle for f in fbs])
    eps = (_vp * nb)(*[E.ctypes.data for E in Es])
    ews = (ctypes.c_uint32 * nb)(*[E.shape[1] for E in Es])
    _check(lib().mpcx_fixedbase_exp_batch(nb, hs, count, eps, ews, Mu.ctypes.data if Mu is not None else None,
                                          Mu.shape[1] if Mu is not None else 0, out.ctypes.data, mod.words))
    return words_to_ints(out)


class FixedBaseGroup(ctypes.Structure):
    _fields_ = [("nbases", ctypes.c_uint32), ("fbs", _vp * 2), ("count", ctypes.c_uint32), ("exps", _vp * 2),
                ("exp_words", ctypes.c_uint32 * 2), ("muls", _vp), ("mul_words", ctypes.c_uint32), ("out", _vp),
                ("out_words", ctypes.c_uint32)]


def fixedbase_multi(groups) -> List[List[int]]:
    keep, outs = [], []
    arr = (FixedBaseGroup * max(1, len(groups)))()
    for i, (fbs, exps, muls) in enumerate(groups):
        nb = len(fbs)
        if nb != len(exps) or not 1 <= nb <= 2:
            raise ValueError("one exponent list per fixed base (1 or 2)")
        count = len(exps[0])
        mod = fbs[0].mod
        g = FixedBaseGroup()
        g.nbases, g.count = nb, count
        for t in range(nb):
            E = ints_to_words(exps[t], max([nwords(v) for v in exps[t]] + [1]))
            keep.append(E)
            g.fbs[t] = fbs[t].handle
            g.exps[t] = E.ctypes.data if count else None
            g.exp_words[t] = E.shape[1]
        Mu = mod._operands(muls, "muls") if muls is not None else None
        keep.append(Mu)
        g.muls = Mu.ctypes.data if Mu is not None else None
        g.mul_words = mod.class_words if Mu is not None else 0
        out = np.zeros((count, mod.words), dtype="<u4")
        outs.append(out)
        g.out = out.ctypes.data if count else None
        g.out_words = mod.words
        arr[i] = g
    _check(lib().mpcx_fixedbase_multi_batch(len(groups), arr))
    return [words_to_ints(o) if o.shape[0] else [] for o in outs]


def exp_batch(m: int, bases: Sequence[int], exps: Union[int, Sequence[int]]) -> List[int]:
    mod = Modulus(m)
    try:
        return mod.exp(bases, exps)
    finally:
        mod.release()


SECP_N = 0xFFFFFFFFFFFFFFFFFFFFFFFFFFFFFFFEBAAEDCE6AF48A03BBFD25E8CD0364141


def ec_combine_batch(items) -> list:
    n = len(items)
    if n == 0:
        return []
    sc = np.zeros((n, 24), dtype="<u4")
    pt = np.zeros((n, 32), dtype="<u4")
    mask = (1 << 256) - 1
    for i, (a, b, c, P, Q) in enumerate(items):
        a, b, c = a % SECP_N, b % SECP_N, c % SECP_N
        sc[i] = int_to_words(a | (b << 256) | (c << 512), 24)
        px = (P[0] | (P[1] << 256)) if P is not None else 0
        qx = (Q[0] | (Q[1] << 256)) if Q is not None else 0
        pt[i] = int_to_words(px | (qx << 512), 32)
    out = np.zeros((n, 16), dtype="<u4")
    _check(lib().mpcx_ec_combine_batch(n, sc.ctypes.data, pt.ctypes.data, out.ctypes.data))
    res = []
    for v in words_to_ints(out):
        res.append(None if v == 0 else (v & mask, v >> 256))
# ... 69 lines not shown
```

Measured before the change: 523,000 modexp/s.

## Add N-squared modexp path representing residues as pairs mod N

When the modulus is a perfect square N^2, the host detects it with an exact integer square root and builds constants over N (digits of N, split constants for 2^k mod N^2 written as a + bN, and MX tables for N). A new kernel keeps each operand as a pair (U,V) of 2048-bit halves and does paired Montgomery products and reductions modulo N, sharing the quotient fragments between the two reductions. The aim is to replace full 4096-bit multiplications with several 2048-bit ones. The path adds host-side precomputation and a larger table workspace per wave. It runs only for shared-exponent launches without multipliers on the geom-2 MX kernel.

```diff
diff --git a/include/mpcx.h b/include/mpcx.h
--- a/include/mpcx.h
+++ b/include/mpcx.h
@@ -158,6 +158,8 @@
 
 int mpcx_mx_tables(const uint32_t* m_words, uint32_t m_len, uint32_t L, uint8_t* out, size_t cap);
 
+int mpcx_nsq_consts(const uint32_t* m_words, uint32_t m_len, uint32_t* out, size_t cap_words, int* is_square);
+
 int mpcx_modulus_geometry(mpcx_mod_t mod, uint32_t* L, uint32_t* P, uint32_t* K, uint32_t* G);
 
 #ifdef __cplusplus
diff --git a/mpcium_amd/csrc/mpcx_api.cpp b/mpcium_amd/csrc/mpcx_api.cpp
--- a/mpcium_amd/csrc/mpcx_api.cpp
+++ b/mpcium_amd/csrc/mpcx_api.cpp
@@ -66,6 +66,9 @@
   uint32_t* d_const[kMaxDevices] = {};
   std::vector<uint8_t> mx_host;
   uint8_t* d_mx[kMaxDevices] = {};
+  int nsq_state = 0;
+  std::vector<uint32_t> nsq_host;
+  uint32_t* d_nsq[kMaxDevices] = {};
 };
 
 struct mpcx_fixedbase_s {
@@ -103,6 +106,10 @@
 #define MPCX_MX_DEFAULT 1
 #endif
 int g_mx = MPCX_MX_DEFAULT;
+#ifndef MPCX_NSQ_DEFAULT
+#define MPCX_NSQ_DEFAULT 1
+#endif
+int g_nsq = MPCX_NSQ_DEFAULT;
 uint32_t g_mx_min = 2048;
 uint32_t g_mx_seg_min = 64;
 double g_mx_step = 0.81;
@@ -131,6 +138,7 @@
     int geom;
     uint32_t ops;
     double alg;
+    bool nsq = false;
   };
   std::vector<KEv> kev_free;
   std::vector<KPend> kpend;
@@ -231,6 +239,7 @@
 std::atomic<bool> g_kstats{false};
 struct KAgg {
   uint64_t launches = 0, ops = 0;
+  uint64_t nsq = 0;
   double alg = 0.0, ms = 0.0;
 };
 std::mutex g_kmu;
@@ -269,7 +278,8 @@
   return (int)l.kpend.size() - 1;
 }
 
-void kstat_end(Lane& l, int slot, const Device& d, int dev, const char* kind, int geom, uint32_t ops, double alg) {
+void kstat_end(Lane& l, int slot, const Device& d, int dev, const char* kind, int geom, uint32_t ops, double alg,
+               bool nsq = false) {
   if (slot < 0) return;
   Lane::KPend& p = l.kpend[(size_t)slot];
   if (!d.kref || hipEventRecord(p.ev.b, l.st) != hipSuccess) {
@@ -283,6 +293,7 @@
   p.geom = geom;
   p.ops = ops;
   p.alg = alg;
+  p.nsq = nsq;
 }
 
 void kstat_credit(const char* kind, int geom, uint64_t ops, double alg) {
@@ -301,6 +312,7 @@
         hipEventElapsedTime(&t0, p.ref, p.ev.a) == hipSuccess) {
       KAgg& a = g_kagg[{p.kind, p.geom}];
       a.launches += 1;
+      a.nsq += p.nsq ? 1 : 0;
       a.ops += p.ops;
       a.alg += p.alg;
       a.ms += ms;
@@ -399,6 +411,8 @@
     *o = {mpcx::MxG2::N7, mpcx::MxG2::D, mpcx::MxG2::TAB_STRIDE, mpcx::MxG2::IMG_BYTES};
   } else if (L == mpcx::MxG5::L) {
     *o = {mpcx::MxG5::N7, mpcx::MxG5::D, mpcx::MxG5::TAB_STRIDE, mpcx::MxG5::IMG_BYTES};
+  } else if (L == mpcx::MxN2::L) {
+    *o = {mpcx::MxN2::N7, mpcx::MxN2::D, mpcx::MxN2::TAB_STRIDE, mpcx::MxN2::IMG_BYTES};
   } else {
     return false;
   }
@@ -455,6 +469,94 @@
   };
   fill(n2, out.data());
   fill(n1, out.data() + dm.img / 2);
+}
+
+static void trim(std::vector<uint32_t>& x) {
+  while (x.size() > 1 && x.back() == 0) x.pop_back();
+}
+static std::vector<uint32_t> isqrt_words(const std::vector<uint32_t>& m, bool* exact) {
+  const size_t n = m.size();
+  std::vector<uint32_t> rem(m), res(n, 0), t(n);
+  auto bit_of = [&](uint32_t b) { return std::pair<size_t, uint32_t>(b >> 5, 1u << (b & 31)); };
+  for (int b = (int)((bit_length(m) - 1) & ~1u); b >= 0; b -= 2) {
+    t = res;
+    const auto [wi, msk] = bit_of((uint32_t)b);
+    t[wi] |= msk;
+    bool ge = true;
+    for (int i = (int)n - 1; i >= 0; --i)
+      if (rem[i] != t[i]) {
+        ge = rem[i] > t[i];
+        break;
+      }
+    uint32_t c = 0;
+    for (int i = (int)n - 1; i >= 0; --i) {
+      const uint32_t nc = res[i] & 1u;
+      res[i] = (res[i] >> 1) | (c << 31);
+      c = nc;
+    }
+    if (ge) {
+      uint64_t br = 0;
+      for (size_t i = 0; i < n; ++i) {
+        const uint64_t d = (uint64_t)rem[i] - t[i] - br;
+        rem[i] = (uint32_t)d;
+        br = (d >> 63) & 1;
+      }
+      res[wi] |= msk;
+    }
+  }
+  *exact = true;
+  for (uint32_t w : rem) *exact = *exact && w == 0;
+  trim(res);
+  return res;
+}
+static void divmod_words(const std::vector<uint32_t>& x, const std::vector<uint32_t>& n, std::vector<uint32_t>* q,
+                         std::vector<uint32_t>* r) {
+  const size_t k = n.size();
+  std::vector<uint32_t> rem(k + 1, 0), nn(n);
+  nn.push_back(0);
+  q->assign(x.size(), 0);
+  for (int b = (int)(32 * x.size()) - 1; b >= 0; --b) {
+    uint32_t c = (x[(size_t)b >> 5] >> (b & 31)) & 1u;
+    for (size_t i = 0; i <= k; ++i) {
+      const uint32_t nc = rem[i] >> 31;
+      rem[i] = (rem[i] << 1) | c;
+      c = nc;
+    }
+    if (geq(rem, nn)) {
+      uint64_t br = 0;
+      for (size_t i = 0; i <= k; ++i) {
+        const uint64_t d = (uint64_t)rem[i] - nn[i] - br;
+        rem[i] = (uint32_t)d;
+        br = (d >> 63) & 1;
+      }
+      (*q)[(size_t)b >> 5] |= 1u << (b & 31);
+    }
+  }
+  rem.resize(k);
+  *r = rem;
+}
+static bool nsq_build(const std::vector<uint32_t>& m, std::vector<uint32_t>& out) {
+  constexpr uint32_t L = mpcx::MxN2::L;
+  if ((m[0] & 7u) != 1u) return false;
+  bool exact = false;
+  const std::vector<uint32_t> n = isqrt_words(m, &exact);
+  if (!exact || bit_length(n) > 2048 || bit_length(n) < 1025) return false;
+  out.clear();
+  const auto nd = to_digits(n, L);
+  out.insert(out.end(), nd.begin(), nd.end());
+  for (uint32_t extra : {0u, (uint32_t)MPCX_NSQ_SPLIT_BITS}) {
+    std::vector<uint32_t> c = pow2_mod(2 * kDigitBits * L + extra, m), a, b;
+    divmod_words(c, n, &b, &a);
+    const auto ad = to_digits(a, L), bd = to_digits(b, L);
+    out.insert(out.end(), ad.begin(), ad.end());
+    out.insert(out.end(), bd.begin(), bd.end());
+  }
+  std::vector<uint8_t> img;
+  mx_tables(n, L, img);
+  const size_t at = out.size();
+  out.resize(at + img.size() / 4);
+  std::memcpy(out.data() + at, img.data(), img.size());
+  return true;
 }
 
 hipError_t mpcx_launch_modexp(int geom, const mpcx::ModexpArgs* a, uint32_t waves, hipStream_t st) {
@@ -947,6 +1049,26 @@
     mod->d_mx[di] = p;
   }
   *out = mod->d_mx[di];
+  return MPCX_OK;
+}
+
+int nsq_const(mpcx_mod_t mod, int di, const uint32_t** out) {
+  std::lock_guard<std::mutex> lk(mod->mu);
+  *out = nullptr;
+  if (mod->nsq_state == 0) mod->nsq_state = nsq_build(mod->m, mod->nsq_host) ? 1 : -1;
+  if (mod->nsq_state < 0) return MPCX_OK;
+  if (!mod->d_nsq[di]) {
+    uint32_t* p = nullptr;
+    const size_t bytes = mod->nsq_host.size() * sizeof(uint32_t);
+    hipError_t e = hipMalloc((void**)&p, bytes);
+    if (e != hipSuccess) return fail(MPCX_ENOMEM, "hipMalloc(nsq constants): %s", hipGetErrorString(e));
+    if (int rc = copy_sync(p, mod->nsq_host.data(), bytes, hipMemcpyHostToDevice, nullptr)) {
+      (void)hipFree(p);
+      return rc;
+    }
+    mod->d_nsq[di] = p;
+  }
+  *out = mod->d_nsq[di];
   return MPCX_OK;
 }
 
@@ -1262,6 +1384,8 @@
   std::lock_guard<std::mutex> lk(g_mu);
   if (std::strcmp(key, "mx") == 0) {
     *value = g_mx;
+  } else if (std::strcmp(key, "nsq") == 0) {
+    *value = g_nsq;
   } else if (std::strcmp(key, "mx_min") == 0) {
     *value = (int)g_mx_min;
   } else if (std::strcmp(key, "mx_seg_min") == 0) {
@@ -1307,6 +1431,9 @@
   } else if (std::strcmp(key, "mx") == 0) {
     if (value < 0 || value > 2) return fail(MPCX_EINVAL, "mx %d not 0, 1 or 2", value);
     g_mx = value;
+  } else if (std::strcmp(key, "nsq") == 0) {
+    if (value < 0 || value > 1) return fail(MPCX_EINVAL, "nsq %d not 0 or 1", value);
+    g_nsq = value;
   } else if (std::strcmp(key, "mx_min") == 0) {
     if (value < 1) return fail(MPCX_EINVAL, "mx_min %d < 1", value);
     g_mx_min = (uint32_t)value;
@@ -1366,6 +1493,8 @@
   if (fw) g_fb_window = std::max(4, std::min(MPCX_FB_MAX_WINDOW_BITS, std::atoi(fw)));
   const char* mx = std::getenv("MPCX_MX");
   if (mx) g_mx = std::max(0, std::min(2, std::atoi(mx)));
+  const char* nq = std::getenv("MPCX_NSQ");
+  if (nq) g_nsq = std::max(0, std::min(1, std::atoi(nq)));
   const char* ms = std::getenv("MPCX_MX_STEP");
   if (ms) g_mx_step = std::max(10, std::min(200, std::atoi(ms))) / 100.0;
   const char* gt = std::getenv("MPCX_GEOM_TPUT");
@@ -1442,10 +1571,10 @@
       alg += kv.second.alg;
       std::snprintf(line, sizeof line,
                     "%s{\"kind\":\"%s\",\"geom\":%d,\"launches\":%llu,\"operands\":%llu,\"alg_macs\":%.6e,"
-                    "\"kernel_ms\":%.4f}",
+                    "\"kernel_ms\":%.4f,\"nsq_launches\":%llu}",
                     ks.empty() ? "" : ",", kv.first.first.c_str(), kv.first.second,
                     (unsigned long long)kv.second.launches, (unsigned long long)kv.second.ops, kv.second.alg,
-                    kv.second.ms);
+                    kv.second.ms, (unsigned long long)kv.second.nsq);
       ks += line;
     }
     std::snprintf(line, sizeof line, "{\"enabled\":%d,\"busy_ms\":%.4f,\"alg_macs\":%.6e,\"kernels\":[",
@@ -1552,6 +1681,7 @@
   for (int i = 0; i < n && i < kMaxDevices; ++i) {
     if (mod->d_const[i] && bind(g_devs[i]) == MPCX_OK) (void)hipFree(mod->d_const[i]);
     if (mod->d_mx[i] && bind(g_devs[i]) == MPCX_OK) (void)hipFree(mod->d_mx[i]);
+    if (mod->d_nsq[i] && bind(g_devs[i]) == MPCX_OK) (void)hipFree(mod->d_nsq[i]);
   }
   delete mod;
   return MPCX_OK;
@@ -1560,7 +1690,7 @@
 int mpcx_mx_tables(const uint32_t* m_words, uint32_t m_len, uint32_t L, uint8_t* out, size_t cap) {
   if (!m_words || !out || m_len == 0) return fail(MPCX_EINVAL, "null modulus or output");
   MxDims dm{};
-  if (!mx_dims(L, &dm)) return fail(MPCX_EINVAL, "L %u is not an MX geometry's (148 or 74)", L);
+  if (!mx_dims(L, &dm)) return fail(MPCX_EINVAL, "L %u is not an MX geometry's (148, 76 or 74)", L);
   if (cap < dm.img) return fail(MPCX_EINVAL, "mx tables need %u bytes", dm.img);
   std::vector<uint32_t> m(m_words, m_words + m_len);
   while (m.size() > 1 && m.back() == 0) m.pop_back();
@@ -1569,6 +1699,21 @@
   std::vector<uint8_t> t;
   mx_tables(m, L, t);
   std::memcpy(out, t.data(), dm.img);
+  return MPCX_OK;
+}
+
+int mpcx_nsq_consts(const uint32_t* m_words, uint32_t m_len, uint32_t* out, size_t cap_words, int* is_square) {
+  if (!m_words || !is_square || m_len == 0) return fail(MPCX_EINVAL, "null modulus or output");
+  std::vector<uint32_t> m(m_words, m_words + m_len);
+  while (m.size() > 1 && m.back() == 0) m.pop_back();
+  if ((m[0] & 1u) == 0 || class_for_bits(bit_length(m)) != 2)
+    return fail(MPCX_EINVAL, "nsq constants need an odd modulus of the 4096-bit class");
+  std::vector<uint32_t> c;
+  *is_square = nsq_build(m, c) ? 1 : 0;
+  if (*is_square) {
+    if (!out || cap_words < c.size()) return fail(MPCX_EINVAL, "nsq constants need %zu words", c.size());
+    std::memcpy(out, c.data(), c.size() * sizeof(uint32_t));
+  }
   return MPCX_OK;
 }
 
@@ -1611,24 +1756,31 @@
   const uint32_t G = (uint32_t)MPCX_GEOM_G(geom), K = (uint32_t)MPCX_GEOM_K(geom);
   const uint32_t waves = (count + G - 1) / G;
   const bool use_sched = exp_shared && exp_bits > 0 && g_sched_width > 0;
-  const size_t sched_off = (size_t)waves * MPCX_TABLE_ENTRIES * K * 64u;
+  const bool mx = runs_on_mx(geom, count, count, false);
+  const uint32_t* dnsq = nullptr;
+  if (g_nsq && mx && geom == 2 && use_sched && !d_muls && (rc = nsq_const(mod, di, &dnsq))) return rc;
+  const size_t sched_off = (size_t)waves * MPCX_TABLE_ENTRIES * (dnsq ? (uint32_t)MPCX_NSQ_TABLE_SLOTS : K) * 64u;
   const size_t ws_words = sched_off + (use_sched ? MPCX_SCHED_WORDS(32u * exp_words) : 0);
   if ((rc = ensure_workspace(lane, ws_words * sizeof(uint32_t)))) return rc;
   uint32_t* sched = use_sched ? lane.ws + sched_off : nullptr;
   if (use_sched && (rc = launch_expsched(d_exps, exp_words, sched, lane.st))) return rc;
-  const bool mx = runs_on_mx(geom, count, count, false);
   const uint8_t* mx_img = nullptr;
-  if (mx && (rc = mx_const(mod, di, &mx_img))) return rc;
-  const mpcx::ModexpArgs a =
+  if (dnsq) {
+    mx_img = reinterpret_cast<const uint8_t*>(dnsq + MPCX_NSQ_CONST_DIGITS);
+  } else if (mx && (rc = mx_const(mod, di, &mx_img))) {
+    return rc;
+  }
+  mpcx::ModexpArgs a =
       modexp_args(mod, geom, dconst, count, d_bases, base_words, d_exps, exp_words, d_muls, mul_words, d_out,
                   out_words, lane.ws, exp_bits, exp_shared, sched, mx_img, waves);
+  a.nsq = dnsq;
   const char* kind = mx ? "modexp_mx" : "modexp";
   const int ks = kstat_begin(lane);
   hipError_t e = mpcx_launch_modexp(geom, &a, waves, lane.st);
   if (e != hipSuccess) return hip_fail(e, "launch k_modexp");
   dev.launches.fetch_add(1, std::memory_order_relaxed);
   const double alg = alg_macs >= 0 ? alg_macs : go_macs(mod->bits, a.exp_bits) * count;
-  kstat_end(lane, ks, dev, di, kind, geom, count, alg);
+  kstat_end(lane, ks, dev, di, kind, geom, count, alg, dnsq != nullptr);
   launch_log(kind, geom, count, mod->bits, a.exp_bits, alg);
   return MPCX_OK;
 }
diff --git a/mpcium_amd/csrc/mpcx_device.hpp b/mpcium_amd/csrc/mpcx_device.hpp
--- a/mpcium_amd/csrc/mpcx_device.hpp
+++ b/mpcium_amd/csrc/mpcx_device.hpp
@@ -496,6 +496,257 @@
   modexp_wave<P, K, G, true>(a, blockIdx.x * MX_WG + (threadIdx.x >> 6));
 }
 
+#ifndef MX_PROF
+__device__ __forceinline__ void modexp_nsq_wave(const ModexpArgs& a, const uint32_t blk) {
+  using S = MxN2;
+  constexpr int P = S::P, K = S::K, L = S::L, G = S::G, ROW = S::ROW;
+  constexpr int KT = MPCX_NSQ_TABLE_SLOTS;
+  constexpr int WAVE_WORDS = 2 * G * ROW + 4 + ((64 + L + 3) / 4) * 4;
+  constexpr int WAVES_OFF = S::IMG_BYTES / 4 + L + 4;
+  __shared__ __attribute__((aligned(16))) uint32_t lds_all[WAVES_OFF + MPCX_NSQ_WG * WAVE_WORDS];
+  {
+    const uint32_t* img = static_cast<const uint32_t*>(a.mx_img);
+    for (int i = (int)threadIdx.x; i < S::IMG_BYTES / 4; i += 64 * MPCX_NSQ_WG) lds_all[i] = img[i];
+    for (int i = (int)threadIdx.x; i < L; i += 64 * MPCX_NSQ_WG) lds_all[S::IMG_BYTES / 4 + i] = a.nsq[i];
+    __syncthreads();
+    if (blk >= a.nwaves) return;
+  }
+  const int lane = (int)(threadIdx.x & 63u);
+  const int g = lane / P, p = lane % P;
+  const uint32_t op = blk * G + (uint32_t)g;
+  const bool active = op < a.count;
+  const uint32_t* md = lds_all + S::IMG_BYTES / 4;
+  uint32_t* ra = lds_all + WAVES_OFF + (blk % MPCX_NSQ_WG) * WAVE_WORDS;
+  uint32_t* rb = ra + G * ROW;
+  uint32_t* tr = ra + 2 * G * ROW + 4 + lane;
+  uint32_t* ga = ra + g * ROW;
+  uint32_t* gb = rb + g * ROW;
+  const MxConsts mxc = mx_consts<S>(reinterpret_cast<const uint8_t*>(lds_all), lane);
+  uint32_t* out = a.out + (size_t)op * a.out_words;
+
+  const uint32_t top = __builtin_amdgcn_readfirstlane(a.sched[MPCX_SCHED_TOP]);
+  if (top == MPCX_SCHED_NONE) {
+    if (active)
+      for (uint32_t w = (uint32_t)p; w < a.out_words; w += P) out[w] = w == 0 ? 1u : 0u;
+    return;
+  }
+  const uint32_t T = __builtin_amdgcn_readfirstlane(a.sched[MPCX_SCHED_TN]);
+  const uint32_t nsteps = __builtin_amdgcn_readfirstlane(a.sched[MPCX_SCHED_N]);
+
+  uint32_t U[K], V[K];
+  uint32_t* tbl = a.table + (size_t)blk * MPCX_TABLE_ENTRIES * KT * 64u;
+  const auto tbl_rsrc =
+      __builtin_amdgcn_make_buffer_rsrc(tbl, (short)0, (int)(MPCX_TABLE_ENTRIES * KT * 64u * 4u), 0x00020000);
+  auto tbl_store = [&](uint32_t e) __attribute__((always_inline)) {
+    const int voff = lane * 4 + (int)(e * KT * 256u);
+#pragma unroll
+    for (int k = 0; k < K; ++k) {
+      __builtin_amdgcn_raw_buffer_store_b32(U[k], tbl_rsrc, voff, k * 256, 0);
+      __builtin_amdgcn_raw_buffer_store_b32(V[k], tbl_rsrc, voff, (K + k) * 256, 0);
+    }
+  };
+  auto tbl_load = [&](uint32_t e, uint32_t (&u)[K], uint32_t (&v)[K]) __attribute__((always_inline)) {
+    const int voff = lane * 4 + (int)(e * KT * 256u);
+#pragma unroll
+    for (int k = 0; k < K; ++k) {
+      u[k] = __builtin_amdgcn_raw_buffer_load_b32(tbl_rsrc, voff, k * 256, 0);
+      v[k] = __builtin_amdgcn_raw_buffer_load_b32(tbl_rsrc, voff, (K + k) * 256, 0);
+    }
+  };
+  auto stage_entry = [&](uint32_t e) __attribute__((always_inline)) {
+    uint32_t u[K], v[K];
+    tbl_load(e, u, v);
+    lds_store_digits<K>(ga, p, u);
+    lds_store_digits<K>(gb, p, v);
+  };
+  auto stage_const = [&](const uint32_t* src) __attribute__((always_inline)) {
+    asm volatile("" : "+s"(src));
+    int pp = p;
+    asm volatile("" : "+v"(pp));
+#pragma unroll
+    for (int k = 0; k < K; ++k) {
+      ga[pp * K + k] = src[pp * K + k];
+      gb[pp * K + k] = src[L + pp * K + k];
+    }
+  };
+  auto stage_sqr = [&]() __attribute__((always_inline)) {
+    lds_store_sqr<K>(ga, p, U);
+    lds_store_sqr<K>(gb, p, U);
+  };
+  auto stage_unit = [&](uint32_t* row1, uint32_t* row0) __attribute__((always_inline)) {
+#pragma unroll
+    for (int k = 0; k < K; ++k) {
+      row1[p * K + k] = (p == 0 && k == 0) ? 1u : 0u;
+      row0[p * K + k] = 0u;
+    }
+  };
+  auto load_half = [&](uint32_t d0) __attribute__((always_inline)) {
+    const uint32_t* src = a.base;
+    asm volatile("" : "+s"(src));
+    int pp = p;
+    asm volatile("" : "+v"(pp));
+#pragma unroll
+    for (int k = 0; k < K; ++k) {
+      const uint32_t d = (uint32_t)(pp * K + k);
+      const uint32_t bit = (d0 + d) * DB;
+      const uint32_t w = bit >> 5, sh = bit & 31u;
+      uint64_t v = 0;
+      if (active && d < (uint32_t)MPCX_NSQ_SPLIT_DIGITS) {
+        const uint32_t* x = src + (size_t)op * a.base_words;
+        const uint32_t lo = w < a.base_words ? x[w] : 0u;
+        const uint32_t hi = (w + 1) < a.base_words ? x[w + 1] : 0u;
+        v = ((uint64_t)hi << 32) | lo;
+      }
+      U[k] = (uint32_t)(v >> sh) & M28;
+      V[k] = 0u;
+    }
+  };
+
+  enum { ST_IN0, ST_IN1, ST_TSQ, ST_STAB, ST_EXP, ST_OUT };
+  int st = ST_IN0;
+  uint32_t idx = 1, sq_left = 0;
+  int pend = -1, restage = -1;
+  bool sqr = false;
+  stage_const(a.nsq + L);
+  load_half(0);
+  wave_lds_fence();
+  for (;;) {
+    if (restage != -1) {
+      stage_entry((uint32_t)restage);
+      restage = -1;
+      wave_lds_fence();
+    }
+    if (sqr) {
+      pairmul_mx<S, true>(U, V, ra, rb, tr, md, mxc, lane);
+    } else {
+      pairmul_mx<S, false>(U, V, ra, rb, tr, md, mxc, lane);
+    }
+    sqr = false;
+    wave_lds_fence();
+    bool start_exp = false, run_exp = false;
+    if (st == ST_IN0) {
+      tbl_store(0);
+      stage_const(a.nsq + 3 * L);
+      load_half(MPCX_NSQ_SPLIT_DIGITS);
+      st = ST_IN1;
+    } else if (st == ST_IN1) {
+      uint32_t u0[K], v0[K];
+      tbl_load(0, u0, v0);
+#pragma unroll
+      for (int k = 0; k < K; ++k) {
+        U[k] += u0[k];
+        V[k] += v0[k];
+      }
+      carry_pass32<P, K>(U);
+      carry_pass32<P, K>(V);
+      tbl_store(0);
+      if (T > 0u) {
+        stage_sqr();
+        sqr = true;
+        st = ST_TSQ;
+      } else {
+        start_exp = true;
+      }
+    } else if (st == ST_TSQ) {
+      lds_store_digits<K>(ga, p, U);
+      lds_store_digits<K>(gb, p, V);
+      tbl_store(MPCX_SQ_ENTRY);
+      tbl_load(0, U, V);
+      st = ST_STAB;
+      idx = 1;
+    } else if (st == ST_STAB) {
+      tbl_store(idx);
+      if (idx < T) {
+        restage = MPCX_SQ_ENTRY;
+        ++idx;
+      } else {
+        start_exp = true;
+      }
+    } else if (st == ST_EXP) {
+      run_exp = true;
+    } else {
+      break;
+    }
+    if (start_exp) {
+      tbl_load(top, U, V);
+      st = ST_EXP;
+      idx = 0;
+      run_exp = true;
+    }
+    if (run_exp) {
+      for (;;) {
+        if (sq_left) {
+          --sq_left;
+          stage_sqr();
+          sqr = true;
+          break;
+        }
+        if (pend >= 0) {
+          stage_entry((uint32_t)pend);
+          pend = -1;
+          break;
+        }
+        if (idx == nsteps) {
+          st = ST_OUT;
+          stage_unit(ga, gb);
+          break;
+        }
+        const uint32_t s = __builtin_amdgcn_readfirstlane(a.sched[MPCX_SCHED_STEPS + idx]);
+        sq_left = s >> 8;
+        pend = (s & 0xFFu) == 0xFFu ? -1 : (int)(s & 0xFFu);
+        ++idx;
+      }
+    }
+    wave_lds_fence();
+  }
+
+  stage_unit(gb, ga);
+#pragma unroll
+  for (int k = 0; k < K; ++k) ga[p * K + k] = md[p * K + k];
+  wave_lds_fence();
+  mx_product2<P, K>(U, V, ga, gb, tr, p);
+  canonicalize<P, K>(V);
+  wave_lds_fence();
+  lds_store_digits<K>(ga, p, V);
+  wave_lds_fence();
+  auto digit = [&](uint32_t d) __attribute__((always_inline)) -> uint32_t {
+    return d < (uint32_t)L ? gb[d] : (d < 2u * L ? ga[d - L] : 0u);
+  };
+  if (p == 0) {
+    constexpr uint32_t L2 = (uint32_t)MPCX_GEOM_L(2);
+    int c = 0;
+    for (int d = 2 * L - 1; d >= 0; --d) {
+      const uint32_t x = digit((uint32_t)d), m = (uint32_t)d < L2 ? a.nd[d] : 0u;
+      if (c == 0 && x != m) c = x > m ? 1 : -1;
+    }
+    if (c >= 0) {
+      uint32_t borrow = 0;
+      for (uint32_t d = 0; d < 2u * L; ++d) {
+        const uint32_t m = d < L2 ? a.nd[d] : 0u;
+        const uint32_t t = digit(d) - m - borrow;
+        borrow = t >> 31;
+        (d < (uint32_t)L ? gb[d] : ga[d - L]) = t & M28;
+      }
+    }
+  }
+  wave_lds_fence();
+  if (active) {
+    for (uint32_t w = (uint32_t)p; w < a.out_words; w += P) {
+      const uint32_t bit = w * 32u;
+      const uint32_t d0 = bit / DB, s0 = bit % DB;
+      const uint64_t lo = digit(d0), hi = digit(d0 + 1u);
+      out[w] = (uint32_t)((lo | (hi << DB)) >> s0);
+    }
+  }
+}
+
+template <int WPE>
+__global__ __launch_bounds__(64 * MPCX_NSQ_WG) __attribute__((amdgpu_waves_per_eu(WPE))) void k_modexp_nsq(
+    const ModexpArgs a) {
+  modexp_nsq_wave(a, blockIdx.x * MPCX_NSQ_WG + __builtin_amdgcn_readfirstlane(threadIdx.x >> 6));
+}
+#endif
+
 template <int P, int K, int G, int WPE>
 __global__ __launch_bounds__(64) __attribute__((amdgpu_waves_per_eu(WPE))) void k_modexp_multi(
     const ModexpArgs* __restrict__ segs, const uint32_t* __restrict__ first, uint32_t nsegs) {
diff --git a/mpcium_amd/csrc/mpcx_geom.hip b/mpcium_amd/csrc/mpcx_geom.hip
--- a/mpcium_amd/csrc/mpcx_geom.hip
+++ b/mpcium_amd/csrc/mpcx_geom.hip
@@ -45,6 +45,13 @@
 
 __attribute__((visibility("hidden"))) hipError_t MPCX_CAT(mpcx_launch_modexp_g, MPCX_GEOM_ID)(
     const mpcx::ModexpArgs* a, uint32_t waves, hipStream_t st) {
+#if MPCX_GEOM_ID == 2
+  if (a->nsq) {
+    hipLaunchKernelGGL((mpcx::k_modexp_nsq<MPCX_NSQ_WPE>), dim3((waves + MPCX_NSQ_WG - 1) / MPCX_NSQ_WG),
+                       dim3(64 * MPCX_NSQ_WG), 0, st, *a);
+    return hipGetLastError();
+  }
+#endif
 #if MPCX_GEOM_ID == 2 || MPCX_GEOM_ID == 5
   if (a->mx_img) {
     hipLaunchKernelGGL((mpcx::k_modexp_mx<MPCX_GEOM_P(MPCX_GEOM_ID), MPCX_GEOM_K(MPCX_GEOM_ID),
diff --git a/mpcium_amd/csrc/mpcx_internal.h b/mpcium_amd/csrc/mpcx_internal.h
--- a/mpcium_amd/csrc/mpcx_internal.h
+++ b/mpcium_amd/csrc/mpcx_internal.h
@@ -59,6 +59,7 @@
   const uint32_t* sched;
   const void* mx_img;
   uint32_t nwaves;
+  const uint32_t* nsq;
 };
 #ifndef MX_WG
 #define MX_WG 4
@@ -91,6 +92,17 @@
 };
 using MxG2 = MxShape<4, 37, 16>;
 using MxG5 = MxShape<2, 37, 32>;
+using MxN2 = MxShape<4, 19, 16>;
+#define MPCX_NSQ_SPLIT_DIGITS 74
+#define MPCX_NSQ_SPLIT_BITS (28 * MPCX_NSQ_SPLIT_DIGITS)
+#define MPCX_NSQ_CONST_DIGITS (5 * 76)
+#ifndef MPCX_NSQ_WG
+#define MPCX_NSQ_WG 4
+#endif
+#ifndef MPCX_NSQ_WPE
+#define MPCX_NSQ_WPE 2
+#endif
+#define MPCX_NSQ_TABLE_SLOTS (2 * 19)
 
 
 #define MPCX_FB_WINDOW_BITS 12
diff --git a/mpcium_amd/csrc/mpcx_mx.hpp b/mpcium_amd/csrc/mpcx_mx.hpp
--- a/mpcium_amd/csrc/mpcx_mx.hpp
+++ b/mpcium_amd/csrc/mpcx_mx.hpp
@@ -68,6 +68,43 @@
   A[0] += from_prev_lane(ctop);
 }
 
+template <int P, int K>
+__device__ __forceinline__ void mx_product2(const uint32_t (&U)[K], uint32_t (&V)[K], const uint32_t* al,
+                                            uint32_t* bl, uint32_t* tr, int p) {
+  uint64_t acc[K];
+#pragma unroll
+  for (int k = 0; k < K; ++k) acc[k] = 0;
+  uint32_t anext = al[0], bnext = bl[0];
+#pragma nounroll
+  for (int o = 0; o < P; ++o) {
+    const uint32_t* ao = al + o * K;
+    const uint32_t* bo = bl + o * K;
+    uint32_t* to = (p == 0 ? bl : tr) + o * K;
+    static_for<0, K>([&](auto uc) {
+      constexpr int u = decltype(uc)::value;
+      const uint32_t ai = anext, bi = bnext;
+      anext = ao[u + 1];
+      bnext = bo[u + 1];
+      static_for<0, K>([&](auto kc) {
+        constexpr int k = decltype(kc)::value;
+        mad64(acc[(k + u) % K], U[k], bi);
+        mad64(acc[(k + u) % K], V[k], ai);
+      });
+      const uint64_t a0 = acc[u];
+      acc[(u + 1) % K] += a0 >> DB;
+      const uint32_t lo = (uint32_t)a0 & M28;
+      to[u] = lo;
+      acc[u] = from_next_lane(p == 0 ? 0u : lo);
+    });
+  }
+  carry_pass64<P, K>(acc);
+  const uint32_t ctop = (uint32_t)(acc[K - 1] >> DB);
+#pragma unroll
+  for (int k = K - 1; k >= 1; --k) V[k] = ((uint32_t)acc[k] & M28) + (uint32_t)(acc[k - 1] >> DB);
+  V[0] = (uint32_t)acc[0] & M28;
+  V[0] += from_prev_lane(ctop);
+}
+
 __device__ __forceinline__ int mx_from_prev_quarter(int v, int lane) {
   return __builtin_amdgcn_ds_bpermute(((lane - 16) & 63) << 2, v);
 }
@@ -84,12 +121,12 @@
   return (int)__builtin_amdgcn_alignbit((uint32_t)((uint64_t)v >> 32), (uint32_t)v, 28);
 }
 
-template <class S, int NJ, int O0, int O1>
+template <class S, int NJ, int O0, int O1, bool ACCUM = false>
 __device__ __forceinline__ void mx_toeplitz(mx_v4i (&acc)[O1 - O0], const uint8_t* f, const mx_v4i (&bf)[S::KB]) {
   auto ld = [&](int j) __attribute__((always_inline)) {
     return *reinterpret_cast<const mx_v4i*>(f + 16 * (S::JMAX - j));
   };
-  static_for<0, O1 - O0>([&](auto oc) { acc[decltype(oc)::value] = mx_v4i{0, 0, 0, 0}; });
+  if constexpr (!ACCUM) static_for<0, O1 - O0>([&](auto oc) { acc[decltype(oc)::value] = mx_v4i{0, 0, 0, 0}; });
   constexpr int JLO = (O0 - 4 * (S::KB - 1)) > 0 ? (O0 - 4 * (S::KB - 1)) : 0;
   constexpr int JHI = (O1 - 1) < (NJ - 1) ? (O1 - 1) : (NJ - 1);
   mx_v4i fnext = ld(JLO);
@@ -128,30 +165,73 @@
     __builtin_amdgcn_sched_barrier(0);                       \
   } while (0)
 #define MX_PROF_ARG , MxProf* pf
+#define MX_PROF_PASS , pf
 #else
 #define MX_STAMP(i) \
   do {              \
   } while (0)
 #define MX_PROF_ARG
+#define MX_PROF_PASS
 #endif
-template <class S, bool SQR, bool B2IN>
-__device__ __forceinline__ void montmul_mx(uint32_t (&A)[S::K], uint32_t* rows, const uint32_t* md,
-                                           const MxConsts& c, int lane MX_PROF_ARG) {
+#ifndef MPCX_MX_TIMING
+#define MPCX_MX_TIMING 0
+#endif
+
+constexpr int PRIO_PRODUCT = 3;
+constexpr int PRIO_FRAG = 2;
+constexpr int PRIO_Q = 1;
+constexpr int PRIO_QM = 0;
+constexpr int PRIO_CARRY = 0;
+
+template <class S>
+struct MxQ {
+  mx_v4i f[S::KB];
+  int top;
+};
+
+__device__ __forceinline__ int mx_neg_bytes(int x) {
+  const uint32_t b = (uint32_t)x, H = 0x80808080u;
+  return (int)((H - (b & ~H)) ^ (~b & H));
+}
+
+template <class S>
+__device__ __forceinline__ void mx_readback(uint32_t (&A)[S::K], const uint32_t* rg, int p MX_PROF_ARG) {
+  constexpr int P = S::P, K = S::K, L = S::L;
+  wave_lds_fence();
+#pragma unroll
+  for (int k = 0; k < K; ++k) A[k] = rg[p * K + k];
+  MX_STAMP(5);
+  uint32_t sg = 0;
+#pragma unroll
+  for (int k = 0; k < K; ++k) sg |= A[k];
+  const bool need = __any((int)sg < 0);
+  for (int it = 0; need && it < L + 2; ++it) {
+    const int top = (int)A[K - 1];
+    const int ctop = (p == P - 1) ? 0 : (top >> DB);
+#pragma unroll
+    for (int k = K - 1; k >= 1; --k) {
+      const int cur = (int)A[k];
+      const bool keep = (k == K - 1) && (p == P - 1);
+      A[k] = (uint32_t)((keep ? cur : (cur & (int)M28)) + ((int)A[k - 1] >> DB));
+    }
+    const int c0 = (int)from_prev_lane((uint32_t)ctop);
+    A[0] = (uint32_t)(((int)A[0] & (int)M28) + (p == 0 ? 0 : c0));
+    bool neg = false;
+#pragma unroll
+    for (int k = 0; k < K; ++k) neg |= (int)A[k] < 0;
+    if (!__any(neg)) break;
+  }
+  MX_STAMP(6);
+}
+
+template <class S, int MODE>
+__device__ __forceinline__ void mx_reduce(uint32_t (&A)[S::K], uint32_t* rows, const uint32_t* md,
+                                          const MxConsts& c, int lane, MxQ<S>& q1 MX_PROF_ARG) {
+  static_assert(MODE == 0 || S::HALVES == 1, "the pair of reductions serves 16 operands per wave");
   constexpr int P = S::P, K = S::K, L = S::L, ROW = S::ROW, KB = S::KB;
   const int g = lane / P, p = lane % P;
   const int n = lane & 15, h = lane >> 4;
   uint32_t* rg = rows + g * ROW;
-#ifndef MPCX_MX_TIMING
-#define MPCX_MX_TIMING 0
-#endif
-  constexpr int PRIO_PRODUCT = 3;
-  constexpr int PRIO_FRAG = 2;
-  constexpr int PRIO_Q = 1;
-  constexpr int PRIO_QM = 0;
-  constexpr int PRIO_CARRY = 0;
-  MX_STAMP(0);
-  __builtin_amdgcn_s_setprio(PRIO_PRODUCT);
-  if constexpr (MPCX_MX_TIMING != 2) mx_product<P, K, SQR, B2IN>(A, rg, rg, rows + S::TRASH_OFF + lane, p);
   __builtin_amdgcn_s_setprio(PRIO_FRAG);
   MX_STAMP(1);
   if constexpr (MPCX_MX_TIMING == 1) return;
@@ -179,13 +259,14 @@
   wave_lds_fence();
   MX_STAMP(2);
 #pragma unroll
-  for (int k = 0; k < K; ++k) rg[p * K + k] = A[k] + md[p * K + k];
+  for (int k = 0; k < K; ++k) rg[p * K + k] = A[k] + md[p * K + k] - (MODE == 2 && k == 0 && p == 0 ? 1u : 0u);
   __builtin_amdgcn_s_setprio(PRIO_Q);
   static_for<0, S::HALVES>([&](auto sc) {
     constexpr int s = decltype(sc)::value;
     uint32_t* rn = rows + (16 * s + n) * ROW;
     if constexpr (s > 0) __builtin_amdgcn_s_setprio(PRIO_Q);
-    mx_v4i qf[KB];
+    mx_v4i qf_own[KB];
+    mx_v4i(&qf)[KB] = MODE == 1 ? q1.f : qf_own;
     {
       int xprev = 0;
       uint32_t X[4] = {0u, 0u, 0u, 0u};
@@ -197,6 +278,7 @@
         int e = lo + (h == 0 ? xprev : x);
         xprev = x;
         if (4 * o + 3 >= L && 4 * o + h >= L) e = 0;
+        if (MODE == 1 && o == (L - 1) / 4) q1.top = e;
         return mx_spread7((uint32_t)e);
       };
       auto norm_block = [&](const mx_v4i& cs, auto oc) __attribute__((always_inline)) {
@@ -214,6 +296,7 @@
         constexpr int O1 = O0 + S::CS1 < S::O1 ? O0 + S::CS1 : S::O1;
         mx_v4i acc[O1 - O0];
         mx_toeplitz<S, S::NJ1, O0, O1>(acc, c.t1, bf[s]);
+        if constexpr (MODE == 2) mx_toeplitz<S, S::NJ1, O0, O1, true>(acc, c.t1, q1.f);
         static_for<0, O1 - O0>([&](auto oc) {
           norm_block(acc[decltype(oc)::value], std::integral_constant<int, O0 + decltype(oc)::value>{});
         });
@@ -229,7 +312,7 @@
         const bool carry_lane = pos == S::N7 - 4;
         const int d = (pos - S::N7) >> 2;
         const int dc = d < 0 ? 0 : d;
-        const int add = carry_lane ? ttop[s] + (1 << 27) : (int)rn[dc];
+        const int add = carry_lane ? ttop[s] + (1 << 27) - (MODE == 2 ? q1.top : 0) : (int)rn[dc];
         const int64_t v = mx_sum64(cs, add);
         const int hi = mx_hi28(v);
         const int top = (int)(uint32_t)v;
@@ -250,34 +333,50 @@
         __builtin_amdgcn_sched_barrier(0);
       });
     }
+    if constexpr (MODE == 1) {
+#pragma unroll
+      for (int kb = 0; kb < KB; ++kb)
+#pragma unroll
+        for (int i = 0; i < 4; ++i) q1.f[kb][i] = mx_neg_bytes(q1.f[kb][i]);
+    }
   });
   __builtin_amdgcn_s_setprio(PRIO_CARRY);
   MX_STAMP(4);
-  wave_lds_fence();
-#pragma unroll
-  for (int k = 0; k < K; ++k) A[k] = rg[p * K + k];
-  MX_STAMP(5);
-  uint32_t sg = 0;
-#pragma unroll
-  for (int k = 0; k < K; ++k) sg |= A[k];
-  const bool need = __any((int)sg < 0);
-  for (int it = 0; need && it < L + 2; ++it) {
-    const int top = (int)A[K - 1];
-    const int ctop = (p == P - 1) ? 0 : (top >> DB);
-#pragma unroll
-    for (int k = K - 1; k >= 1; --k) {
-      const int cur = (int)A[k];
-      const bool keep = (k == K - 1) && (p == P - 1);
-      A[k] = (uint32_t)((keep ? cur : (cur & (int)M28)) + ((int)A[k - 1] >> DB));
-    }
-    const int c0 = (int)from_prev_lane((uint32_t)ctop);
-    A[0] = (uint32_t)(((int)A[0] & (int)M28) + (p == 0 ? 0 : c0));
-    bool neg = false;
-#pragma unroll
-    for (int k = 0; k < K; ++k) neg |= (int)A[k] < 0;
-    if (!__any(neg)) break;
+  if constexpr (MODE == 0) mx_readback<S>(A, rg, p MX_PROF_PASS);
+}
+
+template <class S, bool SQR, bool B2IN>
+__device__ __forceinline__ void montmul_mx(uint32_t (&A)[S::K], uint32_t* rows, const uint32_t* md,
+                                           const MxConsts& c, int lane MX_PROF_ARG) {
+  uint32_t* rg = rows + (lane / S::P) * S::ROW;
+  MX_STAMP(0);
+  __builtin_amdgcn_s_setprio(PRIO_PRODUCT);
+  if constexpr (MPCX_MX_TIMING != 2)
+    mx_product<S::P, S::K, SQR, B2IN>(A, rg, rg, rows + S::TRASH_OFF + lane, lane % S::P);
+  MxQ<S> q;
+  mx_reduce<S, 0>(A, rows, md, c, lane, q MX_PROF_PASS);
+}
+
+template <class S, bool SQR>
+__device__ __forceinline__ void pairmul_mx(uint32_t (&U)[S::K], uint32_t (&V)[S::K], uint32_t* ra, uint32_t* rb,
+                                           uint32_t* tr, const uint32_t* md, const MxConsts& c, int lane) {
+  constexpr int P = S::P, K = S::K;
+  const int g = lane / P, p = lane % P;
+  uint32_t* ga = ra + g * S::ROW;
+  uint32_t* gb = rb + g * S::ROW;
+  __builtin_amdgcn_s_setprio(PRIO_PRODUCT);
+  if constexpr (SQR) {
+    mx_product<P, K, false, false>(V, gb, gb, tr, p);
+    mx_product<P, K, true, true>(U, ga, ga, tr, p);
+  } else {
+    mx_product2<P, K>(U, V, ga, gb, tr, p);
+    mx_product<P, K, false, false>(U, ga, ga, tr, p);
   }
-  MX_STAMP(6);
-}
-
-}
+  MxQ<S> q;
+  mx_reduce<S, 1>(U, ra, md, c, lane, q);
+  mx_reduce<S, 2>(V, rb, md, c, lane, q);
+  mx_readback<S>(U, ga, p);
+  mx_readback<S>(V, gb, p);
+}
+
+}
diff --git a/mpcium_amd/mpcx.py b/mpcium_amd/mpcx.py
--- a/mpcium_amd/mpcx.py
+++ b/mpcium_amd/mpcx.py
@@ -33,6 +33,7 @@
     ("mpcx_modulus_info", ctypes.c_int, [_vp, _u32p, _u32p]),
     ("mpcx_modulus_geometry", ctypes.c_int, [_vp, _u32p, _u32p, _u32p, _u32p]),
     ("mpcx_mx_tables", ctypes.c_int, [_u32p, ctypes.c_uint32, ctypes.c_uint32, ctypes.c_void_p, ctypes.c_size_t]),
+    ("mpcx_nsq_consts", ctypes.c_int, [_u32p, ctypes.c_uint32, _u32p, ctypes.c_size_t, ctypes.POINTER(ctypes.c_int)]),
     ("mpcx_modexp_batch", ctypes.c_int, [_vp, ctypes.c_uint32, _vp, ctypes.c_uint32, _vp, ctypes.c_uint32,
                                          ctypes.c_int, _vp, ctypes.c_uint32]),
     ("mpcx_modexp_batch_device", ctypes.c_int, [_vp, ctypes.c_uint32, _vp, ctypes.c_uint32, _vp, ctypes.c_uint32,
@@ -159,7 +160,7 @@
     return {"direct_bytes": v[0].value, "bounced_bytes": v[1].value, "bounce_allocs": v[2].value}
 
 
-MX_TABLE_BYTES = {148: 2 * 16 * 720, 74: 2 * 16 * 432}
+MX_TABLE_BYTES = {148: 2 * 16 * 720, 76: 2 * 16 * 432, 74: 2 * 16 * 432}
 
 
 def mx_tables(m: int, L: int = 148) -> bytes:
@@ -168,6 +169,19 @@
     out = ctypes.create_string_buffer(max(n, 1))
     _check(lib().mpcx_mx_tables(w.ctypes.data_as(ctypes.POINTER(ctypes.c_uint32)), 128, L, out, n))
     return out.raw
+
+
+def nsq_consts(m: int):
+    w = int_to_words(m, 128)
+    n = 5 * 76 + MX_TABLE_BYTES[76] // 4
+    out = np.zeros(n, dtype="<u4")
+    sq = ctypes.c_int(0)
+    u32p = ctypes.POINTER(ctypes.c_uint32)
+    _check(lib().mpcx_nsq_consts(w.ctypes.data_as(u32p), 128, out.ctypes.data_as(u32p), n, ctypes.byref(sq)))
+    if not sq.value:
+        return None
+    v = [sum(int(d) << (28 * i) for i, d in enumerate(out[76 * j:76 * j + 76])) for j in range(5)]
+    return v[0], (v[1], v[2]), (v[3], v[4]), out[380:].tobytes()
 
 
 def select_device(index: int):
```

Result: faster. 595,700 modexp/s, median of 6 (+13.9%).
